# txthpc/amg

Measured on AMD Instinct MI355X. Metric: V-cycle iters/sec + fine-level SpMV GB/s (%HBM peak), 64M-row 7pt Poisson, higher is better.
Workload: dtype f64

## Files before the change

amg_amd/_native.py:

```python
from __future__ import annotations

import ctypes as C
import os
from pathlib import Path

import numpy as np

ROOT = Path(__file__).resolve().parent.parent
LIB_PATH = Path(os.environ["SSS_AMG_LIB"]) if os.environ.get("SSS_AMG_LIB") else ROOT / "amg_amd" / "lib" / "libsss_amg.so"
BIN_PATH = ROOT / "amg_amd" / "bin" / "amg"

_dbl_p = C.POINTER(C.c_double)
_int_p = C.POINTER(C.c_int)


class SSS_MAT(C.Structure):
    _fields_ = [("num_rows", C.c_int), ("num_cols", C.c_int), ("num_nnzs", C.c_int),
                ("row_ptr", _int_p), ("col_idx", _int_p), ("val", _dbl_p)]


class SSS_IMAT(C.Structure):
    _fields_ = [("num_rows", C.c_int), ("num_cols", C.c_int), ("num_nnzs", C.c_int),
                ("row_ptr", _int_p), ("col_idx", _int_p), ("val", _int_p)]


class SSS_VEC(C.Structure):
    _fields_ = [("n", C.c_int), ("d", _dbl_p)]


class SSS_IVEC(C.Structure):
    _fields_ = [("n", C.c_int), ("d", _int_p)]


class SSS_RTN(C.Structure):
    _fields_ = [("ares", C.c_double), ("rres", C.c_double), ("nits", C.c_int)]


class SSS_AMG_PARS(C.Structure):
    _fields_ = [("cycle_type", C.c_int), ("tol", C.c_double), ("ctol", C.c_double), ("max_it", C.c_int),
                ("cs_type", C.c_int), ("max_levels", C.c_int), ("coarse_dof", C.c_int), ("smoother", C.c_int),
                ("relax", C.c_double), ("cf_order", C.c_int), ("pre_iter", C.c_int), ("post_iter", C.c_int),
                ("poly_deg", C.c_int), ("interp_type", C.c_int), ("strong_threshold", C.c_double),
                ("max_row_sum", C.c_double), ("trunc_threshold", C.c_double)]


class SSS_AMG_COMP(C.Structure):
    _fields_ = [("A", SSS_MAT), ("R", SSS_MAT), ("P", SSS_MAT), ("b", SSS_VEC), ("x", SSS_VEC),
                ("cfmark", SSS_IVEC), ("wp", SSS_VEC)]


class SSS_AMG(C.Structure):
    _fields_ = [("num_levels", C.c_int), ("cg", C.POINTER(SSS_AMG_COMP)), ("pars", SSS_AMG_PARS),
                ("rtn", SSS_RTN)]


class SSS_SMTR(C.Structure):
    _fields_ = [("smoother", C.c_int), ("A", C.POINTER(SSS_MAT)), ("b", C.POINTER(SSS_VEC)),
                ("x", C.POINTER(SSS_VEC)), ("relax", C.c_double), ("nsweeps", C.c_int), ("istart", C.c_int),
                ("iend", C.c_int), ("istep", C.c_int), ("ndeg", C.c_int), ("cf_order", C.c_int),
                ("ordering", _int_p)]


class SSS_KRYLOV(C.Structure):
    _fields_ = [("tol", C.c_double), ("A", C.POINTER(SSS_MAT)), ("b", C.POINTER(SSS_VEC)),
                ("u", C.POINTER(SSS_VEC)), ("restart", C.c_int), ("matrix", C.c_int), ("stop_type", C.c_int)]


class SSS_HIP_OPTS(C.Structure):
    _fields_ = [("device", C.c_int), ("smoother", C.c_int), ("coarse", C.c_int), ("row_cap", C.c_int),
                ("use_graph", C.c_int), ("verbose", C.c_int),
                ("inner", C.c_int), ("inner_from", C.c_int), ("relabel", C.c_int),
                ("sorted_tiles", C.c_int), ("sum_order", C.c_int), ("inner_long", C.c_int), ("formats", C.c_int)]

FORMATS = {"auto": -1, "full": 0, "lean": 1}


class SSS_HIP_LEVEL_INFO(C.Structure):
    _fields_ = [("rows", C.c_int), ("nnz", C.c_int), ("nnz_p", C.c_int), ("dag_f", C.c_int),
                ("dag_c", C.c_int), ("smoother_kind", C.c_int), ("gs_engine_f", C.c_int), ("gs_engine_c", C.c_int),
                ("gs_stall", C.c_int), ("a_format", C.c_int), ("a_stream_bytes", C.c_longlong),
                ("inner", C.c_int), ("r_format", C.c_int), ("p_format", C.c_int), ("pad_", C.c_int)]


SMOOTH = {"exact": 0, "hybrid": 1, "jacobi": 2}
COARSE_RS, COARSE_PMIS = 1, 3
COARSE = {"krylov": 0, "direct": 1}
VEC = {"b": 0, "x": 1, "wp": 2}
SPMV = {"mxy": 0, "amxpy": 1, "resid": 2, "acc": 3}

ABI_SYMBOLS = [
    "SSS_amg_solve", "SSS_amg_cycle", "SSS_amg_coarest_solve", "SSS_amg_smoother_pre", "SSS_amg_smoother_post",
    "SSS_blas_mv_amxpy", "SSS_blas_mv_mxy", "SSS_solver_amg", "SSS_get_time", "SSS_free", "SSS_blas_vec_norm2",
    "SSS_print_itinfo", "SSS_exit_on_errcode", "SSS_blas_array_norm2", "SSS_blas_array_dot", "SSS_blas_array_axpy",
    "SSS_blas_array_norminf", "SSS_blas_array_set", "SSS_blas_array_axpby", "SSS_blas_array_ax", "SSS_vec_create",
    "SSS_vec_set_value", "SSS_mat_destroy", "SSS_vec_destroy", "SSS_calloc", "SSS_amg_data_create",
    "SSS_ivec_create", "SSS_mat_struct_create", "SSS_vec_cp", "SSS_iarray_cp", "SSS_blas_array_cp", "SSS_mat_cp",
    "SSS_mat_get_diag", "SSS_ivec_destroy", "SSS_amg_data_destroy", "SSS_imat_trans", "SSS_iarray_set",
    "SSS_imat_destroy", "SSS_mat_trans", "SSS_blas_mat_rap", "SSS_realloc", "SSS_amg_complexity_print",
    "SSS_amg_setup", "SSS_amg_coarsen", "SSS_amg_interp", "SSS_amg_interp_trunc", "interp_DIR", "SSS_mat_read",
    "SSS_amg_pars_init", "SSS_amg_pars_print", "mmio_info", "mmio_data",
    "sss_hip_opts_default", "sss_hip_device_count", "sss_hip_mem_info", "sss_hip_hier_create", "sss_hip_hier_destroy",
    "sss_hip_setup_create", "sss_amg_setup_hooked", "sss_hip_rap", "sss_hip_pmis", "sss_pmis_host",
    "sss_hip_std_pattern", "sss_std_pattern_host", "sss_hip_interp_std",
    "sss_hip_upload_vec", "sss_hip_download_vec", "sss_hip_cycle", "sss_hip_residual_norm", "sss_hip_pcg",
    "sss_hip_fgmres", "sss_hip_host_orth",
    "SSS_amg_save", "SSS_amg_load",
    "sss_hip_coarse_solve", "sss_hip_smooth", "sss_hip_sync", "sss_hip_level_info_get", "sss_hip_num_levels", "sss_hip_tail_from",
    "sss_hip_cycle_launches", "sss_hip_cycle_bytes",
    "sss_hip_spmv_plan_create", "sss_hip_spmv_plan_destroy", "sss_hip_spmv", "sss_hip_host_spmv", "sss_hip_host_spmv_order",
    "sss_hip_host_smooth", "sss_hip_host_coarse_solve", "sss_hip_host_cache_clear", "sss_hip_time_level0_spmv", "sss_hip_time_iterations",
    "sss_hip_time_level0_spmv_csr", "sss_hip_time_levels", "sss_hip_dist_time_tail_levels",
    "sss_gen_stencil",
    "sss_hip_rccl_unique_id", "sss_hip_comm_rccl", "sss_hip_comm_host", "sss_hip_comm_timing", "sss_hip_comm_destroy",
    "sss_hip_dist_create", "sss_hip_dist_destroy", "sss_hip_dist_info", "sss_hip_dist_level_flags",
    "sss_hip_dist_upload_vec",
    "sss_hip_dist_download_vec", "sss_hip_dist_cycle", "sss_hip_dist_residual_norm", "sss_hip_dist_sync",
    "sss_hip_dist_time_level0_spmv", "sss_hip_dist_time_levels", "sss_hip_dist_halo_stats",
    "sss_part_plan_create", "sss_part_plan_destroy", "sss_part_save", "sss_part_plan_load",
    "sss_hip_dist_create_from_files", "sss_hip_dist_level_size", "sss_part_plan_nagg", "sss_part_plan_level",
    "sss_part_plan_matrix", "sss_part_plan_ids", "sss_part_plan_halo",
]

_ip, _dp = C.POINTER(C.c_int), C.POINTER(C.c_double)
EXCHANGE_FN = C.CFUNCTYPE(C.c_int, C.c_void_p, C.c_int, _ip, _ip, _dp, C.c_int, _ip, _ip, _dp)
ALLREDUCE_FN = C.CFUNCTYPE(C.c_int, C.c_void_p, _dp, C.c_int)
ALLGATHERV_FN = C.CFUNCTYPE(C.c_int, C.c_void_p, _dp, C.c_int, _dp, _ip, _ip)


A_FORMATS = {0: "CSR (12 B/entry)", 1: "column-sorted tiles (12 B/entry)", 2: "dictionary tiles (4 B/entry)",
             3: "value-dictionary sorted tiles (5 B/entry)"}


def a_format_name(code: int) -> str:
    if code & 64:
        return "dictionary ELL (1 B/entry, padded rows)"
    if code & 128:
        return "column ELL (4 B/entry, padded rows)"
    return A_FORMATS.get(code & 3, A_FORMATS[0])


class SSS_HIP_HOST_TRANSPORT(C.Structure):
    _fields_ = [("ctx", C.c_void_p), ("exchange", EXCHANGE_FN), ("allreduce_sum", ALLREDUCE_FN),
                ("allgatherv", ALLGATHERV_FN)]

_lib = None


def _declare(lib):
    P = C.POINTER
    sig = {
        "SSS_amg_pars_init": (None, [P(SSS_AMG_PARS)]),
        "SSS_amg_pars_print": (None, [P(SSS_AMG_PARS)]),
        "SSS_amg_setup": (None, [P(SSS_AMG), P(SSS_MAT), P(SSS_AMG_PARS)]),
        "SSS_amg_data_destroy": (None, [P(SSS_AMG)]),
        "SSS_amg_solve": (SSS_RTN, [P(SSS_AMG), P(SSS_VEC), P(SSS_VEC)]),
        "SSS_print_itinfo": (None, [C.c_int, C.c_int, C.c_double, C.c_double, C.c_double]),
        "SSS_amg_cycle": (None, [P(SSS_AMG)]),
        "SSS_solver_amg": (SSS_RTN, [P(SSS_MAT), P(SSS_VEC), P(SSS_VEC), P(SSS_AMG_PARS)]),
        "SSS_mat_read": (None, [C.c_char_p, P(SSS_MAT)]),
        "SSS_mat_destroy": (None, [P(SSS_MAT)]),
        "SSS_mat_trans": (SSS_MAT, [P(SSS_MAT)]),
        "SSS_blas_mat_rap": (SSS_MAT, [P(SSS_MAT), P(SSS_MAT), P(SSS_MAT)]),
        "SSS_amg_coarsen": (C.c_int, [P(SSS_MAT), P(SSS_IVEC), P(SSS_MAT), P(SSS_IMAT), P(SSS_AMG_PARS)]),
        "SSS_amg_interp": (None, [P(SSS_MAT), P(SSS_IVEC), P(SSS_MAT), P(SSS_IMAT), P(SSS_AMG_PARS)]),
        "SSS_ivec_create": (SSS_IVEC, [C.c_int]),
        "SSS_blas_mv_amxpy": (None, [C.c_double, P(SSS_MAT), P(SSS_VEC), P(SSS_VEC)]),
        "SSS_blas_mv_mxy": (None, [P(SSS_MAT), P(SSS_VEC), P(SSS_VEC)]),
        "mmio_info": (C.c_int, [_int_p, _int_p, _int_p, _int_p, C.c_char_p]),
        "mmio_data": (C.c_int, [_int_p, _int_p, _dbl_p, C.c_char_p]),
        "sss_gen_stencil": (C.c_int, [C.c_int] * 6 + [P(SSS_MAT)]),
        "sss_hip_opts_default": (None, [P(SSS_HIP_OPTS)]),
        "sss_hip_device_count": (C.c_int, []),
        "sss_hip_mem_info": (C.c_int, [P(C.c_size_t), P(C.c_size_t)]),
        "sss_hip_hier_create": (C.c_void_p, [P(SSS_AMG), P(SSS_HIP_OPTS)]),
        "sss_hip_setup_create": (C.c_void_p, [P(SSS_AMG), P(SSS_MAT), P(SSS_AMG_PARS), P(SSS_HIP_OPTS),
                                              P(C.c_double)]),
        "sss_hip_hier_destroy": (None, [C.c_void_p]),
        "sss_hip_rap": (C.c_int, [P(SSS_MAT), P(SSS_MAT), P(SSS_MAT), P(SSS_MAT)]),
        "sss_hip_pmis": (C.c_int, [P(SSS_IMAT), _int_p, _int_p, _int_p]),
        "sss_pmis_host": (C.c_int, [P(SSS_IMAT), _int_p, _int_p, _int_p]),
        "sss_hip_std_pattern": (C.c_int, [P(SSS_IMAT), _int_p, C.c_int, P(SSS_MAT)]),
        "sss_std_pattern_host": (C.c_int, [P(SSS_IMAT), _int_p, C.c_int, P(SSS_MAT)]),
        "sss_hip_interp_std": (C.c_int, [P(SSS_MAT), P(SSS_IMAT), _int_p, P(SSS_MAT), C.c_double]),
        "SSS_mat_struct_create": (SSS_MAT, [C.c_int, C.c_int, C.c_int]),
        "sss_hip_upload_vec": (C.c_int, [C.c_void_p, C.c_int, C.c_int, _dbl_p, C.c_int]),
        "sss_hip_download_vec": (C.c_int, [C.c_void_p, C.c_int, C.c_int, _dbl_p, C.c_int]),
        "sss_hip_cycle": (C.c_int, [C.c_void_p]),
        "sss_hip_residual_norm": (C.c_int, [C.c_void_p, _dbl_p]),
        "sss_hip_pcg": (C.c_int, [C.c_void_p, C.c_double, C.c_int, P(C.c_int), _dbl_p, _dbl_p, C.c_int]),
        "sss_hip_fgmres": (C.c_int, [C.c_void_p, C.c_double, C.c_int, C.c_int, P(C.c_int), _dbl_p, _dbl_p, C.c_int]),
        "sss_hip_host_orth": (C.c_int, [C.c_int, C.c_int, _dbl_p, _dbl_p, _dbl_p, _dbl_p]),
        "SSS_amg_save": (C.c_int, [P(SSS_AMG), C.c_char_p]),
        "SSS_amg_load": (C.c_int, [P(SSS_AMG), C.c_char_p]),
        "sss_hip_coarse_solve": (C.c_int, [C.c_void_p]),
        "sss_hip_smooth": (C.c_int, [C.c_void_p, C.c_int, C.c_int]),
        "sss_hip_sync": (C.c_int, [C.c_void_p]),
        "sss_hip_level_info_get": (C.c_int, [C.c_void_p, C.c_int, P(SSS_HIP_LEVEL_INFO)]),
        "sss_hip_num_levels": (C.c_int, [C.c_void_p]),
        "sss_hip_tail_from": (C.c_int, [C.c_void_p]),
        "sss_hip_cycle_launches": (C.c_int, [C.c_void_p]),
        "sss_hip_cycle_bytes": (C.c_int, [C.c_void_p, C.POINTER(C.c_double), C.c_int]),
        "sss_hip_host_spmv": (C.c_int, [C.c_int, C.c_double, P(SSS_MAT), _dbl_p, _dbl_p, _dbl_p, C.c_int]),
        "sss_hip_host_spmv_order": (C.c_int, [C.c_int, C.c_double, P(SSS_MAT), _dbl_p, _dbl_p, _dbl_p, C.c_int, C.c_int]),
        "sss_hip_host_smooth": (C.c_int, [P(SSS_SMTR), C.c_int]),
        "sss_hip_host_coarse_solve": (C.c_int, [P(SSS_MAT), P(SSS_VEC), P(SSS_VEC), C.c_double, C.c_int,
                                                C.c_int]),
        "sss_hip_time_level0_spmv": (C.c_int, [C.c_void_p, C.c_int, _dbl_p]),
        "sss_hip_time_level0_spmv_csr": (C.c_int, [C.c_void_p, C.c_int, _dbl_p]),
        "sss_hip_time_levels": (C.c_int, [C.c_void_p, C.c_int, _dbl_p, C.c_int]),
        "sss_hip_dist_time_tail_levels": (C.c_int, [C.c_void_p, C.c_int, _dbl_p, C.c_int]),
        "sss_hip_time_iterations": (C.c_int, [C.c_void_p, C.c_int, _dbl_p, _dbl_p]),
        "sss_hip_rccl_unique_id": (C.c_int, [C.c_char_p]),
        "sss_hip_comm_rccl": (C.c_void_p, [C.c_int, C.c_int, C.c_char_p, C.c_int]),
        "sss_hip_comm_host": (C.c_void_p, [C.c_int, C.c_int, P(SSS_HIP_HOST_TRANSPORT)]),
        "sss_hip_comm_timing": (C.c_void_p, [C.c_int, C.c_int]),
        "sss_hip_comm_destroy": (None, [C.c_void_p]),
        "sss_hip_dist_create": (C.c_void_p, [P(SSS_AMG), P(SSS_HIP_OPTS), C.c_void_p, C.c_int]),
        "sss_hip_dist_destroy": (None, [C.c_void_p]),
        "sss_hip_dist_info": (C.c_int, [C.c_void_p, _int_p, _int_p, _int_p, _int_p]),
        "sss_hip_dist_level_size": (C.c_int, [C.c_void_p, C.c_int, _int_p, _int_p, P(C.c_longlong)]),
        "sss_hip_dist_level_flags": (C.c_int, [C.c_void_p, C.c_int]),
        "sss_hip_dist_upload_vec": (C.c_int, [C.c_void_p, C.c_int, _dbl_p, C.c_int]),
        "sss_hip_dist_download_vec": (C.c_int, [C.c_void_p, C.c_int, _dbl_p, C.c_int]),
        "sss_hip_dist_cycle": (C.c_int, [C.c_void_p]),
        "sss_hip_dist_residual_norm": (C.c_int, [C.c_void_p, _dbl_p]),
        "sss_hip_dist_sync": (C.c_int, [C.c_void_p]),
        "sss_hip_dist_time_level0_spmv": (C.c_int, [C.c_void_p, C.c_int, _dbl_p]),
        "sss_hip_dist_time_levels": (C.c_int, [C.c_void_p, C.c_int, _dbl_p, _dbl_p, C.c_int]),
        "sss_hip_dist_halo_stats": (C.c_int, [C.c_void_p, P(C.c_longlong), P(C.c_longlong), C.c_int, C.c_int,
                                              _int_p, _int_p, _int_p]),
        "sss_part_plan_create": (C.c_void_p, [P(SSS_AMG), C.c_int, C.c_int, C.c_int]),
        "sss_part_save": (C.c_int, [P(SSS_AMG), C.c_int, C.c_int, C.c_char_p]),
        "sss_part_plan_load": (C.c_void_p, [C.c_char_p]),
        "sss_hip_dist_create_from_files": (C.c_void_p, [C.c_char_p, P(SSS_HIP_OPTS), C.c_void_p]),
        "sss_part_plan_destroy": (None, [C.c_void_p]),
        "sss_part_plan_nagg": (C.c_int, [C.c_void_p]),
        "sss_part_plan_level": (C.c_int, [C.c_void_p, C.c_int, _int_p, _int_p, _int_p, _int_p]),
        "sss_part_plan_matrix": (C.c_int, [C.c_void_p, C.c_int, C.c_int, P(SSS_MAT)]),
        "sss_part_plan_ids": (C.c_int, [C.c_void_p, C.c_int, P(_int_p), P(_int_p)]),
        "sss_part_plan_halo": (C.c_int, [C.c_void_p, C.c_int, _int_p, P(_int_p), P(_int_p), P(_int_p), _int_p,
                                         P(_int_p), P(_int_p)]),
    }
    for name, (res, args) in sig.items():
        try:
            fn = getattr(lib, name)
        except AttributeError:
            if os.environ.get("SSS_AMG_LIB"):
                continue
            raise
        fn.restype = res
        fn.argtypes = args
    return lib


def lib():
    global _lib
    if _lib is None:
        if not LIB_PATH.exists():
            raise RuntimeError(f"{LIB_PATH} is missing: run `make` (or __graft_entry__.build())")
        _lib = _declare(C.CDLL(str(LIB_PATH)))
    return _lib


def dptr(a: np.ndarray):
    assert a.dtype == np.float64 and a.flags["C_CONTIGUOUS"]
    return a.ctypes.data_as(_dbl_p)


def iptr(a: np.ndarray):
    assert a.dtype == np.int32 and a.flags["C_CONTIGUOUS"]
    return a.ctypes.data_as(_int_p)


def csr_arrays(M: SSS_MAT, copy: bool = True):
    n, nnz = M.num_rows, M.num_nnzs
    rp = np.ctypeslib.as_array(M.row_ptr, shape=(n + 1,))
    ci = np.ctypeslib.as_array(M.col_idx, shape=(nnz,)) if nnz else np.zeros(0, np.int32)
    v = np.ctypeslib.as_array(M.val, shape=(nnz,)) if nnz else np.zeros(0, np.float64)
    return (rp.copy(), ci.copy(), v.copy()) if copy else (rp, ci, v)


class NumpyCSR:

    def __init__(self, rp, ci, v, ncols=None):
        self.rp = np.ascontiguousarray(rp, dtype=np.int32)
        self.ci = np.ascontiguousarray(ci, dtype=np.int32)
        self.v = np.ascontiguousarray(v, dtype=np.float64)
        n = len(self.rp) - 1
        self.mat = SSS_MAT(n, n if ncols is None else ncols, len(self.v), iptr(self.rp), iptr(self.ci),
                           dptr(self.v))


def default_pars() -> SSS_AMG_PARS:
    p = SSS_AMG_PARS()
    lib().SSS_amg_pars_init(C.byref(p))
    return p


def pmis(rp, ci, device: bool = False):
    rp = np.ascontiguousarray(rp, dtype=np.int32)
    ci = np.ascontiguousarray(ci, dtype=np.int32)
    n = len(rp) - 1
    S = SSS_IMAT(n, n, len(ci), iptr(rp), iptr(ci) if len(ci) else None, None)
    mark = np.full(max(n, 1), -7, np.int32)
    nc, rounds = C.c_int(-1), C.c_int(-1)
    fn = lib().sss_hip_pmis if device else lib().sss_pmis_host
    rc = fn(C.byref(S), iptr(mark), C.byref(nc), C.byref(rounds))
    if rc != 0:
        err = RuntimeError(f"PMIS split failed ({rc})")
        err.rc, err.mark = rc, mark[:n]
        raise err
    return mark[:n], nc.value, rounds.value


def _imat(rp, ci):
    rp = np.ascontiguousarray(rp, dtype=np.int32)
    ci = np.ascontiguousarray(ci, dtype=np.int32)
    n = len(rp) - 1
    return SSS_IMAT(n, n, len(ci), iptr(rp), iptr(ci) if len(ci) else None, None), (rp, ci)


def std_pattern(rp, ci, mark, device: bool = False):
    S, keep = _imat(rp, ci)
    mark = np.ascontiguousarray(mark, dtype=np.int32)
    P = SSS_MAT()
    fn = lib().sss_hip_std_pattern if device else lib().sss_std_pattern_host
    rc = fn(C.byref(S), iptr(mark), int((mark == 1).sum()), C.byref(P))
    if rc != 0:
        err = RuntimeError(f"standard pattern failed ({rc})")
        err.rc = rc
        raise err
    prp, pci, _ = csr_arrays(P)
    lib().SSS_mat_destroy(C.byref(P))
    return prp, pci


def interp_std(A_csr, S_csr, mark, P_pattern, trunc: float, device: bool = False):
    Am = NumpyCSR(*A_csr)
    S, keep = _imat(*S_csr)
    mark = np.ascontiguousarray(mark, dtype=np.int32)
    prp = np.ascontiguousarray(P_pattern[0], dtype=np.int32)
    pci = np.ascontiguousarray(P_pattern[1], dtype=np.int32)
    n = len(prp) - 1
    P = lib().SSS_mat_struct_create(n, int((mark == 1).sum()), len(pci))
    C.memmove(P.row_ptr, prp.ctypes.data, prp.nbytes)
    if len(pci):
        C.memmove(P.col_idx, pci.ctypes.data, pci.nbytes)
    try:
        if device:
            rc = lib().sss_hip_interp_std(C.byref(Am.mat), C.byref(S), iptr(mark), C.byref(P), trunc)
            if rc != 0:
                err = RuntimeError(f"standard interpolation failed ({rc})")
                err.rc = rc
                raise err
# ... 473 lines not shown
```

amg_amd/csrc/sss_build.hip:

```cpp
#include <hipcub/hipcub.hpp>

#include "sss_engine.hpp"

namespace sss {

namespace {

__global__ __launch_bounds__(kBlock) void merged_keys(int n, int G, const int *__restrict__ rp,
                                                      const int *__restrict__ ci, const int *__restrict__ seg,
                                                      unsigned *__restrict__ key)
{
    const int r = blockIdx.x * kBlock + threadIdx.x;
    if (r >= n) return;
    const unsigned rig = (unsigned)(r % G);
    const int s = seg ? seg[r] : rp[r + 1];
    for (int k = rp[r]; k < rp[r + 1]; ++k)
        key[k] = ((unsigned)ci[k] << kMergeShift) | ((k >= s ? 1u : 0u) << 3) | rig;
}

__global__ __launch_bounds__(kBlock) void group_bounds(int n, int G, int ng, const int *__restrict__ rp,
                                                       int *__restrict__ gp)
{
    const int g = blockIdx.x * kBlock + threadIdx.x;
    if (g < ng) gp[g] = rp[g * G];
    else if (g == ng) gp[g] = rp[n];
}

__global__ __launch_bounds__(kBlock) void segment_offsets(int n, const int *__restrict__ rp, const int *__restrict__ seg,
                                                          int *__restrict__ off)
{
    const int r = blockIdx.x * kBlock + threadIdx.x;
    if (r < n) {
        off[2 * r] = rp[r];
        off[2 * r + 1] = seg[r];
    } else if (r == n) {
        off[2 * n] = rp[n];
    }
}

int segmented_sort(const unsigned *kin, unsigned *kout, const double *vin, double *vout, int nnz, int nseg,
                   const int *off, hipStream_t s)
{
    if (nnz == 0 || nseg == 0) return 0;
    size_t tb = 0;
    SSS_HIP(hipcub::DeviceSegmentedRadixSort::SortPairs(nullptr, tb, kin, kout, vin, vout, nnz, nseg, off, off + 1, 0,
                                                        32, s));
    void *tmp = nullptr;
    SSS_HIP(hipMalloc(&tmp, std::max<size_t>(tb, 1)));
    const hipError_t e = hipcub::DeviceSegmentedRadixSort::SortPairs(tmp, tb, kin, kout, vin, vout, nnz, nseg, off,
                                                                     off + 1, 0, 32, s);
    const hipError_t e2 = hipStreamSynchronize(s);
    (void)hipFree(tmp);
    SSS_HIP(e);
    SSS_HIP(e2);
    return 0;
}

int upload_seg(const int *h_seg, int n, int **d_seg)
{
    *d_seg = nullptr;
    if (!h_seg) return 0;
    *d_seg = dev_alloc<int>((size_t)n);
    if (!*d_seg) return hip_fail(hipErrorOutOfMemory, "hipMalloc(seg)", __FILE__, __LINE__);
    return h2d(*d_seg, h_seg, sizeof(int) * (size_t)n);
}

}

bool device_builders_on()
{
    const char *e = getenv("SSS_HIP_GPU_BUILD");
    return !(e && *e == '0');
}

int merged_build_device(DevCSR &d, const int *h_seg)
{
    const int n = d.n, G = d.mg_G, ng = (n + G - 1) / G;
    d.mg_ng = ng;
    d.mg_gp = dev_alloc<int>((size_t)ng + 1);
    d.mg_k = dev_alloc<unsigned>((size_t)d.nnz);
    d.mg_v = dev_alloc<double>((size_t)d.nnz);
    unsigned *key = dev_alloc<unsigned>((size_t)d.nnz);
    int *dseg = nullptr;
    int rc = (!d.mg_gp || !d.mg_k || !d.mg_v || !key) ? hip_fail(hipErrorOutOfMemory, "hipMalloc(merged)", __FILE__, __LINE__)
                                                        : upload_seg(h_seg, n, &dseg);
    if (!rc) {
        hipLaunchKernelGGL(group_bounds, dim3((ng + kBlock) / kBlock), dim3(kBlock), 0, nullptr, n, G, ng, d.rp, d.mg_gp);
        if (n > 0)
            hipLaunchKernelGGL(merged_keys, dim3((n + kBlock - 1) / kBlock), dim3(kBlock), 0, nullptr, n, G, d.rp, d.ci,
                               dseg, key);
        const hipError_t e = hipGetLastError();
        if (e != hipSuccess) rc = hip_fail(e, "merged_keys", __FILE__, __LINE__);
    }
    if (!rc) rc = segmented_sort(key, d.mg_k, d.v, d.mg_v, d.nnz, ng, d.mg_gp, nullptr);
    dev_free(key);
    dev_free(dseg);
    return rc;
}

int sort_rows_device(DevCSR &d, const int *h_seg)
{
    const int n = d.n;
    unsigned *kin = dev_alloc<unsigned>((size_t)d.nnz);
    double *vin = dev_alloc<double>((size_t)d.nnz);
    int *dseg = nullptr, *off = nullptr;
    int rc = (!kin || !vin) ? hip_fail(hipErrorOutOfMemory, "hipMalloc(row sort)", __FILE__, __LINE__) : 0;
    if (!rc && h_seg) {
        rc = upload_seg(h_seg, n, &dseg);
        off = rc ? nullptr : dev_alloc<int>(2 * (size_t)n + 1);
        if (!rc && !off) rc = hip_fail(hipErrorOutOfMemory, "hipMalloc(row sort)", __FILE__, __LINE__);
        if (!rc) hipLaunchKernelGGL(segment_offsets, dim3((n + kBlock) / kBlock), dim3(kBlock), 0, nullptr, n, d.rp, dseg, off);
    }
    if (!rc && hipMemcpy(kin, d.ci, sizeof(int) * (size_t)d.nnz, hipMemcpyDeviceToDevice) != hipSuccess) rc = ERROR_MISC;
    if (!rc && hipMemcpy(vin, d.v, sizeof(double) * (size_t)d.nnz, hipMemcpyDeviceToDevice) != hipSuccess) rc = ERROR_MISC;
    if (!rc)
        rc = segmented_sort(kin, reinterpret_cast<unsigned *>(d.ci), vin, d.v, d.nnz, h_seg ? 2 * n : n,
                            h_seg ? off : d.rp, nullptr);
    if (!rc) d.rows_sorted = true;
    dev_free(kin);
    dev_free(vin);
    dev_free(dseg);
    dev_free(off);
    return rc;
}

}
```

amg_amd/csrc/sss_engine.hpp:

```cpp
#pragma once

#include <hip/hip_runtime.h>

#include <algorithm>
#include <atomic>
#include <chrono>
#include <cstdlib>
#include <string>
#include <functional>
#include <memory>
#include <cstdio>
#include <thread>
#include <vector>

#include "../../include/sss_hip.h"

extern "C" void sss_trace_push(const char *fmt, ...) __attribute__((format(printf, 1, 2)));
extern "C" void sss_trace_pop(void);
namespace sss {
struct TraceRange {
    template <class... Args>
    explicit TraceRange(const char *fmt, Args... a) { sss_trace_push(fmt, a...); }
    ~TraceRange() { sss_trace_pop(); }
    TraceRange(const TraceRange &) = delete;
// ... 20 lines not shown
inline T *dev_alloc(size_t count)
{
    void *p = nullptr;
    if (count == 0) count = 1;
    if (hipMalloc(&p, count * sizeof(T)) != hipSuccess) return nullptr;
    return static_cast<T *>(p);
}
inline void dev_free(void *p)
{
    if (p) (void)hipFree(p);
}

template <class T>
struct HostBuf {
    std::unique_ptr<T[]> p;
    size_t n = 0;
    void resize(size_t m)
    {
        p.reset(m ? new T[m] : nullptr);
        sss_huge_hint(p.get(), m * sizeof(T));
        n = m;
    }
    T *data() { return p.get(); }
    const T *data() const { return p.get(); }
    size_t size() const { return n; }
    T &operator[](size_t i) { return p[i]; }
    const T &operator[](size_t i) const { return p[i]; }
};

int host_pool_threads();
void host_thread_background();
bool host_pool_run(const std::function<void()> &work);

template <class Fn>
void parallel_chunks(int n, int grain, Fn fn)
{
    if (n <= 0) return;
    if (n <= grain || host_pool_threads() <= 1) {
        fn(0, n);
        return;
    }
    std::atomic<int> next{0};
    std::function<void()> work = [&]() {
        for (;;) {
            const int lo = next.fetch_add(grain);
            if (lo >= n) return;
            fn(lo, std::min(n, lo + grain));
        }
    };
    if (!host_pool_run(work)) work();
}

struct PhaseTimer {
    const char *what;
    bool on;
    double t;
    std::vector<std::pair<const char *, double>> marks;
    static double now()
    {
        return std::chrono::duration<double>(std::chrono::steady_clock::now().time_since_epoch()).count();
    }
    explicit PhaseTimer(const char *w) : what(w)
    {
        const char *e = getenv("SSS_HIP_TIMING");
        on = e && atoi(e) >= 2;
        t = now();
    }
    void mark(const char *name)
    {
        if (!on) return;
        const double t1 = now();
        marks.emplace_back(name, t1 - t);
        t = t1;
    }
    ~PhaseTimer()
    {
        if (!on || marks.empty()) return;
        std::string s;
        char buf[96];
        for (auto &m : marks) {
            snprintf(buf, sizeof(buf), " %s %.3f", m.first, m.second);
            s += buf;
        }
        fprintf(stderr, "[sss_hip]     %s:%s\n", what, s.c_str());
    }
};

inline void parallel_prefix(int *a, int n)
{
    constexpr int kC = 1 << 16;
    const int nc = (n + kC - 1) / kC;
    if (nc <= 1) {
        for (int i = 0; i < n; ++i) a[i + 1] += a[i];
        return;
    }
    std::vector<long long> tot((size_t)nc + 1, 0);
    parallel_chunks(nc, 1, [&](int c0, int c1) {
        for (int c = c0; c < c1; ++c) {
            long long t = 0;
            for (int i = c * kC; i < std::min(n, (c + 1) * kC); ++i) t += a[i + 1];
            tot[(size_t)c + 1] = t;
        }
    });
    tot[0] = a[0];
    for (int c = 0; c < nc; ++c) tot[(size_t)c + 1] += tot[c];
    parallel_chunks(nc, 1, [&](int c0, int c1) {
        for (int c = c0; c < c1; ++c) {
            long long run = tot[c];
            for (int i = c * kC; i < std::min(n, (c + 1) * kC); ++i) run += a[i + 1], a[i + 1] = (int)run;
        }
    });
}

int h2d(void *dst, const void *src, size_t bytes);

struct DevCSR {
    int n = 0, ncols = 0, nnz = 0;
    int *rp = nullptr, *ci = nullptr;
    double *v = nullptr;
    int nblk = 0;
    int *blk = nullptr;
    int2 *bk = nullptr;
    const int2 *h_bk = nullptr;
    int split_row = -1;
    int split_blk = 0;
    bool wave_rows = false;
    int ngrid = 0;
    unsigned *pk = nullptr;
    double *pv = nullptr;
    int2 *pb = nullptr;
    bool vec_rows = false;
    bool rows_sorted = false;
    bool tree_long = false;
    unsigned char *dv_ell = nullptr;
    int ell_w = 0;
    int *dv_ell_base = nullptr;
    unsigned *dv_xell = nullptr;
    int xell_w = 0;
    int xell_shift = 0;
    long long stream_bytes = 0;
    unsigned *dv_code = nullptr;
    unsigned char *dv_vi = nullptr;
    int4 *dv_pd = nullptr;
    int *dv_dd = nullptr;
    double *dv_vd = nullptr;
    int mg_G = 0;
    int mg_ng = 0;
    int mg_W = 4;
    int mg_acc = 0;
    int *mg_gp = nullptr;
    bool mg_two = false;
    unsigned *mg_k = nullptr;
    double *mg_v = nullptr;
};
constexpr int kMergeShift = 4;
constexpr int kTileShift = 11;
constexpr int kTileColBits = 20;
constexpr unsigned kTileDiagMark = (1u << kTileColBits) - 256;
static_assert((1 << kTileShift) == kTileEntries, "tile packing");
static_assert(1 + kTileColBits + kTileShift == 32, "tile packing");
enum { kEncSortedTiles = 1, kEncFreeOrder = 2, kEncDict = 4, kEncMergedOnly = 8, kEncXell = 16,
       kEncEll = 32,
       kEncEllBase = 64 };
int devcsr_upload(DevCSR &d, const SSS_MAT &h, int split = -1, int enc = 0, const int *seg = nullptr);
int level_encoding(const sss_hip_opts &o);
int transfer_encoding(const sss_hip_opts &o);
int restriction_encoding(const sss_hip_opts &o);
void devcsr_free(DevCSR &d);
int build_row_blocks(const int *h_rp, int n, std::vector<int> &blk, int split = -1);
int upload_block_bounds(int2 **dst, const std::vector<int> &blk, const int *h_rp, const int2 **host = nullptr);
int wave_row_min();
int free_row_min();
int devcsr_sort_rows(DevCSR &d, const SSS_MAT &h, const int *seg = nullptr);
bool device_builders_on();
int merged_build_device(DevCSR &d, const int *h_seg);
int sort_rows_device(DevCSR &d, const int *h_seg);
struct DevDict;
DevDict devdict(const DevCSR &A, int blo);
inline bool has_dict(const DevCSR &A)
{
    return A.dv_code != nullptr || A.dv_vi != nullptr || A.dv_ell != nullptr || A.dv_xell != nullptr;
}
constexpr int kXell = 256;
constexpr int rows_per_wg(int K) { return K >= kXell ? 1 : K >= 8 ? 2 : 1; }
template <class F>
inline void with_tile_kind(const DevCSR &A, F f)
{
    if (A.dv_xell) {
        if (A.xell_w == 8) f(std::integral_constant<int, kXell + 8>{});
        else if (A.xell_w == 16) f(std::integral_constant<int, kXell + 16>{});
        else if (A.xell_w == 20) f(std::integral_constant<int, kXell + 20>{});
        else if (A.xell_w == 24) f(std::integral_constant<int, kXell + 24>{});
        else if (A.xell_w == 32) f(std::integral_constant<int, kXell + 32>{});
        else f(std::integral_constant<int, kXell + 40>{});
    } else if (A.dv_ell) {
        if (A.ell_w == 8) f(std::integral_constant<int, 8>{});
        else if (A.ell_w == 16) f(std::integral_constant<int, 16>{});
        else f(std::integral_constant<int, 32>{});
    } else if (has_dict(A)) {
        f(std::integral_constant<int, 1>{});
    } else {
        f(std::integral_constant<int, 0>{});
    }
}
template <class F>
inline bool with_merged_kind(const DevCSR &A, F f)
{
    if (A.mg_G == 8 && A.mg_acc) f(std::integral_constant<int, 8>{}, std::true_type{});
    else if (A.mg_G == 8) f(std::integral_constant<int, 8>{}, std::false_type{});
    else if (A.mg_G == 4 && A.mg_acc) f(std::integral_constant<int, 4>{}, std::true_type{});
    else if (A.mg_G == 4) f(std::integral_constant<int, 4>{}, std::false_type{});
    else return false;
    return true;
}

struct ByteLedger {
    double bytes[kMaxLevels + 2] = {};
    int slot = 0;
};
extern thread_local ByteLedger *g_ledger;
inline void ledger_add(double b)
{
    if (g_ledger) g_ledger->bytes[g_ledger->slot] += b;
}
inline bool ledger_on() { return g_ledger != nullptr; }
double matrix_bytes(const DevCSR &A, int blo, int bhi);
double matrix_bytes_rows(const DevCSR &A, int lo, int hi);
inline double xgather_bytes(const DevCSR &A, double rows) { return A.n ? 8.0 * rows * A.ncols / A.n : 0.0; }

sss_hip_hier *hier_create_impl(const SSS_AMG *mg, const sss_hip_opts *o, int level_base, hipStream_t stream);
double *hier_vec(sss_hip_hier *h, int level, int which);
const std::vector<int> &hier_perm(sss_hip_hier *h, int level);
int level_kind_of(const sss_hip_opts &o, int global_level);
int hier_stall_check(sss_hip_hier *h);
unsigned *hier_err_word(sss_hip_hier *h);
bool hier_coarse_on_device(sss_hip_hier *h);
void hier_set_err_word(sss_hip_hier *h, unsigned *err);
int level_inner_of(const sss_hip_opts &o, int global_level, long long rows, long long nnz);

int launch_spmv(const DevCSR &A, int op, double alpha, const double *x, const double *b, double *y,
                int cap, double *partial, hipStream_t stream);
int launch_prolong_inject(int m, int lo, const int *col, const double *e, double *x, hipStream_t stream);
int launch_spmv_range(const DevCSR &A, int blo, int bhi, int op, double alpha, const double *x, const double *b,
                      double *y, double *partial, hipStream_t stream);
inline int launch_spmv_blocks(const DevCSR &A, int nblk, int op, double alpha, const double *x, const double *b,
                              double *y, double *partial, hipStream_t stream)
{
    return launch_spmv_range(A, 0, nblk, op, alpha, x, b, y, partial, stream);
}

struct GsPersist {
    int engine = 0;
    int lo = 0, hi = 0;
    int G = 64;
    bool overlap = false;
    bool natural = false, desc = false;
    int nchunks = 0, grid = 0;
    int *ck = nullptr;
    int *h_off = nullptr;
    unsigned *ctl = nullptr;
    unsigned *err = nullptr;
    int spin = 0;
    unsigned long long *gran = nullptr;
};
struct GsFused {
    int engine = 0;
    int sweeps = 0;
    int n = 0, split = 0;
    int G = 64;
    bool overlap = false;
    int shards = 8;
    int depth = 0, nchunks = 0, grid = 0;
    int *ck = nullptr;
    int *nodes = nullptr;
    int *rp0 = nullptr, *ci0 = nullptr;
    double *v0 = nullptr;
    unsigned *ctl = nullptr;
    unsigned *err = nullptr;
    int spin = 0;
    unsigned long long *gran = nullptr;
};
struct PassSchedule {
    int depth = 0;
    std::vector<int> h_off;
    int *rows = nullptr;
    int nrows = 0;
    int max_width = 0;
    bool compact = false;
    bool range = false;
    int lo = 0, hi = 0, blo = 0, bhi = 0;
    double *y2 = nullptr;
    DevCSR ts_nl, ts_lo;
    int *ts_split = nullptr;
    double *ts_P = nullptr;
    DevCSR sub;
    int *map = nullptr;
    double *y = nullptr;
    GsPersist gp;
};
int gs_persist_build(PassSchedule &ps, const SSS_MAT &A, int lo, int hi, bool long_rows, bool natural = false,
                     bool desc = false);
void gs_persist_free(PassSchedule &ps);
int gs_persist_run(const PassSchedule &ps, const DevCSR &A, const double *b, double *x, const double *deff,
                   hipStream_t s);
int gs_persist_error(const PassSchedule &ps, unsigned *out);
int gs_fused_build(GsFused &f, const SSS_MAT &A, const DevCSR *dA, const PassSchedule *pass, const int *cls,
                   int sweeps);
int gs_fused_run(const GsFused &f, const DevCSR &A, const double *b, double *x, const double *d_first,
                 const double *d_later, bool x_zero, hipStream_t s);
void gs_fused_free(GsFused &f);
int gs_fused_error(const GsFused &f, unsigned *out, bool clear);
struct SmootherPlan;
void smoother_set_err(SmootherPlan &sp, unsigned *err);
int launch_err_flag(unsigned *err, double *out, hipStream_t s);
struct SmootherPlan {
    int kind = SSS_HIP_SMOOTH_EXACT;
    bool natural = false;
    double *nd_first = nullptr, *nd_later = nullptr;
    PassSchedule pass[2];
    GsFused fz;
    double *d_first = nullptr;
    double *d_later = nullptr;
    int *cls = nullptr;
    bool long_rows = false;
    int *diag_pos = nullptr;
    int inner = 0;
    double *x2 = nullptr;
    int csplit = 0;
    bool fuse_resid = false;
    bool f_overwritten = false;
    bool own_diag = false;
    bool pend_ok = false;
    bool finite = false;
};
struct ResidFuse {
    double *r = nullptr;
    double *partial = nullptr;
    bool done = false;
};
struct PassHooks {
    void *ctx = nullptr;
    int (*exchange)(void *ctx, double *vec) = nullptr;
    double *w0 = nullptr, *w1 = nullptr;
    std::function<int(double *vec, int blo, int bhi, const std::function<void(int, int)> &launch)> split;
};
int smoother_build(SmootherPlan &sp, const SSS_MAT &A, const int *mark, int kind, const DevCSR *dA = nullptr,
                   int inner = 0, const int *gcls = nullptr, int enc = 0);
int smoother_build_natural(SmootherPlan &sp, const SSS_MAT &A, int lo, int hi);
struct XSrc {
    const double *f, *c;
    int split;
    __device__ __forceinline__ double operator()(int j) const { return j < split ? f[j] : c[j]; }
};
inline XSrc xsrc_of(const double *x) { return XSrc{x, x, 0x7fffffff}; }
void launch_ts_stage0(const DevCSR &M, int lo, const int *split, const double *b, XSrc x, const double *deff,
                      double *P, double *y, hipStream_t s);
void launch_ts_inner(const DevCSR &M, int lo, const double *deff, const double *P, const double *ycols, int col_off,
                     const double *ykeep, double *y, hipStream_t s);
void smoother_free(SmootherPlan &sp);
int smoother_run(const SmootherPlan &sp, const DevCSR &A, const double *b, double *x, int sweeps,
                 hipStream_t stream, const PassHooks *hooks = nullptr, ResidFuse *rf = nullptr,
                 const double *pre_f = nullptr, bool x_zero = false, bool post = false);
int launch_f_residual_pending(const SmootherPlan &sp, const DevCSR &A, const double *b, const double *x, double *r,
                              double *partial, double *pend, hipStream_t s);
// ... 36 lines not shown
```

amg_amd/csrc/sss_hier.hip:

```cpp
#include "sss_engine.hpp"
#include "sss_tail.hpp"

#include <atomic>
#include <condition_variable>
#include <mutex>
#include <thread>

#include <chrono>

#include <cmath>

#include <algorithm>
#include <cstdlib>
#include <cstring>
#include <string>
#include <thread>
#include <vector>

using namespace sss;

struct sss_hip_hier {
    int nl = 0;
    SSS_AMG_PARS pars{};
    sss_hip_opts opts{};
// ... 1197 lines not shown
    };
    SSS_HIP(hipMemcpyAsync(bs, L.b, bytes, hipMemcpyDeviceToDevice, s));
    SSS_HIP(hipMemcpyAsync(xs, L.x, bytes, hipMemcpyDeviceToDevice, s));
    double nb = 0.0, rel = 1.0;
    int it = 0;
    std::vector<double> R((size_t)(m + 1) * m, 0.0), cs((size_t)m), sn((size_t)m), g((size_t)m + 1);
    if ((rc = norm_of(bs, &nb))) return rc;
    if (!std::isfinite(nb)) rc = ERROR_SOLVER_EXIT;
    if (!rc && nb == 0.0) {
        SSS_HIP(hipMemsetAsync(xs, 0, bytes, s));
        rel = 0.0;
    }
    bool done = rc || nb == 0.0 || maxit < 1;
    while (!done) {
        double beta = 0.0;
        if ((rc = launch_spmv(L.A, SSS_HIP_SPMV_RESID, -1.0, xs, bs, V, 0, nullptr, s))) break;
        if ((rc = norm_of(V, &beta))) break;
        if (!std::isfinite(beta)) {
            rc = ERROR_SOLVER_EXIT;
            break;
        }
        if (it == 0) rel = beta / nb;
        if (beta == 0.0) break;
        if ((rc = launch_scale_inv(n, V, dh, s))) break;
        g[0] = beta;
        int ncols = 0;
        for (int j = 0; j < m && !done; ++j) {
            ++it;
            double *w = V + (size_t)(j + 1) * ld, *hj = R.data() + (size_t)j * (m + 1);
            if ((rc = precondition(V + (size_t)j * ld, Z + (size_t)j * ld))) break;
            if ((rc = launch_spmv(L.A, SSS_HIP_SPMV_MXY, 1.0, Z + (size_t)j * ld, nullptr, w, 0, nullptr, s))) break;
            if ((rc = launch_orth_step(n, j + 1, V, ld, w, h->fg_part, dc, dh, s))) break;
            if ((rc = launch_scale_inv(n, w, dh + j + 1, s))) break;
            if ((rc = fetch(dh, j + 2))) break;
            if (!std::isfinite(hh[j + 1])) {
                rc = ERROR_SOLVER_EXIT;
                break;
            }
            for (int i = 0; i < j + 2; ++i) hj[i] = hh[i];
            for (int i = 0; i < j; ++i) {
                const double t = cs[i] * hj[i] + sn[i] * hj[i + 1];
                hj[i + 1] = -sn[i] * hj[i] + cs[i] * hj[i + 1];
                hj[i] = t;
            }
            const double d = std::hypot(hj[j], hj[j + 1]);
            cs[j] = d != 0.0 ? hj[j] / d : 1.0;
            sn[j] = d != 0.0 ? hj[j + 1] / d : 0.0;
            hj[j] = d;
            g[j + 1] = -sn[j] * g[j];
            g[j] = cs[j] * g[j];
            rel = std::fabs(g[j + 1]) / nb;
            if (hist && it <= hist_cap) hist[it - 1] = rel;
            ncols = j + 1;
            done = rel < tol || it >= maxit || hh[j + 1] == 0.0;
        }
        if (rc) break;
        for (int i = ncols - 1; i >= 0; --i) {
            double t = g[i];
            for (int l = i + 1; l < ncols; ++l) t -= R[(size_t)l * (m + 1) + i] * yh[l];
            yh[i] = R[(size_t)i * (m + 1) + i] != 0.0 ? t / R[(size_t)i * (m + 1) + i] : 0.0;
        }
        SSS_HIP(hipMemcpyAsync(dy, yh, sizeof(double) * (size_t)ncols, hipMemcpyHostToDevice, s));
        if ((rc = launch_multi_axpy(n, ncols, Z, ld, dy, 1.0, xs, nullptr, s))) break;
        SSS_HIP(hipStreamSynchronize(s));
    }
    SSS_HIP(hipMemcpyAsync(L.x, xs, bytes, hipMemcpyDeviceToDevice, s));
    SSS_HIP(hipMemcpyAsync(L.b, bs, bytes, hipMemcpyDeviceToDevice, s));
    SSS_HIP(hipStreamSynchronize(s));
    h->resid_c_ready = false;
    h->pending_f = false;
    if (iters) *iters = it;
    if (relres) *relres = rel;
    if (rc) return rc;
    return hier_stall_check(h);
}

extern "C" int sss_hip_sync(sss_hip_hier *h)
{
    SSS_HIP(hipStreamSynchronize(h->stream));
    return hier_stall_check(h);
}

extern "C" int sss_hip_num_levels(sss_hip_hier *h) { return h ? h->nl : 0; }

extern "C" int sss_hip_cycle_bytes(sss_hip_hier *h, double *out, int nslots)
{
    if (!h || !out || nslots < h->nl + 2) return ERROR_INPUT_PAR;
    const bool pend = h->pending_f && h->nl > 1 && h->pars.pre_iter > 0;
    const bool f_only_next = h->nl > 1 && h->L[0].sm.fuse_resid && h->pars.post_iter > 0;
    const bool keep_pending = h->pending_f, keep_ready = h->resid_c_ready;
    ByteLedger led;
    SSS_HIP(hipStreamSynchronize(h->stream));
    SSS_HIP(hipStreamBeginCapture(h->stream, hipStreamCaptureModeThreadLocal));
    g_ledger = &led;
    int rc = walk_cycle(h, [](sss_hip_hier *hh) {
        return hh->coarse_mode == SSS_HIP_COARSE_DIRECT ? coarse_direct_apply(hh->direct, hh->L[hh->nl - 1].b,
                                                                              hh->L[hh->nl - 1].x, hh->stream)
                                                        : 0;
    }, pend);
    led.slot = kMaxLevels;
    if (!rc) rc = enqueue_residual_norm(h, f_only_next);
    g_ledger = nullptr;
    hipGraph_t g = nullptr;
    hipError_t e = hipStreamEndCapture(h->stream, &g);
    if (g) (void)hipGraphDestroy(g);
    h->pending_f = keep_pending;
    h->resid_c_ready = keep_ready;
    if (rc) return rc;
    SSS_HIP(e);
    for (int i = 0; i < nslots; ++i) out[i] = 0.0;
    for (int l = 0; l < h->nl && l < kMaxLevels; ++l) out[l] = led.bytes[l];
    out[nslots - 2] = led.bytes[kMaxLevels];
    out[nslots - 1] = led.bytes[kMaxLevels + 1];
    return 0;
}

extern "C" int sss_hip_tail_from(sss_hip_hier *h) { return h ? h->tail.from : -1; }

extern "C" int sss_hip_cycle_launches(sss_hip_hier *h)
{
    if (!h || !(h->cycle_graph_ready || h->cycle_graph_ready_p)) return -1;
    return h->cycle_graph_ready_p ? h->cycle_kernels_p : h->cycle_kernels;
}

extern "C" int sss_hip_level_info_get(sss_hip_hier *h, int level, sss_hip_level_info *out)
{
    if (!h || level < 0 || level >= h->nl) return ERROR_INPUT_PAR;
    auto &L = h->L[level];
    out->rows = L.A.n;
    out->nnz = L.A.nnz;
    out->nnz_p = L.P.nnz;
    out->dag_f = L.sm.pass[0].depth;
    out->dag_c = L.sm.pass[1].depth;
    out->smoother_kind = L.sm.kind;
    out->inner = L.sm.inner;
    out->gs_engine_f = L.sm.fz.engine ? 3 : L.sm.pass[0].gp.engine;
    out->gs_engine_c = L.sm.fz.engine ? 3 : L.sm.pass[1].gp.engine;
    unsigned ef = 0, ec = 0, ez = 0;
    if (gs_persist_error(L.sm.pass[0], &ef) || gs_persist_error(L.sm.pass[1], &ec)) return ERROR_MISC;
    if (L.sm.fz.err && hipMemcpy(&ez, L.sm.fz.err, sizeof(unsigned), hipMemcpyDeviceToHost) != hipSuccess)
        return ERROR_MISC;
    out->gs_stall = (int)(ef | ec | ez);
    auto fmt = [](const DevCSR &M) {
        return (M.pk ? 1 : 0) | (has_dict(M) ? 2 : 0) | (M.vec_rows ? 4 : 0) | (M.mg_G ? 8 : 0) | (M.wave_rows ? 16 : 0) |
               (M.dv_ell ? 64 : 0) | (M.dv_xell ? 128 : 0);
    };
    out->a_format = fmt(L.A);
    out->r_format = level + 1 < h->nl ? fmt(L.R) : 0;
    out->p_format = level + 1 < h->nl ? fmt(L.P) : 0;
    out->a_stream_bytes = L.A.stream_bytes;
    return 0;
}

extern "C" int sss_hip_time_levels(sss_hip_hier *h, int reps, double *level_ms, int nslots)
{
    if (!h || reps < 1 || nslots < h->nl) return ERROR_INPUT_PAR;
    const size_t nev = (size_t)4 * h->nl + 4;
    h->lev_ev.assign(nev, nullptr);
    h->lev_tag.assign(nev, -1);
    int rc = 0;
    for (auto &e : h->lev_ev)
        if (hipEventCreate(&e) != hipSuccess) rc = ERROR_MISC;
    std::vector<double> acc((size_t)h->nl, 0.0);
    for (int r = 0; r < reps && !rc; ++r) {
        h->lev_n = 0;
        h->resid_c_ready = h->pending_f = false;
        rc = walk_cycle(h, [](sss_hip_hier *hh) { return sss_hip_coarse_solve(hh); }, false);
        if (!rc && hipStreamSynchronize(h->stream) != hipSuccess) rc = ERROR_MISC;
        for (int k = 1; k < h->lev_n && !rc; ++k) {
            float t = 0.0f;
            if (hipEventElapsedTime(&t, h->lev_ev[(size_t)k - 1], h->lev_ev[(size_t)k]) != hipSuccess) rc = ERROR_MISC;
            const int lv = h->lev_tag[(size_t)k];
            if (lv >= 0 && lv < h->nl) acc[(size_t)lv] += t;
        }
    }
    for (hipEvent_t e : h->lev_ev)
        if (e) (void)hipEventDestroy(e);
    h->lev_ev.clear();
    h->lev_tag.clear();
    h->lev_n = 0;
    h->resid_c_ready = h->pending_f = false;
    if (rc) return rc;
    for (int l = 0; l < h->nl; ++l) level_ms[l] = acc[(size_t)l] / reps;
    return 0;
}

extern "C" int sss_hip_time_level0_spmv(sss_hip_hier *h, int reps, double *avg_ms)
{
    auto &L = h->L[0];
    SSS_HIP(hipStreamSynchronize(h->stream));
    SSS_HIP(hipEventRecord(h->ev0, h->stream));
    for (int r = 0; r < reps; ++r) {
        int rc = launch_spmv(L.A, SSS_HIP_SPMV_RESID, -1.0, L.x, L.b, L.wp, 0, nullptr, h->stream);
        if (rc) return rc;
    }
    SSS_HIP(hipEventRecord(h->ev1, h->stream));
    SSS_HIP(hipEventSynchronize(h->ev1));
    float ms = 0.f;
    SSS_HIP(hipEventElapsedTime(&ms, h->ev0, h->ev1));
    *avg_ms = (double)ms / reps;
    return 0;
}

extern "C" int sss_hip_time_level0_spmv_csr(sss_hip_hier *h, int reps, double *avg_ms)
{
    auto &L = h->L[0];
    if (L.A.wave_rows || L.A.vec_rows || L.A.dv_xell) return sss_hip_time_level0_spmv(h, reps, avg_ms);
    DevCSR c = L.A;
    c.pk = nullptr;
    c.pv = nullptr;
    c.pb = nullptr;
    c.dv_ell = nullptr;
    c.dv_code = nullptr;
    c.dv_vi = nullptr;
    SSS_HIP(hipStreamSynchronize(h->stream));
    SSS_HIP(hipEventRecord(h->ev0, h->stream));
    for (int r = 0; r < reps; ++r) {
        int rc = launch_spmv(c, SSS_HIP_SPMV_RESID, -1.0, L.x, L.b, L.wp, 0, nullptr, h->stream);
        if (rc) return rc;
    }
    SSS_HIP(hipEventRecord(h->ev1, h->stream));
    SSS_HIP(hipEventSynchronize(h->ev1));
    float ms = 0.f;
    SSS_HIP(hipEventElapsedTime(&ms, h->ev0, h->ev1));
    *avg_ms = (double)ms / reps;
    return 0;
}

extern "C" int sss_hip_time_iterations(sss_hip_hier *h, int reps, double *avg_ms, double *absres)
{
    SSS_HIP(hipStreamSynchronize(h->stream));
    SSS_HIP(hipEventRecord(h->ev0, h->stream));
    for (int r = 0; r < reps; ++r) {
        int rc = sss_hip_cycle(h);
        if (!rc) rc = sss_hip_residual_norm(h, absres);
        if (rc) return rc;
    }
    SSS_HIP(hipEventRecord(h->ev1, h->stream));
    SSS_HIP(hipEventSynchronize(h->ev1));
    float ms = 0.f;
    SSS_HIP(hipEventElapsedTime(&ms, h->ev0, h->ev1));
    *avg_ms = (double)ms / reps;
    return 0;
}

extern char **environ;

namespace {
struct HostCSR {
    DevCSR d;
    ~HostCSR() { devcsr_free(d); }
};
struct HostSmooth {
    std::mutex run;
    DevCSR d;
    SmootherPlan sp;
    ~HostSmooth()
    {
        smoother_free(sp);
        devcsr_free(d);
    }
};
struct HostCoarse {
    std::mutex run;
    DevCSR d;
    CoarseDirect cd;
    bool direct = false;
    CoarseKrylov *k = nullptr;
    ~HostCoarse()
    {
        if (direct) coarse_direct_free(cd);
        coarse_krylov_destroy(k);
        devcsr_free(d);
    }
};

inline unsigned long long mix64(unsigned long long h, unsigned long long w)
{
    h ^= w * 0x9E3779B97F4A7C15ull;
    h = (h << 31) | (h >> 33);
    return h * 0xC2B2AE3D27D4EB4Full;
}
unsigned long long hash_bytes(const void *p, size_t n, unsigned long long seed)
{
    const unsigned char *b = static_cast<const unsigned char *>(p);
    constexpr size_t kChunk = (size_t)1 << 20;
    const int nc = (int)((n + kChunk - 1) / kChunk);
    std::vector<unsigned long long> part((size_t)std::max(nc, 1), 0);
    parallel_chunks(nc, 1, [&](int c0, int c1) {
        for (int c = c0; c < c1; ++c) {
            const size_t lo = (size_t)c * kChunk, hi = std::min(n, lo + kChunk);
            unsigned long long h = 0x2545F4914F6CDD1Dull ^ (unsigned long long)c;
            size_t i = lo;
            for (; i + 8 <= hi; i += 8) {
                unsigned long long w;
                std::memcpy(&w, b + i, 8);
                h = mix64(h, w);
            }
            for (; i < hi; ++i) h = mix64(h, b[i]);
            part[(size_t)c] = h;
        }
    });
    unsigned long long h = mix64(seed, n);
    for (auto v : part) h = mix64(h, v);
    return h;
}
// ... 202 lines not shown
```

amg_amd/csrc/sss_smooth.hip:

```cpp
#include "sss_engine.hpp"
#include "sss_spmv_dev.hpp"

#include <algorithm>
#include <chrono>
#include <cstdlib>
#include <type_traits>
#include <cmath>

namespace sss {

template <class T>
static int upload_array(T **dst, const T *src, size_t count)
{
    *dst = dev_alloc<T>(count);
    if (!*dst) return hip_fail(hipErrorOutOfMemory, "hipMalloc(plan array)", __FILE__, __LINE__);
    return count == 0 ? 0 : h2d(*dst, src, sizeof(T) * count);
}
static int upload_ints(int **dst, const std::vector<int> &src) { return upload_array(dst, src.data(), src.size()); }
static int upload_ints(int **dst, const HostBuf<int> &src) { return upload_array(dst, src.data(), src.size()); }
static int upload_doubles(double **dst, const HostBuf<double> &src) { return upload_array(dst, src.data(), src.size()); }
static int upload_doubles(double **dst, const std::vector<double> &src) { return upload_array(dst, src.data(), src.size()); }

int smoother_build(SmootherPlan &sp, const SSS_MAT &A, const int *mark, int kind, const DevCSR *dA, int inner,
                   const int *gcls, int enc)
// ... 613 lines not shown
        if (partial && valid) {
            const double t = block_sum(sq, es.red);
            if (threadIdx.x == 0) partial[bid] = t;
        }
    }
}

template <int MODE, int DICT = 0>
__device__ __forceinline__ void relax_range_body(int blo, const int2 *__restrict__ blk, const int *__restrict__ rp,
                                                      const int *__restrict__ ci, const double *__restrict__ v,
                                                      const int *__restrict__ diag_pos, int lo,
                                                      const double *__restrict__ b, double *x,
                                                      const double *__restrict__ yp, double *__restrict__ y,
                                                      const double *__restrict__ deff, const unsigned *__restrict__ pk,
                                                      const double *__restrict__ pv, const int2 *__restrict__ pb,
                                                      double *__restrict__ rr, double *__restrict__ partial, XSrc xs,
                                                      DevDict dt = DevDict())
{
    if constexpr (DICT >= kXell) {
        relax_range_xell<MODE, DICT - kXell>(blo, blk, lo, b, x, y, deff, rr, partial, xs, dt);
    } else if constexpr (DICT == 8 && kEllPairs) {
        relax_range_ell2<MODE>(blo, blk, lo, b, x, y, deff, rr, partial, xs, dt);
    } else if constexpr (DICT >= 8) {
        relax_range_ell<MODE, DICT>(blo, blk, lo, b, x, y, deff, rr, partial, xs, dt);
    } else {
    __shared__ SpmvSmem sm;
    __shared__ std::conditional_t<DICT != 0, DictSmem, char> dsm;
    DictSmem *ds = nullptr;
    if constexpr (DICT != 0) ds = &dsm;
    const int bid = blo + xcd_bid();
    const int2 ba = blk[bid], be = blk[bid + 1];
    const int r0 = ba.x, r1 = be.x, k0 = ba.y, k1 = be.y;
    auto fetch = [&](int c) -> double { return xs(c); };
    auto dval = [&](int r) -> double { return deff ? deff[r] : sm.d[r - r0]; };
    auto finish = [&](int r, double acc) {
        const double d = dval(r);
        if (MODE != 1) {
            if (div_ok(d)) x[r] = acc / d;
        } else {
            y[r - lo] = div_ok(d) ? acc / d : xs(r);
        }
    };
    if (k1 - k0 <= kTileEntries) {
        const int r = r0 + (int)threadIdx.x;
        int a = 0, e = 0, dp = -1;
        double br = 0.0;
        if (r < r1) a = rp[r] - k0, e = rp[r + 1] - k0, dp = diag_pos[r], br = b[r];
        stage_any(sm.v, k0, k1, ci, v, pk, pv, pb, bid, r0, deff ? (double *)nullptr : sm.d, fetch, dt, ds, r1, rp);
        __syncthreads();
        double sq = 0.0;
        if (r < r1) {
            if constexpr (MODE >= 2) {
                const RelaxRow o = relax_row<MODE>(TileProds{sm.v}, a, dp >= 0, dp - k0, e, br, [&] { return dval(r); },
                                                   [&]() -> double { return x[r]; });
                if constexpr (MODE == 2) {
                    if (o.upd) x[r] = o.xn;
                } else {
                    y[r - lo] = o.xn;
                }
                rr[r] = o.res;
                sq = o.res * o.res;
            } else {
                finish(r, relax_acc(TileProds{sm.v}, a, dp >= 0, dp - k0, e, br));
            }
        }
        if constexpr (MODE >= 2) {
            if (partial) {
                const double t = block_sum(sq, sm.red);
                if (threadIdx.x == 0) partial[bid] = t;
            }
        }
    } else if constexpr (MODE < 2) {
        const int r = r0, dp = diag_pos[r];
        const double acc = long_row_chunks(
            k0, k1, b[r],
            [&](int base, int m) {
                stage_any(sm.v, base, base + m, ci, v, pk, pv, pb, bid, r0, deff ? (double *)nullptr : sm.d, fetch, dt,
                          ds, r1, rp);
            },
            [&](int base, int m, double acc) {
                if (dt.tree_long) {
                    if (threadIdx.x == 0 && dp >= base && dp < base + m) sm.v[dp - base] = 0.0;
                    __syncthreads();
                    const double c = block_tree_sum(sm.v, 0, m, sm.red);
                    if (threadIdx.x == 0) acc -= c;
                } else if (threadIdx.x == 0) {
                    if (dp >= base && dp < base + m) {
                        acc = chain_sub(acc, sm.v, 0, dp - base);
                        acc = chain_sub(acc, sm.v, dp - base + 1, m);
                    } else {
                        acc = chain_sub(acc, sm.v, 0, m);
                    }
                }
                return acc;
            });
        if (threadIdx.x == 0) finish(r, acc);
    }
    }
}

#define SSS_RELAX_ARGS                                                                                          \
    int blo, const int2 *__restrict__ blk, const int *__restrict__ rp, const int *__restrict__ ci,                 \
        const double *__restrict__ v, const int *__restrict__ diag_pos, int lo, const double *__restrict__ b,      \
        double *x, const double *__restrict__ yp, double *__restrict__ y, const double *__restrict__ deff,          \
        const unsigned *__restrict__ pk, const double *__restrict__ pv, const int2 *__restrict__ pb,               \
        double *__restrict__ rr, double *__restrict__ partial, XSrc xs, DevDict dt
#define SSS_RELAX_PASS blo, blk, rp, ci, v, diag_pos, lo, b, x, yp, y, deff, pk, pv, pb, rr, partial, xs, dt
template <int MODE, int DICT = 0>
__global__ __launch_bounds__(kBlock) void relax_range(SSS_RELAX_ARGS)
{
    relax_range_body<MODE, DICT>(SSS_RELAX_PASS);
}
template <int MODE, int DICT = 0>
__global__ __launch_bounds__(kBlock) __attribute__((amdgpu_waves_per_eu(5, 8))) void relax_range_occ(SSS_RELAX_ARGS)
{
    relax_range_body<MODE, DICT>(SSS_RELAX_PASS);
}
template <int M, int K, class... Args>
static void launch_relax_range(int blo, int nb, hipStream_t s, DevDict dt, Args... args)
{
    if constexpr (K < 8) {
        hipLaunchKernelGGL((relax_range_occ<M, K>), dim3(nb), dim3(kBlock), 0, s, blo, args..., dt);
    } else {
        dt.bend = blo + nb;
        hipLaunchKernelGGL((relax_range<M, K>), dim3((nb + rows_per_wg(K) - 1) / rows_per_wg(K)), dim3(kBlock), 0, s, blo,
                           args..., dt);
    }
}

template <int MODE, bool TREE>
__global__ __launch_bounds__(kBlock) void relax_range_wave(int lo, int hi, const int *__restrict__ rp,
                                                           const int *__restrict__ ci, const double *__restrict__ v,
                                                           const double *__restrict__ b, double *x,
                                                           const double *__restrict__ yp, double *__restrict__ y,
                                                           const double *__restrict__ deff, XSrc xs)
{
    __shared__ __attribute__((aligned(16))) double strips[TREE ? 1 : 4][TREE ? 1 : kWaveStage];
    const int wave = threadIdx.x >> 6;
    const int r = lo + xcd_bid() * 4 + wave;
    if (r >= hi) return;
    auto prod = [&](int c, double a) -> double { return c == r ? 0.0 : a * (MODE == 1 ? xs(c) : x[c]); };
    const double acc = TREE ? b[r] - wave_row_sum(rp[r], rp[r + 1], ci, v, prod)
                            : wave_row_chain<true>(rp[r], rp[r + 1], ci, v, prod, b[r], strips[TREE ? 0 : wave]);
    if ((threadIdx.x & 63) == 0) {
        const double d = deff[r];
        if (MODE == 0) {
            if (div_ok(d)) x[r] = acc / d;
        } else {
            y[r - lo] = div_ok(d) ? acc / d : xs(r);
        }
    }
}

template <int PATH, bool LDSACC = false>
__global__ __launch_bounds__(kBlock) void ts_stage0(int lo, DevCSR M, const int *__restrict__ split,
                                                    const double *__restrict__ b, XSrc x,
                                                    const double *__restrict__ deff, double *__restrict__ P,
                                                    double *__restrict__ y)
{
    auto finish = [&](int q, double acc) {
        const int r = lo + q;
        const double d = deff[r];
        y[q] = div_ok(d) ? acc / d : x(r);
    };
    if constexpr (PATH >= kXell) {
        constexpr int W = PATH - kXell;
        __shared__ XellSmem es;
        const int bq = blockIdx.x;
        double bq_v = 0.0, dq = 0.0;
        int sp = 0;
        const XellRow<W> row = xell_row_begin<W>(true, M.bk, bq, M.dv_xell, M.dv_pd, M.dv_vd, es, [&](int q) {
            bq_v = b[lo + q];
            dq = deff[lo + q];
            sp = split[q] - M.rp[q];
        });
        const unsigned(&w)[W] = row.w;
        const int q = row.r;
        const bool live = row.live;
        __syncthreads();
        if (live) {
            double xv[W];
            int ds;
            unsigned dcode;
            const int len = xell_gather<W>(w, -1, M.xell_shift, [&](int c) -> double { return x(c); }, xv, ds, dcode);
            const double Pq = xell_sum_bf<true>(bq_v, w, xv, es, M.xell_shift, 0, sp);
            P[q] = Pq;
            const double acc = xell_sum_bf<true>(Pq, w, xv, es, M.xell_shift, sp, len);
            y[q] = div_ok(dq) ? acc / dq : x(lo + q);
        }
        return;
    } else if constexpr (PATH >= 3) {
        constexpr int G = PATH;
        __shared__ double red[8 * G];
        __shared__ double acc[LDSACC ? 4 * 2 * G * kMergeAccDoubles : 1];
        int g = 0, u = 0;
        double n_sum = 0.0, l_sum = 0.0;
        if (merged_block<G, 2, LDSACC>(M.mg_gp, M.mg_ng, M.mg_W, M.mg_k, M.mg_v, [&](int c) -> double { return x(c); },
                                       red, acc, g, u, n_sum, l_sum)) {
            const int q = g * G + u;
            if (q < M.n) {
                const double Pq = b[lo + q] - n_sum;
                P[q] = Pq;
                finish(q, Pq - l_sum);
            }
        }
        return;
    } else if constexpr (PATH == 2) {
        const int q = xcd_bid() * 4 + (threadIdx.x >> 6);
        if (q >= M.n) return;
        auto prod = [&](int c, double a) { return a * x(c); };
        const int a = M.rp[q], sp = split[q], e = M.rp[q + 1];
        const double Pq = b[lo + q] - wave_row_sum(a, sp, M.ci, M.v, prod);
        const double acc = Pq - wave_row_sum(sp, e, M.ci, M.v, prod);
        if ((threadIdx.x & 63) == 0) {
            P[q] = Pq;
            finish(q, acc);
        }
        return;
    } else if constexpr (PATH == 1) {
        __shared__ __attribute__((aligned(16))) double strips[4][kWaveStage];
        const int wave = threadIdx.x >> 6, q = xcd_bid() * 4 + wave;
        if (q >= M.n) return;
        auto prod = [&](int c, double a) { return a * x(c); };
        const int a = M.rp[q], sp = split[q], e = M.rp[q + 1];
        double acc = wave_row_chain<true>(a, sp, M.ci, M.v, prod, b[lo + q], strips[wave]);
        acc = __shfl(acc, 0, 64);
        if ((threadIdx.x & 63) == 0) P[q] = acc;
        acc = wave_row_chain<true>(sp, e, M.ci, M.v, prod, acc, strips[wave]);
        if ((threadIdx.x & 63) == 0) finish(q, acc);
        return;
    } else {
        __shared__ SpmvSmem sm;
        const int bq = xcd_bid();
        const BlockBounds bb = block_bounds(M.bk, M.rp, bq);
        const int q0 = bb.r0, q1 = bb.r1, k0 = bb.k0, k1 = bb.k1;
        if (k1 - k0 <= kTileEntries) {
            const int q = q0 + (int)threadIdx.x;
            int a = 0, sp = 0, e = 0;
            double acc = 0.0;
            if (q < q1) a = M.rp[q] - k0, sp = split[q] - k0, e = M.rp[q + 1] - k0, acc = b[lo + q];
            stage_any(sm.v, k0, k1, M.ci, M.v, M.pk, M.pv, M.pb, bq, q0, (double *)nullptr, [&](int c) -> double { return x(c); });
            __syncthreads();
            if (q < q1) {
                acc = chain_sub(acc, sm.v, a, sp);
                P[q] = acc;
                acc = chain_sub(acc, sm.v, sp, e);
                finish(q, acc);
            }
        } else {
            const int q = q0, sp = split[q];
            const double acc = long_row_chunks(
                k0, k1, b[lo + q],
                [&](int base, int m) {
                    stage_any(sm.v, base, base + m, M.ci, M.v, M.pk, M.pv, M.pb, bq, q0, (double *)nullptr, [&](int c) -> double { return x(c); });
                },
                [&](int base, int m, double acc) {
                    if (M.tree_long) {
                        const int cut = min(max(sp - base, 0), m);
                        const double c1 = block_tree_sum(sm.v, 0, cut, sm.red);
                        const double c2 = block_tree_sum(sm.v, cut, m, sm.red);
                        if (threadIdx.x == 0) {
                            acc -= c1;
                            if (sp >= base && sp < base + m) P[q] = acc;
                            acc -= c2;
                        }
                    } else if (threadIdx.x == 0) {
                        if (sp >= base && sp < base + m) {
                            acc = chain_sub(acc, sm.v, 0, sp - base);
                            P[q] = acc;
                            acc = chain_sub(acc, sm.v, sp - base, m);
                        } else {
                            acc = chain_sub(acc, sm.v, 0, m);
                        }
                    }
                    return acc;
                });
            if (threadIdx.x == 0) {
                if (sp == k1) P[q] = acc;
                finish(q, acc);
            }
        }
    }
}

template <int PATH, bool LDSACC = false>
__global__ __launch_bounds__(kBlock) void ts_inner(int lo, DevCSR M, const double *__restrict__ deff,
                                                   const double *__restrict__ P, const double *ycols, int col_off,
                                                   const double *ykeep, double *__restrict__ y)
{
    auto fetch = [&](int c) -> double { return ycols[c - col_off]; };
    auto finish = [&](int q, double acc) {
        const double d = deff[lo + q];
        y[q] = div_ok(d) ? acc / d : ykeep[q];
    };
    if constexpr (PATH >= kXell) {
        constexpr int W = PATH - kXell;
        __shared__ XellSmem es;
        const int bq = blockIdx.x;
        double pq = 0.0, dq = 0.0;
        const XellRow<W> row = xell_row_begin<W>(true, M.bk, bq, M.dv_xell, M.dv_pd, M.dv_vd, es, [&](int q) {
            pq = P[q];
            dq = deff[lo + q];
        });
        const unsigned(&w)[W] = row.w;
        const int q = row.r;
        const bool live = row.live;
        __syncthreads();
        if (live) {
            double xv[W];
            int ds;
            unsigned dcode;
            const int len = xell_gather<W>(w, -1, M.xell_shift, fetch, xv, ds, dcode);
            const double acc = xell_sum_g<true>(pq, w, xv, es, M.xell_shift, 0, len);
            y[q] = div_ok(dq) ? acc / dq : ykeep[q];
        }
        return;
    } else if constexpr (PATH >= 3) {
        constexpr int G = PATH;
        __shared__ double red[8 * G];
        __shared__ double acc[LDSACC ? 4 * G * kMergeAccDoubles : 1];
        int g = 0, u = 0;
        double l_sum = 0.0, unused = 0.0;
        if (merged_block<G, 1, LDSACC>(M.mg_gp, M.mg_ng, M.mg_W, M.mg_k, M.mg_v, fetch, red, acc, g, u, l_sum,
                                       unused)) {
            const int q = g * G + u;
            if (q < M.n) finish(q, P[q] - l_sum);
        }
        return;
    } else if constexpr (PATH == 2) {
        const int q = xcd_bid() * 4 + (threadIdx.x >> 6);
        if (q >= M.n) return;
        const double acc =
            P[q] - wave_row_sum(M.rp[q], M.rp[q + 1], M.ci, M.v, [&](int c, double a) { return a * fetch(c); });
        if ((threadIdx.x & 63) == 0) finish(q, acc);
        return;
    } else if constexpr (PATH == 1) {
        __shared__ __attribute__((aligned(16))) double strips[4][kWaveStage];
        const int wave = threadIdx.x >> 6, q = xcd_bid() * 4 + wave;
        if (q >= M.n) return;
        const double acc = wave_row_chain<true>(
            M.rp[q], M.rp[q + 1], M.ci, M.v, [&](int c, double a) { return a * fetch(c); }, P[q], strips[wave]);
        if ((threadIdx.x & 63) == 0) finish(q, acc);
        return;
    } else {
        __shared__ SpmvSmem sm;
        const int bq = xcd_bid();
        const BlockBounds bb = block_bounds(M.bk, M.rp, bq);
        const int q0 = bb.r0, q1 = bb.r1, k0 = bb.k0, k1 = bb.k1;
        if (k1 - k0 <= kTileEntries) {
            const int q = q0 + (int)threadIdx.x;
            int a = 0, e = 0;
            double acc = 0.0;
            if (q < q1) a = M.rp[q] - k0, e = M.rp[q + 1] - k0, acc = P[q];
            stage_any(sm.v, k0, k1, M.ci, M.v, M.pk, M.pv, M.pb, bq, q0, (double *)nullptr, fetch);
            __syncthreads();
            if (q < q1) finish(q, chain_sub(acc, sm.v, a, e));
        } else {
            const int q = q0;
            const double acc = long_row_chunks(
                k0, k1, P[q],
                [&](int base, int m) {
                    stage_any(sm.v, base, base + m, M.ci, M.v, M.pk, M.pv, M.pb, bq, q0, (double *)nullptr, fetch);
                },
                [&](int, int m, double acc) {
                    if (M.tree_long) {
                        const double c = block_tree_sum(sm.v, 0, m, sm.red);
                        if (threadIdx.x == 0) acc -= c;
                    } else if (threadIdx.x == 0) {
                        acc = chain_sub(acc, sm.v, 0, m);
                    }
                    return acc;
                });
            if (threadIdx.x == 0) finish(q, acc);
        }
    }
}

static void ledger_pass(const DevCSR &A, const PassSchedule &ps, double vec)
{
    if (!ledger_on()) return;
    const double mat = ps.range ? matrix_bytes_rows(A, ps.lo, ps.hi)
                                : (A.n ? (double)A.stream_bytes * ps.nrows / A.n : 0.0);
    ledger_add(mat + (8.0 + vec) * ps.nrows);
}

void launch_ts_stage0(const DevCSR &M, int lo, const int *split, const double *b, XSrc x, const double *deff,
                      double *P, double *y, hipStream_t s)
{
    if (M.n == 0) return;
    ledger_add((double)M.stream_bytes + 40.0 * M.n);
    if (M.mg_two && with_merged_kind(M, [&](auto G, auto ACC) {
            hipLaunchKernelGGL((ts_stage0<decltype(G)::value, decltype(ACC)::value>), dim3(M.ngrid), dim3(kBlock), 0, s,
                               lo, M, split, b, x, deff, P, y);
        }))
        return;
    if (M.vec_rows)
        hipLaunchKernelGGL(ts_stage0<2>, dim3((M.n + 3) / 4), dim3(kBlock), 0, s, lo, M, split, b, x, deff, P, y);
    else if (M.wave_rows)
        hipLaunchKernelGGL(ts_stage0<1>, dim3(M.ngrid), dim3(kBlock), 0, s, lo, M, split, b, x, deff, P, y);
    else if (M.dv_xell)
        with_tile_kind(M, [&](auto K) {
            constexpr int KK = decltype(K)::value;
            if constexpr (KK >= kXell)
                hipLaunchKernelGGL(ts_stage0<KK>, dim3(M.nblk), dim3(kBlock), 0, s, lo, M, split, b, x, deff, P, y);
        });
    else
        hipLaunchKernelGGL(ts_stage0<0>, dim3(M.nblk), dim3(kBlock), 0, s, lo, M, split, b, x, deff, P, y);
}

void launch_ts_inner(const DevCSR &M, int lo, const double *deff, const double *P, const double *ycols, int col_off,
                     const double *ykeep, double *y, hipStream_t s)
{
    if (M.n == 0) return;
    ledger_add((double)M.stream_bytes + 40.0 * M.n);
    if (with_merged_kind(M, [&](auto G, auto ACC) {
            hipLaunchKernelGGL((ts_inner<decltype(G)::value, decltype(ACC)::value>), dim3(M.ngrid), dim3(kBlock), 0, s,
                               lo, M, deff, P, ycols, col_off, ykeep, y);
        }))
        return;
    if (M.vec_rows)
        hipLaunchKernelGGL(ts_inner<2>, dim3((M.n + 3) / 4), dim3(kBlock), 0, s, lo, M, deff, P, ycols, col_off, ykeep, y);
    else if (M.wave_rows)
        hipLaunchKernelGGL(ts_inner<1>, dim3(M.ngrid), dim3(kBlock), 0, s, lo, M, deff, P, ycols, col_off, ykeep, y);
    else if (M.dv_xell)
        with_tile_kind(M, [&](auto K) {
            constexpr int KK = decltype(K)::value;
            if constexpr (KK >= kXell)
                hipLaunchKernelGGL(ts_inner<KK>, dim3(M.nblk), dim3(kBlock), 0, s, lo, M, deff, P, ycols, col_off, ykeep,
                                   y);
        });
    else
        hipLaunchKernelGGL(ts_inner<0>, dim3(M.nblk), dim3(kBlock), 0, s, lo, M, deff, P, ycols, col_off, ykeep, y);
}

__device__ __forceinline__ double zero_x_sum(double t, const int *__restrict__ ci, const double *__restrict__ v, int a,
                                             int e, int skip_col)
{
    if (t == 0.0 && signbit(t))
        for (int k = a; k < e; ++k)
            if (ci[k] != skip_col && signbit(v[k])) return 0.0;
    return t;
}

template <bool TWO>
__global__ __launch_bounds__(kBlock) void zero_first_pass(int lo, int m, const int *__restrict__ rp,
                                                          const int *__restrict__ ci, const double *__restrict__ v,
                                                          const int *__restrict__ split, const double *__restrict__ b,
                                                          const double *__restrict__ deff, double *__restrict__ P,
                                                          double *__restrict__ y)
{
    const int q = blockIdx.x * kBlock + threadIdx.x;
    if (q >= m) return;
    const int r = lo + q;
    double t;
    if (TWO) {
        const double Pq = zero_x_sum(b[r], ci, v, rp[q], split[q], -1);
        P[q] = Pq;
        t = zero_x_sum(Pq, ci, v, split[q], rp[q + 1], -1);
    } else {
        t = zero_x_sum(b[r], ci, v, rp[r], rp[r + 1], r);
    }
    const double d = deff[r];
    y[q] = div_ok(d) ? t / d : 0.0;
}

int launch_f_residual_pending(const SmootherPlan &sp, const DevCSR &A, const double *b, const double *x, double *r,
                              double *partial, double *pend, hipStream_t s)
{
    if (!sp.pend_ok) return ERROR_INPUT_PAR;
    const PassSchedule &F = sp.pass[0];
    const double *deff = (sp.own_diag && (A.pk || has_dict(A))) ? nullptr : sp.d_first;
    ledger_pass(A, F, deff ? 40.0 : 32.0);
    with_tile_kind(A, [&](auto K) {
        launch_relax_range<3, decltype(K)::value>(F.blo, F.bhi - F.blo, s, devdict(A, 0), A.bk, A.rp, A.ci, A.v,
                                                  sp.diag_pos, F.lo, b, const_cast<double *>(x), (const double *)nullptr,
                                                  pend, deff, A.pk, A.pv, A.pb, r, partial, xsrc_of(x));
    });
    SSS_HIP(hipGetLastError());
    return 0;
}

__global__ __launch_bounds__(kBlock) void scatter_rows(int m, const int *__restrict__ map, const double *__restrict__ y,
                                                       double *__restrict__ x)
{
    const int r = blockIdx.x * kBlock + threadIdx.x;
    if (r < m) x[map[r]] = y[r];
}

static int depth_launches(const PassSchedule &ps, bool long_rows, bool nat, const DevCSR &A, const double *b, double *x,
                          const double *deff, hipStream_t s)
{
    ledger_pass(A, ps, 24.0);
    for (int l = 0; l < ps.depth; ++l) {
        const int off = ps.h_off[l], cnt = ps.h_off[l + 1] - off;
        if (cnt == 0) continue;
        if (long_rows)
            hipLaunchKernelGGL(nat ? gs_depth_wave<true> : gs_depth_wave<false>, dim3((cnt + 3) / 4), dim3(kBlock), 0, s,
                               ps.rows + off, cnt, A.rp, A.ci, A.v, b, x, deff);
        else
            hipLaunchKernelGGL(nat ? gs_depth_thread<true> : gs_depth_thread<false>, dim3((cnt + kBlock - 1) / kBlock),
                               dim3(kBlock), 0, s, ps.rows + off, cnt, A.rp, A.ci, A.v, b, x, deff);
    }
    SSS_HIP(hipGetLastError());
    return 0;
}

int smoother_build_natural(SmootherPlan &sp, const SSS_MAT &A, int lo, int hi)
{
    const int n = A.num_rows, m = hi - lo;
    const int *rp = A.row_ptr, *ci = A.col_idx;
    const double *v = A.val;
    int rc;
    sp.kind = SSS_HIP_SMOOTH_EXACT;
    sp.natural = true;
    long long nnz = 0;
    for (int i = lo; i < hi; ++i) nnz += rp[i + 1] - rp[i];
    sp.long_rows = m > 0 && nnz >= (long long)std::min(32, wave_row_min()) * m;
    std::vector<double> df[2] = {std::vector<double>(n, 0.0), std::vector<double>(n, 0.0)},
                        dl[2] = {std::vector<double>(n, 0.0), std::vector<double>(n, 0.0)};
    for (int dir = 0; dir < 2; ++dir) {
        double d = 0.0;
        for (int sweep = 0; sweep < 2; ++sweep)
            for (int q = 0; q < m; ++q) {
                const int i = dir == 0 ? lo + q : hi - 1 - q;
                for (int k = rp[i]; k < rp[i + 1]; ++k)
                    if (ci[k] == i && SSS_ABS(v[k]) > SMALLFLOAT) d = 1.e+0 / v[k];
                (sweep == 0 ? df : dl)[dir][i] = d;
            }
    }
    for (int dir = 0; dir < 2; ++dir) {
        PassSchedule &ps = sp.pass[dir];
        std::vector<int> depth(n, 0), pushed(n, 0);
        auto in = [&](int j) { return j >= lo && j < hi; };
        for (int q = 0; q < m; ++q) {
            const int i = dir == 0 ? lo + q : hi - 1 - q;
            int dep = pushed[i];
            for (int k = rp[i]; k < rp[i + 1]; ++k) {
                const int j = ci[k];
                if (in(j) && (dir == 0 ? j < i : j > i)) dep = std::max(dep, depth[j] + 1);
            }
            depth[i] = dep;
            for (int k = rp[i]; k < rp[i + 1]; ++k) {
                const int j = ci[k];
                if (in(j) && (dir == 0 ? j > i : j < i)) pushed[j] = std::max(pushed[j], dep + 1);
            }
        }
        int maxd = -1;
        for (int i = lo; i < hi; ++i) maxd = std::max(maxd, depth[i]);
        ps.depth = maxd + 1;
        ps.h_off.assign(ps.depth + 1, 0);
        for (int i = lo; i < hi; ++i) ps.h_off[depth[i] + 1]++;
        for (int l = 0; l < ps.depth; ++l) ps.h_off[l + 1] += ps.h_off[l];
        ps.nrows = m;
        std::vector<int> fill(ps.h_off.begin(), ps.h_off.end()), rows(std::max(m, 1));
        for (int i = lo; i < hi; ++i) rows[fill[depth[i]]++] = i;
        if ((rc = upload_ints(&ps.rows, rows))) return rc;
        if (ps.depth > 1 && (rc = gs_persist_build(ps, A, lo, hi, sp.long_rows, true, dir == 1))) return rc;
    }
    if ((rc = upload_doubles(&sp.d_first, df[0])) || (rc = upload_doubles(&sp.d_later, dl[0])) ||
        (rc = upload_doubles(&sp.nd_first, df[1])) || (rc = upload_doubles(&sp.nd_later, dl[1])))
        return rc;
    return 0;
}

int smoother_run(const SmootherPlan &sp, const DevCSR &A, const double *b, double *x, int sweeps, hipStream_t s,
                 const PassHooks *hk, ResidFuse *rf, const double *pre_f, bool x_zero, bool post)
{
    if (sp.natural) {
        if (hk || pre_f) return ERROR_INPUT_PAR;
        if (rf) rf->done = false;
// ... 188 lines not shown
```

amg_amd/csrc/sss_spmv.hip:

```cpp
#include "sss_engine.hpp"

#include <cstdlib>
#include "sss_spmv_dev.hpp"

#include <algorithm>
#include <type_traits>
#include <condition_variable>
#include <cstring>
#include <mutex>
#include <sched.h>
#include <sys/resource.h>
#include <sys/syscall.h>
#include <unistd.h>

namespace sss {

int hip_fail(hipError_t e, const char *what, const char *file, int line)
{
    fprintf(stderr, "### ERROR: HIP call %s failed at %s:%d: %s\n", what, file, line, hipGetErrorString(e));
    return ERROR_MISC;
}

static int usable_cpus()
{
// ... 253 lines not shown
        int ord[256];
        for (int t = 0; t < n; ++t) ord[t] = t;
        std::sort(ord, ord + n, [&](int a, int b) { return (T)val[a] < (T)val[b]; });
        sorted.resize((size_t)n);
        for (int t = 0; t < n; ++t) rk[ord[t]] = (unsigned char)t, sorted[t] = (T)val[ord[t]];
    }
};
static inline unsigned long long bits_of(double d)
{
    unsigned long long u;
    std::memcpy(&u, &d, sizeof(u));
    return u;
}
static inline double double_of(unsigned long long u)
{
    double d;
    std::memcpy(&d, &u, sizeof(d));
    return d;
}

static bool build_sorted_tiles(const SSS_MAT &h, const std::vector<int> &blk, HostBuf<unsigned> &pk,
                               HostBuf<double> &pv, std::vector<int2> &pb)
{
    const int *rp = h.row_ptr, *ci = h.col_idx;
    const int nb = (int)blk.size() - 1;
    constexpr long long kSpan = kTileDiagMark;
    pk.resize((size_t)h.num_nnzs);
    pv.resize((size_t)h.num_nnzs);
    pb.resize((size_t)std::max(nb, 1));
    std::atomic<int> ok{1};
    parallel_chunks(nb, 512, [&](int qlo, int qhi) {
        std::vector<unsigned long long> key, seg;
        std::vector<int> rowof;
        for (int q = qlo; q < qhi && ok; ++q) {
            const int a0 = rp[blk[q]], e0 = rp[blk[q + 1]];
            if (a0 == e0) {
                pb[q] = make_int2(0, 0);
                continue;
            }
            rowof.resize((size_t)(e0 - a0));
            for (int r = blk[q]; r < blk[q + 1]; ++r)
                for (int k = rp[r]; k < rp[r + 1]; ++k) rowof[(size_t)(k - a0)] = r;
            key.resize((size_t)(e0 - a0));
            for (int k = a0; k < e0; ++k) key[(size_t)(k - a0)] = (unsigned long long)(unsigned)ci[k] << 32 | (unsigned)(k - a0);
            std::sort(key.begin(), key.end());
            auto col = [&](size_t t) { return (int)(key[t] >> 32); };
            const size_t m = key.size();
            size_t gap = 0;
            for (size_t t = 1; t < m; ++t)
                if (col(t) - col(t - 1) > col(gap + 1) - col(gap)) gap = t - 1;
            const int b0 = col(0), b1 = m > 1 ? col(gap + 1) : col(0);
            const int cut = b1;
            if (m > 1 && ((long long)col(gap) - b0 >= kSpan || (long long)col(m - 1) - b1 >= kSpan)) {
                ok = 0;
                return;
            }
            pb[q] = make_int2(b0, b1);
            const int r0 = blk[q];
            for (int a = a0; a < e0; a += kTileEntries) {
                const int e = std::min(e0, a + kTileEntries);
                const unsigned long long *sk = key.data();
                if (e - a != e0 - a0) {
                    seg.resize((size_t)(e - a));
                    for (int k = a; k < e; ++k) seg[(size_t)(k - a)] = (unsigned long long)(unsigned)ci[k] << 32 | (unsigned)(k - a0);
                    std::sort(seg.begin(), seg.end());
                    sk = seg.data();
                }
                for (int t = 0; t < e - a; ++t) {
                    const int k = a0 + (int)(unsigned)sk[t], c = ci[k];
                    const int r = rowof[(size_t)(k - a0)];
                    const unsigned cl = (m > 1 && c >= cut) ? 1u : 0u;
                    const unsigned off = c == r ? kTileDiagMark + (unsigned)(r - r0) : (unsigned)(c - (cl ? b1 : b0));
                    pk[(size_t)a + t] = (cl << 31) | (off << kTileShift) | (unsigned)(k - a);
                    pv[(size_t)a + t] = h.val[k];
                }
            }
        }
    });
    return ok != 0;
}

static void sort_row_segments(const SSS_MAT &h, const int *seg, HostBuf<int> &ci, HostBuf<double> &v)
{
    const int n = h.num_rows;
    const int *rp = h.row_ptr;
    ci.resize((size_t)h.num_nnzs);
    v.resize((size_t)h.num_nnzs);
    parallel_chunks(n, 256, [&](int rlo, int rhi) {
        std::vector<unsigned long long> key;
        for (int r = rlo; r < rhi; ++r) {
            const int cut[3] = {rp[r], seg ? seg[r] : rp[r + 1], rp[r + 1]};
            for (int part = 0; part < 2; ++part) {
                const int a = cut[part], e = cut[part + 1];
                key.resize((size_t)std::max(0, e - a));
                for (int t = 0; t < e - a; ++t) key[t] = (unsigned long long)(unsigned)h.col_idx[a + t] << 32 | (unsigned)t;
                std::sort(key.begin(), key.end());
                for (int t = 0; t < e - a; ++t) {
                    const int k = a + (int)(unsigned)key[t];
                    ci[(size_t)a + t] = h.col_idx[k], v[(size_t)a + t] = h.val[k];
                }
            }
        }
    });
}

static void build_merged(const SSS_MAT &h, const int *seg, int G, std::vector<int> &gp, HostBuf<unsigned> &mk,
                         HostBuf<double> &mv)
{
    const int n = h.num_rows, ng = (n + G - 1) / G;
    const int *rp = h.row_ptr, *ci = h.col_idx;
    gp.resize((size_t)ng + 1);
    mk.resize((size_t)h.num_nnzs);
    mv.resize((size_t)h.num_nnzs);
    parallel_chunks(ng, 64, [&](int glo, int ghi) {
        std::vector<std::pair<unsigned long long, int>> ent;
        std::vector<unsigned long long> key;
        for (int g = glo; g < ghi; ++g) {
            const int r0 = g * G, r1 = std::min(n, r0 + G);
            const int base = rp[r0], cnt = rp[r1] - base;
            if (cnt < (1 << 24)) {
                key.resize((size_t)cnt);
                for (int r = r0; r < r1; ++r)
                    for (int k = rp[r]; k < rp[r + 1]; ++k) {
                        const unsigned long long sg = (seg && k >= seg[r]) ? 1u : 0u;
                        key[(size_t)(k - base)] =
                            ((((unsigned long long)ci[k] << kMergeShift) | (sg << 3) | (unsigned)(r - r0)) << 24) |
                            (unsigned)(k - base);
                    }
                std::sort(key.begin(), key.end());
                gp[g] = base;
                for (int t = 0; t < cnt; ++t) {
                    mk[(size_t)base + t] = (unsigned)(key[t] >> 24);
                    mv[(size_t)base + t] = h.val[base + (int)(key[t] & 0xffffff)];
                }
                continue;
            }
            ent.clear();
            for (int r = r0; r < r1; ++r)
                for (int k = rp[r]; k < rp[r + 1]; ++k) {
                    const unsigned sg = (seg && k >= seg[r]) ? 1u : 0u;
                    ent.emplace_back(((unsigned long long)ci[k] << kMergeShift) | (sg << 3) | (unsigned)(r - r0), k);
                }
            std::sort(ent.begin(), ent.end());
            int pos = rp[r0];
            gp[g] = pos;
            for (const auto &e : ent) {
                mk[pos] = (unsigned)e.first;
                mv[pos] = h.val[e.second];
                ++pos;
            }
        }
    });
    gp[ng] = rp[n];
}

DevDict devdict(const DevCSR &A, int blo)
{
    DevDict t;
    t.tree_long = A.tree_long ? 1 : 0;
    if (!has_dict(A)) return t;
    t.code = A.dv_code;
    t.ell = A.dv_ell;
    t.ellb = A.dv_ell_base;
    t.ellw = A.ell_w;
    t.xell = A.dv_xell;
    t.xshift = A.xell_shift;
    t.pd = A.dv_pd + blo;
    t.dd = A.dv_dd;
    t.vd = A.dv_vd;
    if (A.dv_vi) {
        t.pk = A.pk;
        t.vi = A.dv_vi;
        t.pb = A.pb + blo;
    }
    return t;
}

static bool build_dict_tiles(const SSS_MAT &h, const std::vector<int> &blk, HostBuf<unsigned> &code,
                             std::vector<int4> &pd, std::vector<int> &dd, std::vector<double> &vd)
{
    const int *rp = h.row_ptr, *ci = h.col_idx;
    const double *v = h.val;
    const int nb = (int)blk.size() - 1;
    if (h.num_rows != h.num_cols || nb <= 0) return false;
    std::vector<std::vector<int>> bd(nb);
    std::vector<std::vector<unsigned long long>> bv(nb);
    code.resize((size_t)h.num_nnzs);
    std::atomic<int> ok{1};
    parallel_chunks(nb, 256, [&](int qlo, int qhi) {
        std::unique_ptr<SmallDict> Dd(new SmallDict()), Vd(new SmallDict());
        std::vector<unsigned long long> key;
        std::vector<int> rowof;
        std::vector<unsigned char> did, vid;
        for (int q = qlo; q < qhi && ok; ++q) {
            const int a0 = rp[blk[q]], e0 = rp[blk[q + 1]];
            rowof.resize((size_t)(e0 - a0));
            did.resize((size_t)(e0 - a0));
            vid.resize((size_t)(e0 - a0));
            Dd->clear();
            Vd->clear();
            for (int r = blk[q]; r < blk[q + 1]; ++r)
                for (int k = rp[r]; k < rp[r + 1]; ++k) {
                    rowof[(size_t)(k - a0)] = r;
                    const int di = Dd->insert((unsigned long long)(long long)(ci[k] - r), 256);
                    const int vi = Vd->insert(bits_of(v[k]), 256);
                    if (di < 0 || vi < 0) {
                        ok = 0;
                        return;
                    }
                    did[(size_t)(k - a0)] = (unsigned char)di;
                    vid[(size_t)(k - a0)] = (unsigned char)vi;
                }
            std::vector<long long> ds;
            Dd->finish(ds);
            Vd->finish(bv[q]);
            bd[q].assign(ds.begin(), ds.end());
            for (int a = a0; a < e0; a += kTileEntries) {
                const int e = std::min(e0, a + kTileEntries);
                key.resize((size_t)(e - a));
                for (int k = a; k < e; ++k) key[(size_t)(k - a)] = (unsigned long long)(unsigned)ci[k] << 32 | (unsigned)(k - a);
                std::sort(key.begin(), key.end());
                for (int t = 0; t < e - a; ++t) {
                    const int k = a + (int)(unsigned)key[t];
                    const unsigned dix = Dd->rk[did[(size_t)(k - a0)]], vix = Vd->rk[vid[(size_t)(k - a0)]];
                    code[(size_t)a + t] = vix << (kTileShift + 8) | dix << kTileShift | (unsigned)(k - a);
                }
            }
        }
    });
    if (!ok) return false;
    pd.resize((size_t)nb);
    size_t nd = 0, nv = 0;
    for (int q = 0; q < nb; ++q) {
        pd[q] = make_int4((int)nd, (int)bd[q].size(), (int)nv, (int)bv[q].size());
        nd += bd[q].size();
        nv += bv[q].size();
    }
    dd.resize(std::max<size_t>(nd, 1));
    vd.resize(std::max<size_t>(nv, 1));
    for (int q = 0; q < nb; ++q) {
        std::copy(bd[q].begin(), bd[q].end(), dd.begin() + pd[q].x);
        for (size_t t = 0; t < bv[q].size(); ++t) vd[(size_t)pd[q].z + t] = double_of(bv[q][t]);
    }
    return true;
}

static bool build_value_dict(const std::vector<int> &blk, const int *rp, const HostBuf<double> &pv,
                             HostBuf<unsigned char> &vi, std::vector<int4> &pd, std::vector<double> &vd)
{
    const int nb = (int)blk.size() - 1;
    if (nb <= 0) return false;
    std::vector<std::vector<unsigned long long>> bv(nb);
    vi.resize(pv.size());
    std::atomic<int> ok{1};
    parallel_chunks(nb, 256, [&](int qlo, int qhi) {
        std::unique_ptr<SmallDict> Vd(new SmallDict());
        for (int q = qlo; q < qhi && ok; ++q) {
            const int a0 = rp[blk[q]], e0 = rp[blk[q + 1]];
            Vd->clear();
            for (int k = a0; k < e0; ++k) {
                const int id = Vd->insert(bits_of(pv[(size_t)k]), 256);
                if (id < 0) {
                    ok = 0;
                    return;
                }
                vi[(size_t)k] = (unsigned char)id;
            }
            Vd->finish(bv[q]);
            for (int k = a0; k < e0; ++k) vi[(size_t)k] = Vd->rk[vi[(size_t)k]];
        }
    });
    if (!ok) return false;
    pd.resize((size_t)nb);
    size_t nv = 0;
    for (int q = 0; q < nb; ++q) {
        pd[q] = make_int4(0, 0, (int)nv, (int)bv[q].size());
        nv += bv[q].size();
    }
    vd.resize(std::max<size_t>(nv, 1));
    for (int q = 0; q < nb; ++q)
        for (size_t t = 0; t < bv[q].size(); ++t) vd[(size_t)pd[q].z + t] = double_of(bv[q][t]);
    return true;
}

static bool build_ell(const SSS_MAT &h, const std::vector<int> &blk, HostBuf<unsigned char> &ell, int &W,
                      std::vector<int4> &pd, std::vector<int> &dd, std::vector<double> &vd, const int *base = nullptr)
{
    const int *rp = h.row_ptr, *ci = h.col_idx;
    const double *v = h.val;
    const int n = h.num_rows, nb = (int)blk.size() - 1;
    if (nb <= 0 || n <= 0) return false;
    std::atomic<int> Lmax{0};
    parallel_chunks(n, 1 << 16, [&](int lo, int hi) {
        int L = 0;
        for (int r = lo; r < hi; ++r) L = std::max(L, rp[r + 1] - rp[r]);
        int cur = Lmax.load();
        while (L > cur && !Lmax.compare_exchange_weak(cur, L)) {}
    });
    const int L = Lmax.load();
    if (L > 32) return false;
    W = L <= 8 ? 8 : L <= 16 ? 16 : 32;
    std::vector<int> bdf((size_t)nb * 31), nd_of(nb), nv_of(nb);
    std::vector<double> bvf((size_t)nb * 8);
    ell.resize((size_t)n * W);
    std::atomic<int> ok{1};
    parallel_chunks(nb, 256, [&](int qlo, int qhi) {
// ... 19 lines not shown
            Vd->finish(vs);
            nd_of[q] = (int)ds.size();
            nv_of[q] = (int)vs.size();
            std::copy(ds.begin(), ds.end(), bdf.begin() + (size_t)q * 31);
            for (size_t t = 0; t < vs.size(); ++t) bvf[(size_t)q * 8 + t] = double_of(vs[t]);
            for (int r = blk[q]; r < blk[q + 1]; ++r)
                for (int k = 0; k < rp[r + 1] - rp[r]; ++k) {
                    unsigned char &c = ell[(size_t)r * W + k];
                    c = (unsigned char)(Vd->rk[c >> 5] << 5 | Dd->rk[c & 31]);
                }
        }
    });
    if (!ok) return false;
    pd.resize((size_t)nb);
    size_t nd = 0, nv = 0;
    for (int q = 0; q < nb; ++q) {
        pd[q] = make_int4((int)nd, nd_of[q], (int)nv, nv_of[q]);
        nd += nd_of[q];
        nv += nv_of[q];
    }
    dd.resize(std::max<size_t>(nd, 1));
    vd.resize(std::max<size_t>(nv, 1));
    parallel_chunks(nb, 4096, [&](int qlo, int qhi) {
        for (int q = qlo; q < qhi; ++q) {
            std::copy(bdf.begin() + (size_t)q * 31, bdf.begin() + (size_t)q * 31 + nd_of[q], dd.begin() + pd[q].x);
            std::copy(bvf.begin() + (size_t)q * 8, bvf.begin() + (size_t)q * 8 + nv_of[q], vd.begin() + pd[q].z);
        }
    });
    return true;
}

static int xell_width(int L) { return L <= 8 ? 8 : L <= 16 ? 16 : L <= 20 ? 20 : L <= 24 ? 24 : L <= 32 ? 32 : L <= 40 ? 40 : 0; }
static int xell_shift_for(int ncols)
{
    for (int S = 23; S <= 28; ++S)
        if ((long long)ncols < (1LL << S)) return S;
    return 0;
}
static int build_rows_blocks(int n, std::vector<int> &blk, int split)
{
    blk.clear();
    for (int r = 0; r < n;) {
        blk.push_back(r);
        const int lim = (split > r && split < n) ? split : n;
        r = std::min(lim, r + kBlock);
    }
    blk.push_back(n);
    return (int)blk.size() - 1;
}
struct XellValues {
    static constexpr int kSlots = 4 * kXellValues;
    unsigned long long key[kSlots];
    short slot[kSlots];
    unsigned long long val[kXellValues];
    unsigned short rk[kXellValues];
    int n = 0;
    void clear()
    {
        std::memset(slot, 0xff, sizeof(slot));
        n = 0;
    }
    int insert(unsigned long long u, int cap)
    {
        for (unsigned h = (unsigned)((u * 0x9E3779B97F4A7C15ull) >> 53) & (kSlots - 1);; h = (h + 1) & (kSlots - 1)) {
            if (slot[h] < 0) {
                if (n >= cap) return -1;
                slot[h] = (short)n;
                key[h] = u;
                val[n] = u;
                return n++;
            }
            if (key[h] == u) return slot[h];
        }
    }
    void finish(std::vector<double> &sorted)
    {
        int ord[kXellValues];
        for (int t = 0; t < n; ++t) ord[t] = t;
        std::sort(ord, ord + n, [&](int a, int b) { return val[a] < val[b]; });
        sorted.resize((size_t)n);
        for (int t = 0; t < n; ++t) rk[ord[t]] = (unsigned short)t, sorted[t] = double_of(val[ord[t]]);
    }
};
static bool build_xell(const SSS_MAT &h, int split, int W, int S, std::vector<int> &blk, HostBuf<unsigned> &codes,
                       std::vector<int4> &pd, std::vector<double> &vd)
{
    const int vcap = std::min(kXellValues, 1 << (32 - S));
    const int *rp = h.row_ptr, *ci = h.col_idx;
    const double *v = h.val;
    std::vector<int> chunks;
    const int nc = build_rows_blocks(h.num_rows, chunks, split);
    codes.resize((size_t)h.num_rows * W);
    struct Part {
        int r0;
        std::vector<double> vals;
    };
    std::vector<std::vector<Part>> parts((size_t)nc);
    std::atomic<int> ok{1};
    parallel_chunks(nc, 64, [&](int clo, int chi) {
        std::unique_ptr<XellValues> D(new XellValues());
        std::function<bool(int, int, std::vector<Part> &)> fit = [&](int r0, int r1, std::vector<Part> &out) -> bool {
            D->clear();
            bool fits = true;
            for (int k = rp[r0]; k < rp[r1] && fits; ++k) fits = D->insert(bits_of(v[k]), vcap) >= 0;
            if (!fits) {
                if (r1 - r0 <= 16) return false;
                const int mid = r0 + (r1 - r0) / 2;
                return fit(r0, mid, out) && fit(mid, r1, out);
            }
            Part p;
            p.r0 = r0;
            D->finish(p.vals);
            for (int r = r0; r < r1; ++r) {
                unsigned *row = codes.data() + (size_t)r * W;
                int s = 0;
                for (int k = rp[r]; k < rp[r + 1]; ++k, ++s)
                    row[s] = (unsigned)D->rk[D->insert(bits_of(v[k]), vcap)] << S | (unsigned)ci[k];
                for (; s < W; ++s) row[s] = 0xffffffffu;
            }
            out.push_back(std::move(p));
            return true;
        };
        for (int c = clo; c < chi && ok; ++c)
            if (!fit(chunks[c], chunks[c + 1], parts[c])) ok = 0;
    });
    if (!ok) return false;
    blk.clear();
    pd.clear();
    vd.clear();
    for (int c = 0; c < nc; ++c)
        for (const Part &p : parts[c]) {
            blk.push_back(p.r0);
            pd.push_back(make_int4(0, 0, (int)vd.size(), (int)p.vals.size()));
            vd.insert(vd.end(), p.vals.begin(), p.vals.end());
        }
    blk.push_back(h.num_rows);
    if (vd.empty()) vd.push_back(0.0);
    return true;
}
static bool xell_on()
{
    const char *e = getenv("SSS_HIP_XELL");
    return !(e && *e == '0');
}

static int merge_acc(int G, bool two)
{
    const char *e = getenv("SSS_HIP_MERGE_ACC");
    if (e && *e) return *e != '0';
    (void)G, (void)two;
    return 1;
}

int devcsr_upload(DevCSR &d, const SSS_MAT &h, int split, int enc, const int *seg)
{
    PhaseTimer pt("devcsr");
    d.n = h.num_rows;
    d.ncols = h.num_cols;
    d.nnz = h.num_nnzs;
    d.wave_rows = d.n > 0 && (long long)d.nnz >= (long long)wave_row_min() * d.n;
    d.vec_rows = d.n > 0 && (enc & kEncFreeOrder) && (long long)d.nnz >= (long long)free_row_min() * d.n;
    d.tree_long = (enc & kEncFreeOrder) && !d.vec_rows;
    if (d.vec_rows && (unsigned long long)std::max(d.ncols, 1) < (1ull << (32 - kMergeShift))) {
        d.mg_G = merge_group_size(d.n);
        if (seg && d.mg_G > 4) d.mg_G = 4;
    }
    d.rp = dev_alloc<int>((size_t)d.n + 1);
    d.ci = dev_alloc<int>((size_t)d.nnz);
    d.v = dev_alloc<double>((size_t)d.nnz);
    if (!d.rp || !d.ci || !d.v) return hip_fail(hipErrorOutOfMemory, "hipMalloc(CSR)", __FILE__, __LINE__);
    pt.mark("alloc");
    if (int rc = h2d(d.rp, h.row_ptr, sizeof(int) * ((size_t)d.n + 1))) return rc;
    if (d.nnz > 0) {
        if (d.vec_rows && !((enc & kEncMergedOnly) && d.mg_G > 0) && !device_builders_on()) {
            HostBuf<int> sci;
            HostBuf<double> sv;
            sort_row_segments(h, seg, sci, sv);
            if (int rc = h2d(d.ci, sci.data(), sizeof(int) * (size_t)d.nnz)) return rc;
            if (int rc = h2d(d.v, sv.data(), sizeof(double) * (size_t)d.nnz)) return rc;
            d.rows_sorted = true;
        } else {
            if (int rc = h2d(d.ci, h.col_idx, sizeof(int) * (size_t)d.nnz)) return rc;
            if (int rc = h2d(d.v, h.val, sizeof(double) * (size_t)d.nnz)) return rc;
        }
    }
    pt.mark("csr");
    std::vector<int> blk;
    d.nblk = build_row_blocks(h.row_ptr, d.n, blk, split);
    d.split_blk = d.nblk;
    d.split_row = split;
    if (split >= 0)
        for (int q = 0; q <= d.nblk; ++q)
            if (blk[q] >= split) { d.split_blk = q; break; }
    d.blk = dev_alloc<int>(blk.size());
    if (!d.blk) return hip_fail(hipErrorOutOfMemory, "hipMalloc(blk)", __FILE__, __LINE__);
    if (int rc = h2d(d.blk, blk.data(), sizeof(int) * blk.size())) return rc;
    if (int rc = upload_block_bounds(&d.bk, blk, h.row_ptr, &d.h_bk)) return rc;
    d.ngrid = (d.wave_rows || d.vec_rows) ? (d.n + 3) / 4 : d.nblk;
    pt.mark("blocks");
    if (d.mg_G > 0 && device_builders_on()) {
        d.mg_two = seg != nullptr;
        const char *wz = getenv("SSS_HIP_MERGE_W");
        d.mg_W = (wz && *wz) ? atoi(wz) : 4;
        d.mg_W = d.mg_W >= 4 ? 4 : d.mg_W >= 2 ? 2 : 1;
        d.mg_acc = merge_acc(d.mg_G, d.mg_two);
        if (int rc = merged_build_device(d, seg)) return rc;
        d.ngrid = (d.mg_ng + 4 / d.mg_W - 1) / (4 / d.mg_W);
    } else if (d.mg_G > 0) {
        std::vector<int> gp;
        HostBuf<unsigned> mk;
        HostBuf<double> mv;
        build_merged(h, seg, d.mg_G, gp, mk, mv);
        d.mg_two = seg != nullptr;
        d.mg_ng = (int)gp.size() - 1;
        const char *wz = getenv("SSS_HIP_MERGE_W");
        d.mg_W = (wz && *wz) ? atoi(wz) : 4;
        d.mg_W = d.mg_W >= 4 ? 4 : d.mg_W >= 2 ? 2 : 1;
        d.mg_acc = merge_acc(d.mg_G, d.mg_two);
        d.ngrid = (d.mg_ng + 4 / d.mg_W - 1) / (4 / d.mg_W);
        d.mg_gp = dev_alloc<int>(gp.size());
        d.mg_k = dev_alloc<unsigned>(mk.size());
        d.mg_v = dev_alloc<double>(mv.size());
        if (!d.mg_gp || !d.mg_k || !d.mg_v) return hip_fail(hipErrorOutOfMemory, "hipMalloc(merged)", __FILE__, __LINE__);
        if (int rc = h2d(d.mg_gp, gp.data(), sizeof(int) * gp.size())) return rc;
        if (int rc = h2d(d.mg_k, mk.data(), sizeof(unsigned) * mk.size())) return rc;
        if (int rc = h2d(d.mg_v, mv.data(), sizeof(double) * mv.size())) return rc;
    }
    if (d.vec_rows && !((enc & kEncMergedOnly) && d.mg_G > 0) && device_builders_on() && d.nnz > 0)
        if (int rc = sort_rows_device(d, seg)) return rc;
    pt.mark("merged");
    const char *dz = getenv("SSS_HIP_DICT");
    const char *ez = getenv("SSS_HIP_ELL");
    const bool based = (enc & kEncEllBase) && d.n != d.ncols;
    if ((enc & (kEncDict | kEncEll | kEncEllBase)) && !(dz && *dz == '0') && !(ez && *ez == '0') && !d.wave_rows &&
        !d.vec_rows && d.nnz > 0 && ((enc & kEncEll) || based || d.n == d.ncols)) {
        HostBuf<unsigned char> ell;
        std::vector<int4> pd;
        std::vector<int> dd;
        std::vector<double> vd;
        std::vector<int> base;
        if (based) {
            base.resize((size_t)d.n);
            parallel_chunks(d.n, 1 << 16, [&](int lo, int hi) {
                for (int r = lo; r < hi; ++r) base[r] = h.row_ptr[r] < h.row_ptr[r + 1] ? h.col_idx[h.row_ptr[r]] : 0;
            });
        }
        int W = 0;
        if (build_ell(h, blk, ell, W, pd, dd, vd, based ? base.data() : nullptr)) {
            if (based) {
                d.dv_ell_base = dev_alloc<int>(base.size());
                if (!d.dv_ell_base) return hip_fail(hipErrorOutOfMemory, "hipMalloc(ELL bases)", __FILE__, __LINE__);
                if (int rc = h2d(d.dv_ell_base, base.data(), sizeof(int) * base.size())) return rc;
            }
            d.ell_w = W;
            d.dv_ell = dev_alloc<unsigned char>(ell.size());
            d.dv_pd = dev_alloc<int4>(pd.size());
            d.dv_dd = dev_alloc<int>(dd.size());
            d.dv_vd = dev_alloc<double>(vd.size());
            if (!d.dv_ell || !d.dv_pd || !d.dv_dd || !d.dv_vd)
                return hip_fail(hipErrorOutOfMemory, "hipMalloc(dictionary ELL)", __FILE__, __LINE__);
            if (int rc = h2d(d.dv_ell, ell.data(), ell.size())) return rc;
            if (int rc = h2d(d.dv_pd, pd.data(), sizeof(int4) * pd.size())) return rc;
            if (int rc = h2d(d.dv_dd, dd.data(), sizeof(int) * dd.size())) return rc;
            if (int rc = h2d(d.dv_vd, vd.data(), sizeof(double) * vd.size())) return rc;
        }
    }
    pt.mark("ell");
    const int xshift = xell_shift_for(d.ncols);
    if ((enc & kEncXell) && !(dz && *dz == '0') && xell_on() && !d.dv_ell && !d.wave_rows && !d.vec_rows &&
        d.nnz > 0 && xshift > 0) {
        std::atomic<int> Lmax{0};
        parallel_chunks(d.n, 1 << 16, [&](int lo, int hi) {
            int L = 0;
            for (int r = lo; r < hi; ++r) L = std::max(L, h.row_ptr[r + 1] - h.row_ptr[r]);
            int cur = Lmax.load();
            while (L > cur && !Lmax.compare_exchange_weak(cur, L)) {}
        });
        int W = xell_width(Lmax.load());
        if ((long long)d.nnz * 3 < (long long)W * d.n) W = 0;
        if (W == 40 && !(enc & kEncMergedOnly)) W = 0;
        std::vector<int> xb;
        HostBuf<unsigned> codes;
        std::vector<int4> pd;
        std::vector<double> vd;
        if (W > 0 && build_xell(h, split, W, xshift, xb, codes, pd, vd)) {
            dev_free(d.blk);
            dev_free(d.bk);
            d.blk = nullptr;
            d.bk = nullptr;
            blk.swap(xb);
            d.nblk = (int)blk.size() - 1;
            d.split_blk = d.nblk;
            if (split >= 0)
                for (int q = 0; q <= d.nblk; ++q)
                    if (blk[q] >= split) { d.split_blk = q; break; }
            d.ngrid = d.nblk;
            d.blk = dev_alloc<int>(blk.size());
            if (!d.blk) return hip_fail(hipErrorOutOfMemory, "hipMalloc(blk)", __FILE__, __LINE__);
            if (int rc = h2d(d.blk, blk.data(), sizeof(int) * blk.size())) return rc;
            if (int rc = upload_block_bounds(&d.bk, blk, h.row_ptr, &d.h_bk)) return rc;
            d.xell_w = W;
            d.xell_shift = xshift;
            d.dv_xell = dev_alloc<unsigned>(codes.size());
            d.dv_pd = dev_alloc<int4>(pd.size());
            d.dv_vd = dev_alloc<double>(vd.size());
            if (!d.dv_xell || !d.dv_pd || !d.dv_vd)
                return hip_fail(hipErrorOutOfMemory, "hipMalloc(column ELL)", __FILE__, __LINE__);
            if (int rc = h2d(d.dv_xell, codes.data(), sizeof(unsigned) * codes.size())) return rc;
            if (int rc = h2d(d.dv_pd, pd.data(), sizeof(int4) * pd.size())) return rc;
            if (int rc = h2d(d.dv_vd, vd.data(), sizeof(double) * vd.size())) return rc;
        }
    }
    pt.mark("xell");
    if ((enc & kEncDict) && !(dz && *dz == '0') && !d.dv_ell && !d.dv_xell && !d.wave_rows && !d.vec_rows && d.nnz > 0) {
        HostBuf<unsigned> code;
        std::vector<int4> pd;
        std::vector<int> dd;
        std::vector<double> vd;
        if (build_dict_tiles(h, blk, code, pd, dd, vd)) {
            d.dv_code = dev_alloc<unsigned>(code.size());
            d.dv_pd = dev_alloc<int4>(pd.size());
            d.dv_dd = dev_alloc<int>(dd.size());
            d.dv_vd = dev_alloc<double>(vd.size());
            if (!d.dv_code || !d.dv_pd || !d.dv_dd || !d.dv_vd)
                return hip_fail(hipErrorOutOfMemory, "hipMalloc(dictionary tiles)", __FILE__, __LINE__);
            if (int rc = h2d(d.dv_code, code.data(), sizeof(unsigned) * code.size())) return rc;
            if (int rc = h2d(d.dv_pd, pd.data(), sizeof(int4) * pd.size())) return rc;
            if (int rc = h2d(d.dv_dd, dd.data(), sizeof(int) * dd.size())) return rc;
            if (int rc = h2d(d.dv_vd, vd.data(), sizeof(double) * vd.size())) return rc;
        }
    }
    pt.mark("dict");
    HostBuf<unsigned> pk;
    HostBuf<double> pv;
    std::vector<int2> pb;
    if ((enc & kEncSortedTiles) && !d.dv_code && !d.dv_ell && !d.dv_xell && !d.wave_rows && !d.vec_rows && d.nnz > 0 &&
        build_sorted_tiles(h, blk, pk, pv, pb)) {
        d.pk = dev_alloc<unsigned>((size_t)d.nnz);
        d.pb = dev_alloc<int2>(pb.size());
        if (!d.pk || !d.pb) return hip_fail(hipErrorOutOfMemory, "hipMalloc(sorted tiles)", __FILE__, __LINE__);
        if (int rc = h2d(d.pk, pk.data(), sizeof(unsigned) * (size_t)d.nnz)) return rc;
        if (int rc = h2d(d.pb, pb.data(), sizeof(int2) * pb.size())) return rc;
        pt.mark("sorted");
        HostBuf<unsigned char> vi;
        std::vector<int4> pd;
        std::vector<double> vd;
        if ((enc & kEncDict) && !(dz && *dz == '0') && build_value_dict(blk, h.row_ptr, pv, vi, pd, vd)) {
            d.dv_vi = dev_alloc<unsigned char>(vi.size());
            d.dv_pd = dev_alloc<int4>(pd.size());
            d.dv_vd = dev_alloc<double>(vd.size());
            if (!d.dv_vi || !d.dv_pd || !d.dv_vd)
                return hip_fail(hipErrorOutOfMemory, "hipMalloc(value dictionaries)", __FILE__, __LINE__);
            if (int rc = h2d(d.dv_vi, vi.data(), vi.size())) return rc;
            if (int rc = h2d(d.dv_pd, pd.data(), sizeof(int4) * pd.size())) return rc;
            if (int rc = h2d(d.dv_vd, vd.data(), sizeof(double) * vd.size())) return rc;
        } else {
            d.pv = dev_alloc<double>((size_t)d.nnz);
            if (!d.pv) return hip_fail(hipErrorOutOfMemory, "hipMalloc(sorted tiles)", __FILE__, __LINE__);
            if (int rc = h2d(d.pv, pv.data(), sizeof(double) * (size_t)d.nnz)) return rc;
        }
    }
    pt.mark("tiles");
    const long long nnz = d.nnz, nb = d.nblk, rows = d.n;
    if (has_dict(d)) {
        long long dict = 0;
        std::vector<int4> pd((size_t)nb);
        if (nb > 0) SSS_HIP(hipMemcpy(pd.data(), d.dv_pd, sizeof(int4) * (size_t)nb, hipMemcpyDeviceToHost));
        for (const auto &p : pd) dict += 4LL * p.y + 8LL * p.w;
        d.stream_bytes = d.dv_xell ? 4LL * d.xell_w * rows + 8 * (nb + 1) + 16 * nb + dict
                         : d.dv_ell ? (long long)(d.ell_w + (d.dv_ell_base ? 4 : 0)) * rows + 8 * (nb + 1) + 16 * nb + dict
                                  : (d.dv_vi ? 5 * nnz + 8 * nb : 4 * nnz) + 4 * (rows + 1) + 8 * (nb + 1) + 16 * nb + dict;
    } else if (d.pk) {
        d.stream_bytes = 12 * nnz + 4 * (rows + 1) + 8 * (nb + 1) + 8 * nb;
    } else {
        d.stream_bytes = 12 * nnz + 4 * (rows + 1) + 8 * (nb + 1);
    }
    return 0;
}

int devcsr_sort_rows(DevCSR &d, const SSS_MAT &h, const int *seg)
{
    if (!d.vec_rows || d.rows_sorted || d.nnz == 0) return 0;
    if (device_builders_on()) return sort_rows_device(d, seg);
    HostBuf<int> sci;
    HostBuf<double> sv;
    sort_row_segments(h, seg, sci, sv);
    if (int rc = h2d(d.ci, sci.data(), sizeof(int) * (size_t)d.nnz)) return rc;
    if (int rc = h2d(d.v, sv.data(), sizeof(double) * (size_t)d.nnz)) return rc;
    d.rows_sorted = true;
    return 0;
}

void devcsr_free(DevCSR &d)
{
    dev_free(d.rp);
    dev_free(d.ci);
    dev_free(d.v);
    dev_free(d.blk);
    dev_free(d.bk);
    dev_free(d.pk);
    dev_free(d.pv);
    dev_free(d.pb);
    dev_free(d.mg_gp);
    dev_free(d.mg_k);
    dev_free(d.mg_v);
    dev_free(d.dv_code);
    dev_free(d.dv_ell);
    dev_free(d.dv_ell_base);
    dev_free(d.dv_xell);
    dev_free(d.dv_vi);
    dev_free(d.dv_pd);
    dev_free(d.dv_dd);
    dev_free(d.dv_vd);
    delete[] d.h_bk;
    d = DevCSR();
}

template <int OP, bool NORM>
__device__ __forceinline__ double spmv_row_out(int r, double s, double alpha, double br, double *__restrict__ y, int cap)
{
    double out;
    if constexpr (OP == SSS_HIP_SPMV_MXY) out = s;
    else if constexpr (OP == SSS_HIP_SPMV_AMXPY) out = y[r] + s * alpha;
    else if constexpr (OP == SSS_HIP_SPMV_RESID) out = br + s * alpha;
    else {
        if (cap > 0 && r >= cap) return 0.0;
        out = y[r] + s;
    }
    y[r] = out;
    return NORM ? out * out : 0.0;
}
template <int OP, bool NORM>
__device__ __forceinline__ double spmv_row_out(int r, double s, double alpha, const double *__restrict__ b,
                                               double *__restrict__ y, int cap)
{
    double br = 0.0;
    if constexpr (OP == SSS_HIP_SPMV_RESID) br = b[r];
    return spmv_row_out<OP, NORM>(r, s, alpha, br, y, cap);
}

template <int OP, bool NORM, int DICT = 0>
__global__ __launch_bounds__(kBlock) void spmv_adaptive(const int2 *__restrict__ blk, const int *__restrict__ rp,
                                                        const int *__restrict__ ci, const double *__restrict__ v,
                                                        const double *__restrict__ x, const double *__restrict__ b,
                                                        double *__restrict__ y, double alpha, int cap,
                                                        double *__restrict__ partial, const unsigned *__restrict__ pk,
                                                        const double *__restrict__ pv, const int2 *__restrict__ pb,
                                                        DevDict dt = DevDict())
{
    if constexpr (DICT >= kXell) {
        constexpr int W = DICT - kXell;
        __shared__ XellSmem es;
        const int bid = blockIdx.x;
        double br = 0.0;
        const bool valid = bid < dt.bend;
        const XellRow<W> row = xell_row_begin<W>(valid, blk, bid, dt.xell, dt.pd, dt.vd, es, [&](int r) {
            if constexpr (OP == SSS_HIP_SPMV_RESID) br = b[r];
        });
        const unsigned(&w)[W] = row.w;
        const int r = row.r;
        __syncthreads();
        double sq = 0.0;
        if (row.live) {
            double xv[W];
            int ds;
            unsigned dcode;
            const int len = xell_gather<W>(w, r, dt.xshift, [&](int c) -> double { return x[c]; }, xv, ds, dcode);
            sq = spmv_row_out<OP, NORM>(r, xell_sum_g<false>(0.0, w, xv, es, dt.xshift, 0, len), alpha, br, y, cap);
        }
        if (NORM && valid) {
            const double t = block_sum(sq, es.red);
            if (threadIdx.x == 0) partial[bid] = t;
        }
    } else if constexpr (DICT >= 8) {
        constexpr int W = DICT;
        constexpr int RPT = kEllRpt;
        __shared__ EllSmem es[RPT];
        const int g = (int)blockIdx.x;
        EllRow<W> row[RPT];
        double br[RPT];
        int rb[RPT];
#pragma unroll
        for (int j = 0; j < RPT; ++j) {
            br[j] = 0.0;
            rb[j] = 0;
            row[j] = ell_row_begin<W>(blk, g * RPT + j, dt, es[j], [&](int r) {
                rb[j] = dt.ellb ? dt.ellb[r] : r;
                if constexpr (OP == SSS_HIP_SPMV_RESID) br[j] = b[r];
            });
        }
        __syncthreads();
#pragma unroll
        for (int j = 0; j < RPT; ++j) {
            double sq = 0.0;
            if (row[j].live) {
                double p[W];
                int ds;
                double dv;
                const int len = ell_decode<W>(row[j].w, rb[j], es[j], [&](int c) -> double { return x[c]; }, p, ds, dv);
                sq = spmv_row_out<OP, NORM>(row[j].r, ell_add(0.0, p, 0, len), alpha, br[j], y, cap);
            }
            if (NORM && row[j].valid) {
                const double t = block_sum(sq, es[j].red);
                if (threadIdx.x == 0) partial[g * RPT + j] = t;
            }
        }
    } else {
        __shared__ SpmvSmem sm;
        __shared__ std::conditional_t<DICT != 0, DictSmem, char> dsm;
        DictSmem *ds = nullptr;
        if constexpr (DICT != 0) ds = &dsm;
        const double sq = csr_block_rows(
            blk, rp, ci, v, x, sm, [&](int r, double s) -> double { return spmv_row_out<OP, NORM>(r, s, alpha, b, y, cap); },
            pk, pv, pb, &dt, ds);
        if (NORM) {
            const double t = block_sum(sq, sm.red);
            if (threadIdx.x == 0) partial[xcd_bid()] = t;
        }
    }
}

template <int OP, bool NORM, bool TREE>
__global__ __launch_bounds__(kBlock) void spmv_wave(int n, const int *__restrict__ rp, const int *__restrict__ ci,
                                                    const double *__restrict__ v, const double *__restrict__ x,
                                                    const double *__restrict__ b, double *__restrict__ y, double alpha,
                                                    int cap, double *__restrict__ partial)
{
    __shared__ __attribute__((aligned(16))) double strips[TREE ? 1 : 4][TREE ? 1 : kWaveStage];
    __shared__ double red[kBlock / 64];
    const int wave = threadIdx.x >> 6, lane = threadIdx.x & 63;
    const int r = xcd_bid() * 4 + wave;
    double sq = 0.0;
    if (r < n) {
        auto prod = [&](int c, double a) { return a * x[c]; };
        const double s = TREE ? wave_row_sum(rp[r], rp[r + 1], ci, v, prod)
                              : wave_row_chain<false>(rp[r], rp[r + 1], ci, v, prod, 0.0, strips[TREE ? 0 : wave]);
        if (lane == 0) sq = spmv_row_out<OP, NORM>(r, s, alpha, b, y, cap);
    }
    if (NORM) {
        const double t = block_sum(sq, red);
        if (threadIdx.x == 0) partial[xcd_bid()] = t;
    }
}

template <int OP, bool NORM, int G, bool LDSACC = false>
__global__ __launch_bounds__(kBlock) void spmv_merged(int n, int ng, int W, const int *__restrict__ gp,
                                                      const unsigned *__restrict__ mk, const double *__restrict__ mv,
                                                      const double *__restrict__ x, const double *__restrict__ b,
                                                      double *__restrict__ y, double alpha, int cap,
                                                      double *__restrict__ partial)
{
    __shared__ double red[8 * G];
    __shared__ double nred[kBlock / 64];
    __shared__ double acc[LDSACC ? 4 * G * kMergeAccDoubles : 1];
    int g = 0, u = 0;
    double sr = 0.0, unused = 0.0, sq = 0.0;
    if (merged_block<G, 1, LDSACC>(gp, ng, W, mk, mv, [&](int c) -> double { return x[c]; }, red, acc, g, u, sr,
                                   unused)) {
        const int r = g * G + u;
        if (r < n) sq = spmv_row_out<OP, NORM>(r, sr, alpha, b, y, cap);
    }
    if (NORM) {
        const double t = block_sum(sq, nred);
        if (threadIdx.x == 0) partial[xcd_bid()] = t;
    }
}

template <int OP, bool NORM>
static void launch_op(const DevCSR &A, double alpha, const double *x, const double *b, double *y, int cap,
                      double *partial, hipStream_t s)
{
    if (with_merged_kind(A, [&](auto G, auto ACC) {
            hipLaunchKernelGGL((spmv_merged<OP, NORM, decltype(G)::value, decltype(ACC)::value>), dim3(A.ngrid),
                               dim3(kBlock), 0, s, A.n, A.mg_ng, A.mg_W, A.mg_gp, A.mg_k, A.mg_v, x, b, y, alpha, cap,
                               partial);
        }))
        return;
    if (A.vec_rows)
        hipLaunchKernelGGL((spmv_wave<OP, NORM, true>), dim3(A.ngrid), dim3(kBlock), 0, s, A.n, A.rp, A.ci, A.v, x,
                           b, y, alpha, cap, partial);
    else if (A.wave_rows)
        hipLaunchKernelGGL((spmv_wave<OP, NORM, false>), dim3(A.ngrid), dim3(kBlock), 0, s, A.n, A.rp, A.ci, A.v, x,
                           b, y, alpha, cap, partial);
    else
        with_tile_kind(A, [&](auto K) {
            constexpr int KK = decltype(K)::value;
            DevDict dt = devdict(A, 0);
            dt.bend = A.nblk;
            const int grid = (A.nblk + rows_per_wg(KK) - 1) / rows_per_wg(KK);
            hipLaunchKernelGGL((spmv_adaptive<OP, NORM, KK>), dim3(grid), dim3(kBlock), 0, s, A.bk, A.rp, A.ci, A.v, x,
                               b, y, alpha, cap, partial, A.pk, A.pv, A.pb, dt);
        });
}

static double spmv_row_bytes(int op) { return op == SSS_HIP_SPMV_MXY ? 8.0 : 16.0; }

template <class F>
static bool with_spmv_op(int op, bool partial, F f)
{
    switch (op) {
    case SSS_HIP_SPMV_MXY: f(std::integral_constant<int, SSS_HIP_SPMV_MXY>(), std::false_type()); break;
    case SSS_HIP_SPMV_AMXPY: f(std::integral_constant<int, SSS_HIP_SPMV_AMXPY>(), std::false_type()); break;
    case SSS_HIP_SPMV_RESID:
        if (partial) f(std::integral_constant<int, SSS_HIP_SPMV_RESID>(), std::true_type());
        else f(std::integral_constant<int, SSS_HIP_SPMV_RESID>(), std::false_type());
        break;
    case SSS_HIP_SPMV_ACC: f(std::integral_constant<int, SSS_HIP_SPMV_ACC>(), std::false_type()); break;
    default: return false;
    }
    return true;
}

int launch_spmv(const DevCSR &A, int op, double alpha, const double *x, const double *b, double *y, int cap,
                double *partial, hipStream_t stream)
{
    if (A.n == 0 || A.nblk == 0) return 0;
    if (ledger_on()) ledger_add(matrix_bytes(A, 0, A.nblk) + xgather_bytes(A, A.n) + spmv_row_bytes(op) * A.n);
    if (!with_spmv_op(op, partial != nullptr, [&](auto O, auto NM) {
            launch_op<decltype(O)::value, decltype(NM)::value>(A, alpha, x, b, y, cap,
                                                               decltype(NM)::value ? partial : nullptr, stream);
        }))
        return ERROR_INPUT_PAR;
    SSS_HIP(hipGetLastError());
    return 0;
}

__global__ __launch_bounds__(kBlock) void prolong_inject(int m, int lo, const int *__restrict__ col,
                                                         const double *__restrict__ e, double *__restrict__ x)
{
    const int q = blockIdx.x * kBlock + (int)threadIdx.x;
    if (q < m) {
        const double s = 0.0 + 1.0 * e[col[q]];
        x[lo + q] = x[lo + q] + s * 1.0;
    }
}

int launch_prolong_inject(int m, int lo, const int *col, const double *e, double *x, hipStream_t s)
{
    if (m <= 0) return 0;
    ledger_add(28.0 * m);
    hipLaunchKernelGGL(prolong_inject, dim3((m + kBlock - 1) / kBlock), dim3(kBlock), 0, s, m, lo, col, e, x);
    SSS_HIP(hipGetLastError());
    return 0;
}

int launch_spmv_range(const DevCSR &A, int blo, int bhi, int op, double alpha, const double *x, const double *b,
                      double *y, double *partial, hipStream_t s)
{
    if (A.wave_rows || A.vec_rows || blo < 0 || bhi > A.nblk) return ERROR_INPUT_PAR;
    if (op != SSS_HIP_SPMV_RESID && op != SSS_HIP_SPMV_AMXPY && op != SSS_HIP_SPMV_MXY) return ERROR_INPUT_PAR;
    const int nb = bhi - blo;
    if (nb <= 0) return 0;
    if (ledger_on()) {
        const double rows = A.h_bk ? A.h_bk[bhi].x - A.h_bk[blo].x : (double)A.n * nb / A.nblk;
        ledger_add(matrix_bytes(A, blo, bhi) + xgather_bytes(A, rows) + spmv_row_bytes(op) * rows);
    }
    const int2 *pb = A.pb ? A.pb + blo : nullptr;
    double *pp = partial ? partial + blo : nullptr;
    DevDict dt = devdict(A, blo);
    dt.bend = nb;
    with_spmv_op(op, partial != nullptr, [&](auto op_c, auto norm_c) {
        constexpr int O = decltype(op_c)::value;
        constexpr bool NM = decltype(norm_c)::value;
        with_tile_kind(A, [&](auto K) {
            constexpr int KK = decltype(K)::value;
            const int grid = (nb + rows_per_wg(KK) - 1) / rows_per_wg(KK);
            hipLaunchKernelGGL((spmv_adaptive<O, NM, KK>), dim3(grid), dim3(kBlock), 0, s, A.bk + blo, A.rp, A.ci, A.v,
                               x, b, y, alpha, 0, pp, A.pk, A.pv, pb, dt);
        });
    });
    SSS_HIP(hipGetLastError());
    return 0;
}

constexpr int kFinalChunks = kFinalScratch;

__device__ __forceinline__ double block_sum_1024(double v, double *red)
{
    for (int off = 32; off > 0; off >>= 1) v += __shfl_xor(v, off, 64);
    if ((threadIdx.x & 63) == 0) red[threadIdx.x >> 6] = v;
    __syncthreads();
    double t = 0.0;
    if (threadIdx.x == 0)
        for (int w = 0; w < 1024 / 64; ++w) t += red[w];
    return t;
}

__global__ __launch_bounds__(1024) void final_sum_chunks(const double *__restrict__ partials, int n, int chunk,
                                                         double *__restrict__ scratch)
{
    __shared__ double red[1024 / 64];
    const int a = blockIdx.x * chunk, e = min(n, a + chunk);
    double v = 0.0;
    for (int i = a + (int)threadIdx.x; i < e; i += 1024) v += partials[i];
    const double t = block_sum_1024(v, red);
    if (threadIdx.x == 0) scratch[blockIdx.x] = t;
}

__global__ __launch_bounds__(1024) void final_sum_kernel(const double *__restrict__ partials, int n,
                                                         double *__restrict__ out, int take_sqrt)
{
    __shared__ double red[1024 / 64];
    double v = 0.0;
    for (int i = threadIdx.x; i < n; i += 1024) v += partials[i];
    const double t = block_sum_1024(v, red);
    if (threadIdx.x == 0) *out = take_sqrt ? sqrt(t) : t;
}

int launch_final_sum(double *partials, int n, double *out, bool take_sqrt, hipStream_t s)
{
    ledger_add(8.0 * n);
    if (n > 4 * 1024) {
        const int chunk = (n + kFinalChunks - 1) / kFinalChunks, nb = (n + chunk - 1) / chunk;
        hipLaunchKernelGGL(final_sum_chunks, dim3(nb), dim3(1024), 0, s, partials, n, chunk, partials + n);
        hipLaunchKernelGGL(final_sum_kernel, dim3(1), dim3(1024), 0, s, partials + n, nb, out, take_sqrt ? 1 : 0);
    } else {
        hipLaunchKernelGGL(final_sum_kernel, dim3(1), dim3(1024), 0, s, partials, n, out, take_sqrt ? 1 : 0);
    }
    SSS_HIP(hipGetLastError());
    return 0;
}

}

struct sss_hip_spmv_plan {
    sss::DevCSR csr;
};

// ... 40 lines not shown
```

amg_amd/csrc/sss_spmv_dev.hpp:

```cpp
#pragma once

#include "sss_engine.hpp"

namespace sss {

__device__ __forceinline__ int xcd_bid() { return blockIdx.x; }

struct SpmvSmem {
    alignas(16) double v[kTileEntries];
    double red[kBlock / 64];
    double d[kBlock];
};

struct DictSmem {
    int dd[256];
    double vd[256];
    unsigned char rowof[kTileEntries];
};
struct DevDict {
    const unsigned *code = nullptr;
    const int4 *pd = nullptr;
    const int *dd = nullptr;
    const double *vd = nullptr;
    const unsigned *pk = nullptr;
// ... 615 lines not shown
        else if (pk) stage_sorted(sm.v, k0, k1, pk, pv, pb[bid], r0, (double *)nullptr, fetch);
        else stage_products(sm.v, k0, k1, ci, v, x);
        __syncthreads();
        if (r < r1) {
            const double s = re - ra >= kPipeRowMin ? chain_pipe16<false>(0.0, sm.v, ra - k0, re - k0)
                                                    : chain_add(0.0, sm.v, ra - k0, re - k0);
            contrib = epi(r, s);
        }
    } else if (!ds && !pk) {
        constexpr int H = kTileEntries / 2;
        double s = 0.0;
        stage_products(sm.v, k0, min(k0 + H, k1), ci, v, x);
        __syncthreads();
        for (int base = k0, c = 0; base < k1; base += H, ++c) {
            const int m = min(H, k1 - base), nb = base + H;
            double *cur = sm.v + (c & 1) * H, *nxt = sm.v + ((c + 1) & 1) * H;
            if (threadIdx.x == 0) s = chain_pipe16<false>(s, cur, 0, m);
            else if (threadIdx.x >= 64 && nb < k1)
                stage_loop<true, kBlock - 64>(nxt, nb, min(nb + H, k1), ci, v, fetch, (int)threadIdx.x - 64);
            __syncthreads();
        }
        if (threadIdx.x == 0) contrib = epi(r0, s);
    } else {
        double s = 0.0;
        for (int base = k0; base < k1; base += kTileEntries) {
            const int m = min(kTileEntries, k1 - base);
            if (ds) stage_dict<false>(sm.v, base, base + m, *dt, bid, r0, r1, rp, *ds, (double *)nullptr, fetch);
            else if (pk) stage_sorted(sm.v, base, base + m, pk, pv, pb[bid], r0, (double *)nullptr, fetch);
            else stage_products(sm.v, base, base + m, ci, v, x);
            __syncthreads();
            if (dt && dt->tree_long) {
                const double c = block_tree_sum(sm.v, 0, m, sm.red);
                if (threadIdx.x == 0) s += c;
            } else if (threadIdx.x == 0) {
                s = chain_pipe16<false>(s, sm.v, 0, m);
            }
            __syncthreads();
        }
        if (threadIdx.x == 0) contrib = epi(r0, s);
    }
    return contrib;
}

template <class Epi>
__device__ __forceinline__ void csr_block_relax(const int *__restrict__ blk, const int *__restrict__ rp,
                                                const int *__restrict__ ci, const double *__restrict__ v,
                                                const int *__restrict__ map, const double *__restrict__ b,
                                                const double *x, SpmvSmem &sm, Epi epi)
{
    const int bid = xcd_bid();
    const int r0 = blk[bid], r1 = blk[bid + 1];
    const int k0 = rp[r0], k1 = rp[r1];
    const int cnt = k1 - k0;
    if (cnt <= kTileEntries) {
        const int r = r0 + (int)threadIdx.x;
        int ra = 0, re = 0, i = 0;
        if (r < r1) ra = rp[r], re = rp[r + 1], i = map[r];
        stage_products(sm.v, k0, k1, ci, v, x);
        __syncthreads();
        if (r < r1) {
            const double acc = chain_sub(b[i], sm.v, ra - k0, re - k0);
            epi(r, i, acc);
        }
    } else {
        const int i = map[r0];
        const double acc = long_row_chunks(
            k0, k1, b[i], [=, &sm](int base, int m) { stage_products(sm.v, base, base + m, ci, v, x); },
            [&sm](int, int m, double acc) { return threadIdx.x == 0 ? chain_sub(acc, sm.v, 0, m) : acc; });
        if (threadIdx.x == 0) epi(r0, i, acc);
    }
}
constexpr int kWaveStage = 256;
constexpr int kWaveRowMin = 600;
constexpr int kFreeRowMin = 300;

__device__ __forceinline__ void wave_sync()
{
    __builtin_amdgcn_fence(__ATOMIC_RELEASE, "wavefront");
    __builtin_amdgcn_wave_barrier();
    __builtin_amdgcn_fence(__ATOMIC_ACQUIRE, "wavefront");
}

template <bool SUB, class Prod>
__device__ __forceinline__ double wave_row_chain(int k0, int k1, const int *__restrict__ ci,
                                                 const double *__restrict__ v, Prod prod, double init,
                                                 double *strip)
{
    constexpr int U = kWaveStage / 64;
    const int lane = threadIdx.x & 63;
    double acc = init;
    for (int base = k0; base < k1; base += kWaveStage) {
        const int m = min(kWaveStage, k1 - base);
        int c[U];
        double a[U];
#pragma unroll
        for (int u = 0; u < U; ++u) {
            const int q = lane + 64 * u, qc = q < m ? q : m - 1;
            const int cv = ci[base + qc];
            const double av = v[base + qc];
            c[u] = cv;
            a[u] = q < m ? av : 0.0;
        }
        double pv[U];
#pragma unroll
        for (int u = 0; u < U; ++u) pv[u] = prod(c[u], a[u]);
#pragma unroll
        for (int u = 0; u < U; ++u) {
            const int q = lane + 64 * u;
            if (q < m) strip[q] = pv[u];
        }
        wave_sync();
        if (lane == 0) acc = chain_pipe16<SUB>(acc, strip, 0, m);
        wave_sync();
    }
    return acc;
}

template <class Prod>
__device__ __forceinline__ double wave_row_sum(int k0, int k1, const int *__restrict__ ci,
                                               const double *__restrict__ v, Prod prod)
{
    constexpr int U = 4;
    const int lane = threadIdx.x & 63;
    double s0 = 0.0, s1 = 0.0;
    for (int k = k0 + lane; k < k1; k += 64 * U) {
        int c[U];
        double a[U];
#pragma unroll
        for (int u = 0; u < U; ++u) {
            const int kk = k + 64 * u, kc = kk < k1 ? kk : k1 - 1;
            const int cv = ci[kc];
            const double av = v[kc];
            c[u] = cv;
            a[u] = kk < k1 ? av : 0.0;
        }
        double pv[U];
#pragma unroll
        for (int u = 0; u < U; ++u) pv[u] = prod(c[u], a[u]);
#pragma unroll
        for (int u = 0; u < U; ++u) {
            const double p = k + 64 * u < k1 ? pv[u] : 0.0;
            if (u & 1) s1 += p;
            else s0 += p;
        }
    }
    double s = s0 + s1;
#pragma unroll
    for (int off = 32; off > 0; off >>= 1) s += __shfl_xor(s, off, 64);
    return s;
}



template <int G, int S, class Fetch>
__device__ __forceinline__ void merged_sums(int k0, int k1, const unsigned *__restrict__ mk,
                                            const double *__restrict__ mv, Fetch fetch, double (&s0)[G],
                                            double (&s1)[G])
{
    constexpr int U = 8;
    const int lane = threadIdx.x & 63;
#pragma unroll
    for (int u = 0; u < G; ++u) s0[u] = 0.0, s1[u] = 0.0;
    for (int k = k0 + lane; k < k1 && S == 2; k += 64 * U) {
        unsigned q[U];
        double a[U];
#pragma unroll
        for (int t = 0; t < U; ++t) {
            const int kk = k + 64 * t;
            q[t] = kk < k1 ? mk[kk] : 0u;
            a[t] = kk < k1 ? mv[kk] : 0.0;
        }
#pragma unroll
        for (int t = 0; t < U; ++t) {
            if (k + 64 * t >= k1) break;
            const double p = a[t] * fetch((int)(q[t] >> kMergeShift));
            const unsigned key = q[t] & ((1u << kMergeShift) - 1);
#pragma unroll
            for (int u = 0; u < G; ++u) {
                s0[u] += key == (unsigned)u ? p : 0.0;
                s1[u] += key == (unsigned)(8 + u) ? p : 0.0;
            }
        }
    }
    for (int k = k0 + lane; k < k1 && S == 1; k += 64 * U) {
        unsigned q[U];
        double a[U], xv[U];
#pragma unroll
        for (int t = 0; t < U; ++t) {
            const int kk = k + 64 * t, kc = kk < k1 ? kk : k1 - 1;
            q[t] = mk[kc];
            a[t] = mv[kc];
        }
#pragma unroll
        for (int t = 0; t < U; ++t) xv[t] = k + 64 * t < k1 ? fetch((int)(q[t] >> kMergeShift)) : 0.0;
#pragma unroll
        for (int t = 0; t < U; ++t) {
            const bool live = k + 64 * t < k1;
            const double p = live ? a[t] * xv[t] : 0.0;
            const unsigned key = live ? q[t] & ((1u << kMergeShift) - 1) : 0u;
#pragma unroll
            for (int u = 0; u < G; ++u) {
                s0[u] += key == (unsigned)u ? p : 0.0;
                if (S == 2) s1[u] += key == (unsigned)(8 + u) ? p : 0.0;
            }
        }
    }
#pragma unroll
    for (int u = 0; u < G; ++u)
#pragma unroll
        for (int off = 32; off > 0; off >>= 1) {
            s0[u] += __shfl_xor(s0[u], off, 64);
            if (S == 2) s1[u] += __shfl_xor(s1[u], off, 64);
        }
}

constexpr int kMergeAccDoubles = 64;
template <int S>
constexpr int kMergeLdsChunks = S == 2 ? 6 : 8;
template <int G, int S>
constexpr unsigned kMergeKeyMask = S == 2 ? (8u | (unsigned)(G - 1)) : (unsigned)(G - 1);
template <int G, int S>
__device__ __forceinline__ constexpr int merged_acc_key(int a)
{
    return S == 2 ? (a / G) << 3 | (a % G) : a;
}
template <int G, int S>
__device__ __forceinline__ int merged_acc_base(int w)
{
    if (S == 2 && G == 4) return ((w >> 1) * 16 + (w & 1) * 4) * kMergeAccDoubles;
    return w * (S * G * kMergeAccDoubles);
}
template <int G, int S, int C, class Fetch>
__device__ __forceinline__ void merged_batch_lds(const unsigned *__restrict__ pk, const double *__restrict__ pv,
                                                 int last_n, Fetch fetch, double *mine)
{
    const int lane = threadIdx.x & 63;
    const int ll = min(lane, last_n - 1);
    unsigned q[C];
    double a[C], xv[C];
#pragma unroll
    for (int t = 0; t < C; ++t) {
        const int o = 64 * t + (t == C - 1 ? ll : lane);
        q[t] = pk[o];
        a[t] = pv[o];
    }
#pragma unroll
    for (int t = 0; t < C; ++t) xv[t] = fetch((int)(q[t] >> kMergeShift));
#pragma unroll
    for (int t = 0; t < C; ++t) {
        static_assert(kMergeKeyMask<G, S> < (1u << kMergeShift), "key bits");
        const unsigned key = q[t] & kMergeKeyMask<G, S>;
        double p = a[t] * xv[t];
        if (t == C - 1) p = lane < last_n ? p : 0.0;
        atomicAdd(&mine[key * kMergeAccDoubles], p);
    }
}
template <int G, int S, int C, class Fetch>
__device__ __forceinline__ void merged_batch_dispatch(int nch, const unsigned *__restrict__ pk,
                                                      const double *__restrict__ pv, int last_n, Fetch fetch,
                                                      double *mine)
{
    if constexpr (C == 1) {
        merged_batch_lds<G, S, 1>(pk, pv, last_n, fetch, mine);
    } else {
        if (nch == C) merged_batch_lds<G, S, C>(pk, pv, last_n, fetch, mine);
        else merged_batch_dispatch<G, S, C - 1>(nch, pk, pv, last_n, fetch, mine);
    }
}
template <int G, int S>
__device__ __forceinline__ void merged_tree_lds(const double *acc, double *out)
{
    constexpr int NA = S * G, LP = 64 / NA;
    static_assert(NA >= 2 && NA <= 32 && LP * NA == 64, "accumulators per wave");
    const int lane = threadIdx.x & 63, a = lane / LP, i = lane % LP;
    const double *col = acc + merged_acc_key<G, S>(a) * kMergeAccDoubles + i;
    wave_sync();
    double v[NA];
#pragma unroll
    for (int m = 0; m < NA; ++m) v[m] = col[LP * m];
#pragma unroll
    for (int h = NA / 2; h > 0; h >>= 1)
#pragma unroll
        for (int m = 0; m < h; ++m) v[m] += v[m + h];
    double s = v[0];
#pragma unroll
    for (int off = LP / 2; off > 0; off >>= 1) s += __shfl_xor(s, off, 64);
    if (i == 0) out[a] = s;
}
template <int G, int S, class Fetch>
__device__ __forceinline__ void merged_sums_lds(int k0, int k1, const unsigned *__restrict__ mk,
                                                const double *__restrict__ mv, Fetch fetch, double *acc,
                                                double *out)
{
    constexpr int U = kMergeLdsChunks<S>;
    const int lane = threadIdx.x & 63;
    double *mine = acc + lane;
#pragma unroll
    for (int a = 0; a < S * G; ++a) mine[merged_acc_key<G, S>(a) * kMergeAccDoubles] = 0.0;
    k1 = __builtin_amdgcn_readfirstlane(k1);
    for (int kb = __builtin_amdgcn_readfirstlane(k0); kb < k1; kb += 64 * U) {
        const int rem = min(k1 - kb, 64 * U), nch = (rem + 63) >> 6, last_n = rem - 64 * (nch - 1);
        const unsigned *pk = mk + kb;
        const double *pv = mv + kb;
        merged_batch_dispatch<G, S, U>(nch, pk, pv, last_n, fetch, mine);
    }
    merged_tree_lds<G, S>(acc, out);
}

template <int G, int S, bool LDSACC, class Fetch>
__device__ __forceinline__ bool merged_block(const int *__restrict__ gp, int ng, int W, const unsigned *__restrict__ mk,
                                             const double *__restrict__ mv, Fetch fetch, double *red, double *acc,
                                             int &g_out, int &u_out, double &t0, double &t1)
{
    const int w = __builtin_amdgcn_readfirstlane(threadIdx.x >> 6), lane = threadIdx.x & 63;
    const int wsh = W >= 4 ? 2 : W >= 2 ? 1 : 0, gpb = 4 >> wsh;
    const int g = xcd_bid() * gpb + (w >> wsh), part = w & ((1 << wsh) - 1);
    if (LDSACC && g < ng) {
        const int k0 = gp[g], k1 = gp[g + 1], len = k1 - k0, per = (len + (1 << wsh) - 1) >> wsh;
        merged_sums_lds<G, S>(k0 + min(len, part * per), k0 + min(len, (part + 1) * per), mk, mv, fetch,
                              acc + merged_acc_base<G, S>(w), red + (w * 2) * G);
    } else {
        double s0[G], s1[G];
        if (g < ng) {
            const int k0 = gp[g], k1 = gp[g + 1], len = k1 - k0, per = (len + (1 << wsh) - 1) >> wsh;
            merged_sums<G, S>(k0 + min(len, part * per), k0 + min(len, (part + 1) * per), mk, mv, fetch, s0, s1);
        } else {
#pragma unroll
            for (int u = 0; u < G; ++u) s0[u] = 0.0, s1[u] = 0.0;
        }
        if (lane == 0)
#pragma unroll
            for (int u = 0; u < G; ++u) {
                red[(w * 2) * G + u] = s0[u];
                if (S == 2) red[(w * 2 + 1) * G + u] = s1[u];
            }
    }
    __syncthreads();
    const int t = threadIdx.x;
    if (t >= gpb * G) return false;
    const int gi = t / G, u = t % G, gg = xcd_bid() * gpb + gi;
    if (gg >= ng) return false;
    const int w0 = gi << wsh;
    double a0 = red[(w0 * 2) * G + u], a1 = S == 2 ? red[(w0 * 2 + 1) * G + u] : 0.0;
    for (int v = 1; v < (1 << wsh); ++v) {
        a0 += red[((w0 + v) * 2) * G + u];
        if (S == 2) a1 += red[((w0 + v) * 2 + 1) * G + u];
    }
    g_out = gg, u_out = u, t0 = a0, t1 = a1;
    return true;
}

}
```

include/sss_hip.h:

```cpp
#ifndef SSS_HIP_H
#define SSS_HIP_H

#include "sss_amg.h"

#ifdef __cplusplus
extern "C" {
#endif

enum {
    SSS_HIP_SMOOTH_EXACT = 0,
    SSS_HIP_SMOOTH_HYBRID = 1,
    SSS_HIP_SMOOTH_JACOBI = 2
};
enum {
    SSS_HIP_COARSE_KRYLOV = 0,
    SSS_HIP_COARSE_DIRECT = 1
};
enum { SSS_HIP_VEC_B = 0, SSS_HIP_VEC_X = 1, SSS_HIP_VEC_WP = 2 };

typedef struct sss_hip_opts {
    int device;
    int smoother;
    int coarse;
    int row_cap;
    int use_graph;
    int verbose;
    int inner;
    int inner_from;
    int relabel;
    int sorted_tiles;
    int sum_order;
    int inner_long;
    int formats;
} sss_hip_opts;

#define SSS_HIP_LONG_ROW_MIN 300
void sss_hip_opts_default(sss_hip_opts *o);

int sss_hip_device_count(void);
int sss_hip_mem_info(size_t *free_bytes, size_t *total_bytes);

typedef struct sss_hip_hier sss_hip_hier;

sss_hip_hier *sss_hip_hier_create(const SSS_AMG *mg, const sss_hip_opts *o);
void sss_hip_hier_destroy(sss_hip_hier *h);

sss_hip_hier *sss_hip_setup_create(SSS_AMG *mg, SSS_MAT *A, SSS_AMG_PARS *pars, const sss_hip_opts *o,
                                   double *times);

int sss_hip_rap(const SSS_MAT *R, const SSS_MAT *A, const SSS_MAT *P, SSS_MAT *C);

#define SSS_SETUP_GPU_PMIS_MIN_DEFAULT 10000000
int sss_hip_pmis(const SSS_IMAT *S, int *mark, int *ncoarse, int *rounds);
int sss_pmis_host(const SSS_IMAT *S, int *mark, int *ncoarse, int *rounds);

#define SSS_SETUP_GPU_INTERP_MIN_DEFAULT 10000000
int sss_hip_std_pattern(const SSS_IMAT *S, const int *mark, int ncoarse, SSS_MAT *P);
int sss_hip_interp_std(const SSS_MAT *A, const SSS_IMAT *S, const int *mark, SSS_MAT *P, double trunc_threshold);
int sss_std_pattern_host(const SSS_IMAT *S, const int *mark, int ncoarse, SSS_MAT *P);

typedef void (*sss_setup_hook)(void *ctx, const SSS_AMG *mg, int done, int final);
void sss_amg_setup_hooked(SSS_AMG *mg, SSS_MAT *A, SSS_AMG_PARS *pars, sss_setup_hook hook, void *ctx);

int sss_hip_upload_vec(sss_hip_hier *h, int level, int which, const double *src, int n);
int sss_hip_download_vec(sss_hip_hier *h, int level, int which, double *dst, int n);

int sss_hip_cycle(sss_hip_hier *h);
int sss_hip_residual_norm(sss_hip_hier *h, double *absres);
int SSS_amg_save(const SSS_AMG *mg, const char *path);
int SSS_amg_load(SSS_AMG *mg, const char *path);

int sss_hip_pcg(sss_hip_hier *h, double tol, int maxit, int *iters, double *relres, double *hist, int hist_cap);
int sss_hip_fgmres(sss_hip_hier *h, double tol, int restart, int maxit, int *iters, double *relres, double *hist,
                   int hist_cap);
int sss_hip_coarse_solve(sss_hip_hier *h);
int sss_hip_smooth(sss_hip_hier *h, int level, int post);
int sss_hip_sync(sss_hip_hier *h);

typedef struct sss_hip_level_info {
    int rows, nnz, nnz_p, dag_f, dag_c, smoother_kind;
    int gs_engine_f, gs_engine_c, gs_stall, a_format;
    long long a_stream_bytes;
    int inner;
    int r_format, p_format;
    int pad_;
} sss_hip_level_info;
int sss_hip_level_info_get(sss_hip_hier *h, int level, sss_hip_level_info *out);
int sss_hip_num_levels(sss_hip_hier *h);
int sss_hip_tail_from(sss_hip_hier *h);
int sss_hip_cycle_launches(sss_hip_hier *h);
int sss_hip_cycle_bytes(sss_hip_hier *h, double *out, int nslots);

enum {
    SSS_HIP_SPMV_MXY = 0,
    SSS_HIP_SPMV_AMXPY = 1,
    SSS_HIP_SPMV_RESID = 2,
    SSS_HIP_SPMV_ACC = 3
};
typedef struct sss_hip_spmv_plan sss_hip_spmv_plan;
sss_hip_spmv_plan *sss_hip_spmv_plan_create(int n, int nnz, const int *d_rp, const int *h_rp);
void sss_hip_spmv_plan_destroy(sss_hip_spmv_plan *p);
int sss_hip_spmv(const sss_hip_spmv_plan *p, int op, double alpha, const int *d_rp, const int *d_ci,
                 const double *d_v, const double *d_x, const double *d_b, double *d_y, int cap,
                 void *stream);

int sss_hip_host_spmv(int op, double alpha, const SSS_MAT *A, const double *x, const double *b,
                      double *y, int cap);
int sss_hip_host_spmv_order(int op, double alpha, const SSS_MAT *A, const double *x, const double *b,
                            double *y, int cap, int sum_order);
int sss_hip_host_smooth(const SSS_SMTR *s, int post);
int sss_hip_host_orth(int n, int k, const double *V, double *w, double *hcol, double *norm);
void sss_hip_host_cache_clear(void);
int sss_hip_host_coarse_solve(SSS_MAT *A, SSS_VEC *b, SSS_VEC *x, double ctol, int coarse_mode,
                              int row_cap);

int sss_hip_time_level0_spmv(sss_hip_hier *h, int reps, double *avg_ms);
int sss_hip_time_levels(sss_hip_hier *h, int reps, double *level_ms, int nslots);
int sss_hip_time_level0_spmv_csr(sss_hip_hier *h, int reps, double *avg_ms);
int sss_hip_time_iterations(sss_hip_hier *h, int reps, double *avg_ms, double *absres);

typedef struct sss_hip_comm sss_hip_comm;
typedef struct sss_hip_dist sss_hip_dist;
typedef struct sss_hip_host_transport {
    void *ctx;
    int (*exchange)(void *ctx, int nsend, const int *sdst, const int *scount, const double *sbuf, int nrecv,
                    const int *rsrc, const int *rcount, double *rbuf);
    int (*allreduce_sum)(void *ctx, double *v, int n);
    int (*allgatherv)(void *ctx, const double *mine, int count, double *all, const int *counts, const int *displs);
} sss_hip_host_transport;

#define SSS_HIP_RCCL_ID_BYTES 128
int sss_hip_rccl_unique_id(unsigned char *id);
sss_hip_comm *sss_hip_comm_rccl(int nranks, int rank, const unsigned char *id, int device);
sss_hip_comm *sss_hip_comm_host(int nranks, int rank, const sss_hip_host_transport *t);
sss_hip_comm *sss_hip_comm_timing(int nranks, int rank);
void sss_hip_comm_destroy(sss_hip_comm *c);

sss_hip_dist *sss_hip_dist_create(const SSS_AMG *mg, const sss_hip_opts *o, sss_hip_comm *c, int agg_rows);
sss_hip_dist *sss_hip_dist_create_from_files(const char *prefix, const sss_hip_opts *o, sss_hip_comm *c);
void sss_hip_dist_destroy(sss_hip_dist *d);
int sss_hip_dist_info(sss_hip_dist *d, int *lo, int *hi, int *nagg, int *nghost0);
int sss_hip_dist_level_size(sss_hip_dist *d, int l, int *m, int *g, long long *nnz);
int sss_hip_dist_level_flags(sss_hip_dist *d, int l);
int sss_hip_dist_upload_vec(sss_hip_dist *d, int which, const double *own, int n);
int sss_hip_dist_download_vec(sss_hip_dist *d, int which, double *own, int n);
int sss_hip_dist_cycle(sss_hip_dist *d);
int sss_hip_dist_residual_norm(sss_hip_dist *d, double *absres);
int sss_hip_dist_sync(sss_hip_dist *d);
int sss_hip_dist_time_level0_spmv(sss_hip_dist *d, int reps, double *avg_ms);
int sss_hip_dist_time_levels(sss_hip_dist *d, int reps, double *cycle_ms, double *level_ms, int nslots);
int sss_hip_dist_time_tail_levels(sss_hip_dist *d, int reps, double *level_ms, int nslots);
int sss_hip_dist_halo_stats(sss_hip_dist *d, long long *calls, long long *doubles, int nslots, int reset,
                            int *nc_own, int *nc_all, int *tail_levels);

typedef struct sss_part_plan sss_part_plan;
sss_part_plan *sss_part_plan_create(const SSS_AMG *mg, int nranks, int rank, int agg_rows);
int sss_part_save(const SSS_AMG *mg, int nranks, int agg_rows, const char *prefix);
sss_part_plan *sss_part_plan_load(const char *path);
void sss_part_plan_destroy(sss_part_plan *p);
int sss_part_plan_nagg(const sss_part_plan *p);
int sss_part_plan_level(const sss_part_plan *p, int l, int *lo, int *hi, int *m, int *g);
int sss_part_plan_matrix(const sss_part_plan *p, int l, int which, SSS_MAT *out);
int sss_part_plan_ids(const sss_part_plan *p, int l, const int **perm, const int **ghosts);
int sss_part_plan_halo(const sss_part_plan *p, int l, int *nsend, const int **sdst, const int **scount,
                       const int **sidx, int *nrecv, const int **rsrc, const int **rcount);

int sss_gen_stencil(int kind, int nx, int ny, int nz, int z0, int z1, SSS_MAT *A);

#ifdef __cplusplus
}
#endif
#endif
```

Measured before the change: 54.34.

## Compress merged SpMV column keys to 16-bit deltas with per-chunk descriptors

Replaces the 32-bit sorted column keys of the merged-group SpMV/smoother format with 16-bit keys. Each key holds a 13-bit column offset from one or two per-64-entry base columns plus the accumulator slot, and the bases live in an int4 descriptor per chunk. Wave shares whose chunks cannot be encoded this way fall back to an escape array of full 32-bit keys. The intent is to cut index traffic in the bandwidth-bound fine-level kernels, at the cost of extra descriptor loads, decode arithmetic and more template instantiations. Gating depends on merge_key16_on().

Result: faster. 55.35, median of 6 (+1.9%).

```diff
diff --git a/amg_amd/_native.py b/amg_amd/_native.py
--- a/amg_amd/_native.py
+++ b/amg_amd/_native.py
@@ -107,6 +107,7 @@
     "SSS_amg_save", "SSS_amg_load",
     "sss_hip_coarse_solve", "sss_hip_smooth", "sss_hip_sync", "sss_hip_level_info_get", "sss_hip_num_levels", "sss_hip_tail_from",
     "sss_hip_cycle_launches", "sss_hip_cycle_bytes",
+    "sss_hip_merged_narrow", "sss_hip_merged_key_stats", "sss_hip_merged_keys_get",
     "sss_hip_spmv_plan_create", "sss_hip_spmv_plan_destroy", "sss_hip_spmv", "sss_hip_host_spmv", "sss_hip_host_spmv_order",
     "sss_hip_host_smooth", "sss_hip_host_coarse_solve", "sss_hip_host_cache_clear", "sss_hip_time_level0_spmv", "sss_hip_time_iterations",
     "sss_hip_time_level0_spmv_csr", "sss_hip_time_levels", "sss_hip_dist_time_tail_levels",
@@ -200,6 +201,11 @@
         "sss_hip_tail_from": (C.c_int, [C.c_void_p]),
         "sss_hip_cycle_launches": (C.c_int, [C.c_void_p]),
         "sss_hip_cycle_bytes": (C.c_int, [C.c_void_p, C.POINTER(C.c_double), C.c_int]),
+        "sss_hip_merged_narrow": (C.c_int, [C.c_void_p, C.c_longlong, _int_p, C.c_int, C.c_int, C.c_int, C.c_void_p,
+                                            C.c_void_p, C.c_longlong, P(C.c_longlong), C.c_void_p, C.c_longlong,
+                                            P(C.c_longlong), P(C.c_longlong)]),
+        "sss_hip_merged_key_stats": (C.c_int, [C.c_void_p, C.c_int, C.c_int, P(C.c_longlong)]),
+        "sss_hip_merged_keys_get": (C.c_int, [C.c_void_p, C.c_int, C.c_int, C.c_void_p, C.c_void_p, C.c_void_p]),
         "sss_hip_host_spmv": (C.c_int, [C.c_int, C.c_double, P(SSS_MAT), _dbl_p, _dbl_p, _dbl_p, C.c_int]),
         "sss_hip_host_spmv_order": (C.c_int, [C.c_int, C.c_double, P(SSS_MAT), _dbl_p, _dbl_p, _dbl_p, C.c_int, C.c_int]),
         "sss_hip_host_smooth": (C.c_int, [P(SSS_SMTR), C.c_int]),
diff --git a/amg_amd/csrc/sss_build.hip b/amg_amd/csrc/sss_build.hip
--- a/amg_amd/csrc/sss_build.hip
+++ b/amg_amd/csrc/sss_build.hip
@@ -56,6 +56,91 @@
     return 0;
 }
 
+struct ShareSpan {
+    int a, e;
+    long long d0;
+};
+__device__ __forceinline__ ShareSpan share_span(long long s, int W, const int *__restrict__ gp)
+{
+    const int g = (int)(s / W), part = (int)(s % W);
+    const long long k0 = gp[g], len = gp[g + 1] - k0, per = (len + W - 1) / W;
+    ShareSpan sp;
+    sp.a = (int)(k0 + min(len, part * per));
+    sp.e = (int)(k0 + min(len, (part + 1) * per));
+    sp.d0 = (sp.a >> 6) + (long long)g * W + part;
+    return sp;
+}
+__global__ __launch_bounds__(kBlock) void narrow_chunks(int ng, int W, int two, const int *__restrict__ gp,
+                                                        const unsigned *__restrict__ key,
+                                                        unsigned short *__restrict__ k16, int4 *__restrict__ desc,
+                                                        int *__restrict__ elen, unsigned long long *__restrict__ cnt)
+{
+    constexpr int kSpan = 1 << kMergeDeltaBits;
+    const int lane = threadIdx.x & 63;
+    const long long s = (long long)blockIdx.x * (kBlock / 64) + (threadIdx.x >> 6);
+    if (s >= (long long)ng * W) return;
+    const ShareSpan sp = share_span(s, W, gp);
+    unsigned c[4] = {0, 0, 0, 0};
+    bool wide = false;
+    int ch = 0;
+    for (int kb = sp.a; kb < sp.e; kb += 64, ++ch) {
+        const int m = min(64, sp.e - kb);
+        const bool live = lane < m;
+        const unsigned q = live ? key[kb + lane] : 0u;
+        const int col = (int)(q >> kMergeShift);
+        const int prev = __shfl_up(col, 1, 64);
+        const int w = (live && lane >= 1) ? col - prev : 0;
+        unsigned long long best = ((unsigned long long)(unsigned)w << 6) | (unsigned)(63 - lane);
+#pragma unroll
+        for (int off = 32; off > 0; off >>= 1) {
+            const unsigned long long o = __shfl_xor(best, off, 64);
+            best = o > best ? o : best;
+        }
+        int split = (best >> 6) > 0 ? 63 - (int)(best & 63) : 64;
+        const int first = __shfl(col, 0, 64), last = __shfl(col, m - 1, 64);
+        int lo = first, hi = first, kind;
+        if (last - first < kSpan) {
+            kind = 1, split = 64;
+        } else {
+            hi = __shfl(col, split, 64);
+            const int below = __shfl(col, split - 1, 64) - first;
+            kind = (below < kSpan && last - hi < kSpan) ? 2 : 3;
+        }
+        ++c[0], ++c[kind];
+        unsigned short k = 0;
+        int4 d = make_int4(0, 0, 64, -1);
+        if (kind == 3) {
+            wide = true;
+        } else {
+            d = make_int4(lo, hi, split, -1);
+            const unsigned acc = two ? ((q >> 1) & 4u) | (q & 3u) : q & 7u;
+            k = (unsigned short)((unsigned)(col - (lane < split ? lo : hi)) << 3 | acc);
+        }
+        if (live) k16[kb + lane] = k;
+        if (lane == 0) desc[sp.d0 + ch] = d;
+    }
+    if (lane == 0) {
+        elen[s] = wide ? sp.e - sp.a : 0;
+        for (int i = 0; i < 4; ++i)
+            if (c[i]) atomicAdd(&cnt[i], (unsigned long long)c[i]);
+        if (wide) atomicAdd(&cnt[4], (unsigned long long)ch);
+    }
+}
+__global__ __launch_bounds__(kBlock) void narrow_escape(int ng, int W, const int *__restrict__ gp,
+                                                        const unsigned *__restrict__ key, const int *__restrict__ eoff,
+                                                        int4 *__restrict__ desc, unsigned *__restrict__ ke)
+{
+    const int lane = threadIdx.x & 63;
+    const long long s = (long long)blockIdx.x * (kBlock / 64) + (threadIdx.x >> 6);
+    if (s >= (long long)ng * W) return;
+    const int o = eoff[s];
+    if (eoff[s + 1] == o) return;
+    const ShareSpan sp = share_span(s, W, gp);
+    const int m = sp.e - sp.a;
+    for (int i = lane; i < m; i += 64) ke[o + i] = key[sp.a + i];
+    for (int c = lane; c < (m + 63) >> 6; c += 64) desc[sp.d0 + c].w = o + 64 * c;
+}
+
 int upload_seg(const int *h_seg, int n, int **d_seg)
 {
     *d_seg = nullptr;
@@ -65,6 +150,58 @@
     return h2d(*d_seg, h_seg, sizeof(int) * (size_t)n);
 }
 
+int merged_narrow_device(DevCSR &d, const unsigned *sorted)
+{
+    const int ng = d.mg_ng, W = d.mg_W;
+    const long long ns = (long long)ng * W, nd = merged_desc_slots(d.nnz, ng, W);
+    d.mg_nd = nd;
+    d.mg_k16 = dev_alloc<unsigned short>((size_t)d.nnz);
+    d.mg_d = dev_alloc<int4>((size_t)nd);
+    int *elen = dev_alloc<int>((size_t)ns + 1), *eoff = dev_alloc<int>((size_t)ns + 1);
+    unsigned long long *cnt = dev_alloc<unsigned long long>(5);
+    void *tmp = nullptr;
+    int rc = (!d.mg_k16 || !d.mg_d || !elen || !eoff || !cnt) ? hip_fail(hipErrorOutOfMemory, "hipMalloc(narrow)", __FILE__, __LINE__) : 0;
+    auto check = [&](hipError_t e, const char *what) {
+        if (!rc && e != hipSuccess) rc = hip_fail(e, what, __FILE__, __LINE__);
+    };
+    if (!rc) {
+        check(hipMemsetAsync(d.mg_d, 0, sizeof(int4) * (size_t)nd, nullptr), "hipMemset(narrow)");
+        check(hipMemsetAsync(elen, 0, sizeof(int) * ((size_t)ns + 1), nullptr), "hipMemset(narrow)");
+        check(hipMemsetAsync(cnt, 0, sizeof(unsigned long long) * 5, nullptr), "hipMemset(narrow)");
+    }
+    const unsigned grid = (unsigned)((ns + kBlock / 64 - 1) / (kBlock / 64));
+    int total = 0;
+    if (!rc && ns > 0) {
+        hipLaunchKernelGGL(narrow_chunks, dim3(grid), dim3(kBlock), 0, nullptr, ng, W, d.mg_two ? 1 : 0, d.mg_gp, sorted,
+                           d.mg_k16, d.mg_d, elen, cnt);
+        check(hipGetLastError(), "narrow_chunks");
+        size_t tb = 0;
+        check(hipcub::DeviceScan::ExclusiveSum(nullptr, tb, elen, eoff, (int)(ns + 1), nullptr), "scan(narrow)");
+        check(hipMalloc(&tmp, std::max<size_t>(tb, 1)), "hipMalloc(narrow)");
+        if (!rc) check(hipcub::DeviceScan::ExclusiveSum(tmp, tb, elen, eoff, (int)(ns + 1), nullptr), "scan(narrow)");
+        if (!rc) check(hipMemcpy(&total, eoff + ns, sizeof(int), hipMemcpyDeviceToHost), "hipMemcpy(narrow)");
+    }
+    if (!rc) {
+        unsigned long long c[5] = {};
+        check(hipMemcpy(c, cnt, sizeof(c), hipMemcpyDeviceToHost), "hipMemcpy(narrow)");
+        for (int i = 0; i < 5; ++i) d.mg_cnt[i] = (long long)c[i];
+        d.mg_ne = total;
+        d.mg_ke = dev_alloc<unsigned>((size_t)std::max(total, 1));
+        if (!d.mg_ke) rc = hip_fail(hipErrorOutOfMemory, "hipMalloc(narrow)", __FILE__, __LINE__);
+    }
+    if (!rc && total > 0) {
+        hipLaunchKernelGGL(narrow_escape, dim3(grid), dim3(kBlock), 0, nullptr, ng, W, d.mg_gp, sorted, eoff, d.mg_d,
+                           d.mg_ke);
+        check(hipGetLastError(), "narrow_escape");
+    }
+    check(hipStreamSynchronize(nullptr), "narrow");
+    (void)hipFree(tmp);
+    dev_free(elen);
+    dev_free(eoff);
+    dev_free(cnt);
+    return rc;
+}
+
 }
 
 bool device_builders_on()
@@ -77,13 +214,14 @@
 {
     const int n = d.n, G = d.mg_G, ng = (n + G - 1) / G;
     d.mg_ng = ng;
+    const bool narrow = merged_key16_ok(d);
     d.mg_gp = dev_alloc<int>((size_t)ng + 1);
-    d.mg_k = dev_alloc<unsigned>((size_t)d.nnz);
+    unsigned *sorted = dev_alloc<unsigned>((size_t)d.nnz);
     d.mg_v = dev_alloc<double>((size_t)d.nnz);
     unsigned *key = dev_alloc<unsigned>((size_t)d.nnz);
     int *dseg = nullptr;
-    int rc = (!d.mg_gp || !d.mg_k || !d.mg_v || !key) ? hip_fail(hipErrorOutOfMemory, "hipMalloc(merged)", __FILE__, __LINE__)
-                                                        : upload_seg(h_seg, n, &dseg);
+    int rc = (!d.mg_gp || !sorted || !d.mg_v || !key) ? hip_fail(hipErrorOutOfMemory, "hipMalloc(merged)", __FILE__, __LINE__)
+                                                       : upload_seg(h_seg, n, &dseg);
     if (!rc) {
         hipLaunchKernelGGL(group_bounds, dim3((ng + kBlock) / kBlock), dim3(kBlock), 0, nullptr, n, G, ng, d.rp, d.mg_gp);
         if (n > 0)
@@ -92,9 +230,15 @@
         const hipError_t e = hipGetLastError();
         if (e != hipSuccess) rc = hip_fail(e, "merged_keys", __FILE__, __LINE__);
     }
-    if (!rc) rc = segmented_sort(key, d.mg_k, d.v, d.mg_v, d.nnz, ng, d.mg_gp, nullptr);
+    if (!rc) rc = segmented_sort(key, sorted, d.v, d.mg_v, d.nnz, ng, d.mg_gp, nullptr);
     dev_free(key);
     dev_free(dseg);
+    if (!narrow || rc) {
+        d.mg_k = sorted;
+        return rc;
+    }
+    rc = merged_narrow_device(d, sorted);
+    dev_free(sorted);
     return rc;
 }
 
diff --git a/amg_amd/csrc/sss_engine.hpp b/amg_amd/csrc/sss_engine.hpp
--- a/amg_amd/csrc/sss_engine.hpp
+++ b/amg_amd/csrc/sss_engine.hpp
@@ -196,8 +196,26 @@
     bool mg_two = false;
     unsigned *mg_k = nullptr;
     double *mg_v = nullptr;
-};
+    unsigned short *mg_k16 = nullptr;
+    int4 *mg_d = nullptr;
+    unsigned *mg_ke = nullptr;
+    long long mg_nd = 0, mg_ne = 0;
+    long long mg_cnt[5] = {};
+};
+struct MergedKeys {
+    const unsigned *k;
+    const unsigned short *k16;
+    const int4 *d;
+    const unsigned *ke;
+};
+__host__ __device__ inline MergedKeys merged_keys_of(const DevCSR &A) { return MergedKeys{A.mg_k, A.mg_k16, A.mg_d, A.mg_ke}; }
 constexpr int kMergeShift = 4;
+constexpr int kMergeDeltaBits = 13;
+inline long long merged_desc_slots(long long nnz, int ng, int W) { return (nnz >> 6) + (long long)ng * W + 1; }
+void merged_narrow(const unsigned *keys, long long nnz, const int *gp, int ng, bool two, int W, unsigned short *k16,
+                   int *desc, std::vector<unsigned> &esc, long long cnt[5]);
+bool merge_key16_on();
+inline bool merged_key16_ok(const DevCSR &d) { return merge_key16_on() && d.mg_G > 0 && !(d.mg_two && d.mg_G > 4); }
 constexpr int kTileShift = 11;
 constexpr int kTileColBits = 20;
 constexpr unsigned kTileDiagMark = (1u << kTileColBits) - 256;
@@ -250,10 +268,16 @@
 template <class F>
 inline bool with_merged_kind(const DevCSR &A, F f)
 {
-    if (A.mg_G == 8 && A.mg_acc) f(std::integral_constant<int, 8>{}, std::true_type{});
-    else if (A.mg_G == 8) f(std::integral_constant<int, 8>{}, std::false_type{});
-    else if (A.mg_G == 4 && A.mg_acc) f(std::integral_constant<int, 4>{}, std::true_type{});
-    else if (A.mg_G == 4) f(std::integral_constant<int, 4>{}, std::false_type{});
+    auto acc = [&](auto G, auto K16) {
+        if (A.mg_acc) f(G, std::true_type{}, K16);
+        else f(G, std::false_type{}, K16);
+    };
+    auto keys = [&](auto G) {
+        if (A.mg_k16) acc(G, std::true_type{});
+        else acc(G, std::false_type{});
+    };
+    if (A.mg_G == 8) keys(std::integral_constant<int, 8>{});
+    else if (A.mg_G == 4) keys(std::integral_constant<int, 4>{});
     else return false;
     return true;
 }
diff --git a/amg_amd/csrc/sss_hier.hip b/amg_amd/csrc/sss_hier.hip
--- a/amg_amd/csrc/sss_hier.hip
+++ b/amg_amd/csrc/sss_hier.hip
@@ -1373,6 +1373,41 @@
     return 0;
 }
 
+static const DevCSR *merged_copy(sss_hip_hier *h, int level, int which)
+{
+    if (!h || level < 0 || level >= h->nl || which < 0 || which > 4) return nullptr;
+    auto &L = h->L[level];
+    if (which == 0) return &L.A;
+    const auto &p = L.sm.pass[(which - 1) & 1];
+    return which <= 2 ? &p.ts_nl : &p.ts_lo;
+}
+
+extern "C" int sss_hip_merged_key_stats(sss_hip_hier *h, int level, int which, long long *out)
+{
+    const DevCSR *M = merged_copy(h, level, which);
+    if (!M || !out) return ERROR_INPUT_PAR;
+    for (int i = 0; i < 8; ++i) out[i] = 0;
+    if (!M->mg_k16) return 1;
+    for (int i = 0; i < 5; ++i) out[i] = M->mg_cnt[i];
+    out[5] = M->nnz, out[6] = M->mg_nd, out[7] = M->mg_ne;
+    return 0;
+}
+
+extern "C" int sss_hip_merged_keys_get(sss_hip_hier *h, int level, int which, unsigned short *k16, int *desc,
+                                       unsigned *esc)
+{
+    const DevCSR *M = merged_copy(h, level, which);
+    if (!M || !M->mg_k16 || !k16 || !desc) return ERROR_INPUT_PAR;
+    SSS_HIP(hipDeviceSynchronize());
+    SSS_HIP(hipMemcpy(k16, M->mg_k16, sizeof(unsigned short) * (size_t)M->nnz, hipMemcpyDeviceToHost));
+    SSS_HIP(hipMemcpy(desc, M->mg_d, sizeof(int4) * (size_t)M->mg_nd, hipMemcpyDeviceToHost));
+    if (M->mg_ne > 0) {
+        if (!esc) return ERROR_INPUT_PAR;
+        SSS_HIP(hipMemcpy(esc, M->mg_ke, sizeof(unsigned) * (size_t)M->mg_ne, hipMemcpyDeviceToHost));
+    }
+    return 0;
+}
+
 extern "C" int sss_hip_time_levels(sss_hip_hier *h, int reps, double *level_ms, int nslots)
 {
     if (!h || reps < 1 || nslots < h->nl) return ERROR_INPUT_PAR;
diff --git a/amg_amd/csrc/sss_smooth.hip b/amg_amd/csrc/sss_smooth.hip
--- a/amg_amd/csrc/sss_smooth.hip
+++ b/amg_amd/csrc/sss_smooth.hip
@@ -789,7 +789,7 @@
     }
 }
 
-template <int PATH, bool LDSACC = false>
+template <int PATH, bool LDSACC = false, bool K16 = false>
 __global__ __launch_bounds__(kBlock) void ts_stage0(int lo, DevCSR M, const int *__restrict__ split,
                                                     const double *__restrict__ b, XSrc x,
                                                     const double *__restrict__ deff, double *__restrict__ P,
@@ -832,8 +832,9 @@
         __shared__ double acc[LDSACC ? 4 * 2 * G * kMergeAccDoubles : 1];
         int g = 0, u = 0;
         double n_sum = 0.0, l_sum = 0.0;
-        if (merged_block<G, 2, LDSACC>(M.mg_gp, M.mg_ng, M.mg_W, M.mg_k, M.mg_v, [&](int c) -> double { return x(c); },
-                                       red, acc, g, u, n_sum, l_sum)) {
+        constexpr bool K = K16 && 2 * G <= 8;
+        if (merged_block<G, 2, LDSACC, K>(M.mg_gp, M.mg_ng, M.mg_W, merged_keys_of(M), M.mg_v,
+                                          [&](int c) -> double { return x(c); }, red, acc, g, u, n_sum, l_sum)) {
             const int q = g * G + u;
             if (q < M.n) {
                 const double Pq = b[lo + q] - n_sum;
@@ -920,7 +921,7 @@
     }
 }
 
-template <int PATH, bool LDSACC = false>
+template <int PATH, bool LDSACC = false, bool K16 = false>
 __global__ __launch_bounds__(kBlock) void ts_inner(int lo, DevCSR M, const double *__restrict__ deff,
                                                    const double *__restrict__ P, const double *ycols, int col_off,
                                                    const double *ykeep, double *__restrict__ y)
@@ -958,8 +959,8 @@
         __shared__ double acc[LDSACC ? 4 * G * kMergeAccDoubles : 1];
         int g = 0, u = 0;
         double l_sum = 0.0, unused = 0.0;
-        if (merged_block<G, 1, LDSACC>(M.mg_gp, M.mg_ng, M.mg_W, M.mg_k, M.mg_v, fetch, red, acc, g, u, l_sum,
-                                       unused)) {
+        if (merged_block<G, 1, LDSACC, K16>(M.mg_gp, M.mg_ng, M.mg_W, merged_keys_of(M), M.mg_v, fetch, red, acc, g, u,
+                                            l_sum, unused)) {
             const int q = g * G + u;
             if (q < M.n) finish(q, P[q] - l_sum);
         }
@@ -1026,9 +1027,9 @@
 {
     if (M.n == 0) return;
     ledger_add((double)M.stream_bytes + 40.0 * M.n);
-    if (M.mg_two && with_merged_kind(M, [&](auto G, auto ACC) {
-            hipLaunchKernelGGL((ts_stage0<decltype(G)::value, decltype(ACC)::value>), dim3(M.ngrid), dim3(kBlock), 0, s,
-                               lo, M, split, b, x, deff, P, y);
+    if (M.mg_two && with_merged_kind(M, [&](auto G, auto ACC, auto K16) {
+            hipLaunchKernelGGL((ts_stage0<decltype(G)::value, decltype(ACC)::value, decltype(K16)::value>), dim3(M.ngrid),
+                               dim3(kBlock), 0, s, lo, M, split, b, x, deff, P, y);
         }))
         return;
     if (M.vec_rows)
@@ -1050,9 +1051,9 @@
 {
     if (M.n == 0) return;
     ledger_add((double)M.stream_bytes + 40.0 * M.n);
-    if (with_merged_kind(M, [&](auto G, auto ACC) {
-            hipLaunchKernelGGL((ts_inner<decltype(G)::value, decltype(ACC)::value>), dim3(M.ngrid), dim3(kBlock), 0, s,
-                               lo, M, deff, P, ycols, col_off, ykeep, y);
+    if (with_merged_kind(M, [&](auto G, auto ACC, auto K16) {
+            hipLaunchKernelGGL((ts_inner<decltype(G)::value, decltype(ACC)::value, decltype(K16)::value>), dim3(M.ngrid),
+                               dim3(kBlock), 0, s, lo, M, deff, P, ycols, col_off, ykeep, y);
         }))
         return;
     if (M.vec_rows)
diff --git a/amg_amd/csrc/sss_spmv.hip b/amg_amd/csrc/sss_spmv.hip
--- a/amg_amd/csrc/sss_spmv.hip
+++ b/amg_amd/csrc/sss_spmv.hip
@@ -429,6 +429,111 @@
         }
     });
     gp[ng] = rp[n];
+}
+
+bool merge_key16_on()
+{
+    const char *e = getenv("SSS_HIP_MERGE_KEY16");
+    return !(e && *e == '0');
+}
+
+void merged_narrow(const unsigned *keys, long long nnz, const int *gp, int ng, bool two, int W, unsigned short *k16,
+                   int *desc, std::vector<unsigned> &esc, long long cnt[5])
+{
+    constexpr int kSpan = 1 << kMergeDeltaBits;
+    const long long nd = merged_desc_slots(nnz, ng, W);
+    std::memset(desc, 0, sizeof(int) * 4 * (size_t)nd);
+    std::vector<long long> eoff((size_t)ng * W + 1, 0);
+    std::mutex mu;
+    for (int i = 0; i < 5; ++i) cnt[i] = 0;
+    auto acc_of = [two](unsigned q) { return two ? ((q >> 1) & 4u) | (q & 3u) : q & 7u; };
+    parallel_chunks(ng, 64, [&](int glo, int ghi) {
+        long long c[5] = {};
+        for (int g = glo; g < ghi; ++g) {
+            const long long k0 = gp[g], len = gp[g + 1] - k0, per = (len + W - 1) / W;
+            for (int part = 0; part < W; ++part) {
+                const long long a = k0 + std::min(len, part * per), e = k0 + std::min(len, (part + 1) * per);
+                if (a >= e) continue;
+                const long long d0 = (a >> 6) + (long long)g * W + part;
+                bool wide = false;
+                for (long long kb = a, ch = 0; kb < e; kb += 64, ++ch) {
+                    const int m = (int)std::min<long long>(64, e - kb);
+                    int *d = desc + 4 * (d0 + ch);
+                    const int first = (int)(keys[kb] >> kMergeShift), last = (int)(keys[kb + m - 1] >> kMergeShift);
+                    int split = 64, gap = 0;
+                    for (int l = 1; l < m; ++l) {
+                        const int w = (int)(keys[kb + l] >> kMergeShift) - (int)(keys[kb + l - 1] >> kMergeShift);
+                        if (w > gap) gap = w, split = l;
+                    }
+                    ++c[0];
+                    int lo = first, hi = first, kind;
+                    if (last - first < kSpan) {
+                        kind = 1, split = 64;
+                    } else {
+                        hi = (int)(keys[kb + split] >> kMergeShift);
+                        const int below = (int)(keys[kb + split - 1] >> kMergeShift) - first;
+                        kind = (below < kSpan && last - hi < kSpan) ? 2 : 3;
+                    }
+                    ++c[kind];
+                    if (kind == 3) {
+                        wide = true;
+                        d[0] = d[1] = 0, d[2] = 64, d[3] = -1;
+                        for (int l = 0; l < m; ++l) k16[kb + l] = 0;
+                        continue;
+                    }
+                    d[0] = lo, d[1] = hi, d[2] = split, d[3] = -1;
+                    for (int l = 0; l < m; ++l) {
+                        const unsigned q = keys[kb + l];
+                        const unsigned delta = (q >> kMergeShift) - (unsigned)(l < split ? lo : hi);
+                        k16[kb + l] = (unsigned short)(delta << 3 | acc_of(q));
+                    }
+                }
+                if (wide) {
+                    eoff[(size_t)g * W + part] = e - a;
+                    c[4] += (e - a + 63) >> 6;
+                }
+            }
+        }
+        std::lock_guard<std::mutex> lk(mu);
+        for (int i = 0; i < 5; ++i) cnt[i] += c[i];
+    });
+    long long run = 0;
+    for (auto &x : eoff) {
+        const long long l = x;
+        x = run, run += l;
+    }
+    esc.resize((size_t)run);
+    parallel_chunks(ng, 64, [&](int glo, int ghi) {
+        for (int g = glo; g < ghi; ++g) {
+            const long long k0 = gp[g], len = gp[g + 1] - k0, per = (len + W - 1) / W;
+            for (int part = 0; part < W; ++part) {
+                const size_t s = (size_t)g * W + part;
+                if (eoff[s + 1] == eoff[s]) continue;
+                const long long a = k0 + std::min(len, part * per), e = k0 + std::min(len, (part + 1) * per);
+                const long long d0 = (a >> 6) + (long long)g * W + part;
+                std::memcpy(esc.data() + eoff[s], keys + a, sizeof(unsigned) * (size_t)(e - a));
+                for (long long kb = a, ch = 0; kb < e; kb += 64, ++ch) desc[4 * (d0 + ch) + 3] = (int)(eoff[s] + 64 * ch);
+            }
+        }
+    });
+}
+
+extern "C" int sss_hip_merged_narrow(const unsigned *keys, long long nnz, const int *gp, int ng, int two, int W,
+                                     unsigned short *k16, int *desc, long long desc_cap, long long *n_desc,
+                                     unsigned *esc, long long esc_cap, long long *n_esc, long long *counts)
+{
+    if (!keys || !gp || ng < 0 || nnz < 0 || (W != 1 && W != 2 && W != 4) || !k16 || !desc || !n_desc || !n_esc || !counts)
+        return ERROR_INPUT_PAR;
+    if (nnz >= (1ll << 31) || gp[ng] != nnz) return ERROR_INPUT_PAR;
+    const long long nd = merged_desc_slots(nnz, ng, W);
+    *n_desc = nd;
+    if (desc_cap < nd) return ERROR_INPUT_PAR;
+    std::vector<unsigned> e;
+    merged_narrow(keys, nnz, gp, ng, two != 0, W, k16, desc, e, counts);
+    *n_esc = (long long)e.size();
+    if ((long long)e.size() > esc_cap || (!e.empty() && !esc)) return ERROR_INPUT_PAR;
+    if (!e.empty()) std::memcpy(esc, e.data(), sizeof(unsigned) * e.size());
+    return 0;
 }
 
 DevDict devdict(const DevCSR &A, int blo)
@@ -754,6 +859,27 @@
     return 1;
 }
 
+static int merged_upload_narrow(DevCSR &d, const unsigned *hk, const int *hgp)
+{
+    const long long nd = merged_desc_slots(d.nnz, d.mg_ng, d.mg_W);
+    HostBuf<unsigned short> k16;
+    HostBuf<int> desc;
+    std::vector<unsigned> esc;
+    k16.resize((size_t)d.nnz);
+    desc.resize(4 * (size_t)nd);
+    merged_narrow(hk, d.nnz, hgp, d.mg_ng, d.mg_two, d.mg_W, k16.data(), desc.data(), esc, d.mg_cnt);
+    d.mg_nd = nd, d.mg_ne = (long long)esc.size();
+    d.mg_k16 = dev_alloc<unsigned short>((size_t)d.nnz);
+    d.mg_d = dev_alloc<int4>((size_t)nd);
+    d.mg_ke = dev_alloc<unsigned>(std::max<size_t>(esc.size(), 1));
+    if (!d.mg_k16 || !d.mg_d || !d.mg_ke) return hip_fail(hipErrorOutOfMemory, "hipMalloc(merged)", __FILE__, __LINE__);
+    if (int rc = h2d(d.mg_k16, k16.data(), sizeof(unsigned short) * (size_t)d.nnz)) return rc;
+    if (int rc = h2d(d.mg_d, desc.data(), sizeof(int4) * (size_t)nd)) return rc;
+    if (!esc.empty())
+        if (int rc = h2d(d.mg_ke, esc.data(), sizeof(unsigned) * esc.size())) return rc;
+    return 0;
+}
+
 int devcsr_upload(DevCSR &d, const SSS_MAT &h, int split, int enc, const int *seg)
 {
     PhaseTimer pt("devcsr");
@@ -820,12 +946,18 @@
         d.mg_W = d.mg_W >= 4 ? 4 : d.mg_W >= 2 ? 2 : 1;
         d.mg_acc = merge_acc(d.mg_G, d.mg_two);
         d.ngrid = (d.mg_ng + 4 / d.mg_W - 1) / (4 / d.mg_W);
+        const bool narrow = merged_key16_ok(d);
         d.mg_gp = dev_alloc<int>(gp.size());
-        d.mg_k = dev_alloc<unsigned>(mk.size());
+        if (!narrow) d.mg_k = dev_alloc<unsigned>(mk.size());
         d.mg_v = dev_alloc<double>(mv.size());
-        if (!d.mg_gp || !d.mg_k || !d.mg_v) return hip_fail(hipErrorOutOfMemory, "hipMalloc(merged)", __FILE__, __LINE__);
+        if (!d.mg_gp || (!narrow && !d.mg_k) || !d.mg_v)
+            return hip_fail(hipErrorOutOfMemory, "hipMalloc(merged)", __FILE__, __LINE__);
         if (int rc = h2d(d.mg_gp, gp.data(), sizeof(int) * gp.size())) return rc;
-        if (int rc = h2d(d.mg_k, mk.data(), sizeof(unsigned) * mk.size())) return rc;
+        if (narrow) {
+            if (int rc = merged_upload_narrow(d, mk.data(), gp.data())) return rc;
+        } else if (int rc = h2d(d.mg_k, mk.data(), sizeof(unsigned) * mk.size())) {
+            return rc;
+        }
         if (int rc = h2d(d.mg_v, mv.data(), sizeof(double) * mv.size())) return rc;
     }
     if (d.vec_rows && !((enc & kEncMergedOnly) && d.mg_G > 0) && device_builders_on() && d.nnz > 0)
@@ -977,6 +1109,7 @@
     } else {
         d.stream_bytes = 12 * nnz + 4 * (rows + 1) + 8 * (nb + 1);
     }
+    if (d.mg_k16) d.stream_bytes += 2 * nnz + 16 * d.mg_nd + 4 * d.mg_ne - 4 * nnz;
     return 0;
 }
 
@@ -1006,6 +1139,9 @@
     dev_free(d.mg_gp);
     dev_free(d.mg_k);
     dev_free(d.mg_v);
+    dev_free(d.mg_k16);
+    dev_free(d.mg_d);
+    dev_free(d.mg_ke);
     dev_free(d.dv_code);
     dev_free(d.dv_ell);
     dev_free(d.dv_ell_base);
@@ -1145,9 +1281,9 @@
     }
 }
 
-template <int OP, bool NORM, int G, bool LDSACC = false>
+template <int OP, bool NORM, int G, bool LDSACC = false, bool K16 = false>
 __global__ __launch_bounds__(kBlock) void spmv_merged(int n, int ng, int W, const int *__restrict__ gp,
-                                                      const unsigned *__restrict__ mk, const double *__restrict__ mv,
+                                                      MergedKeys mk, const double *__restrict__ mv,
                                                       const double *__restrict__ x, const double *__restrict__ b,
                                                       double *__restrict__ y, double alpha, int cap,
                                                       double *__restrict__ partial)
@@ -1157,8 +1293,8 @@
     __shared__ double acc[LDSACC ? 4 * G * kMergeAccDoubles : 1];
     int g = 0, u = 0;
     double sr = 0.0, unused = 0.0, sq = 0.0;
-    if (merged_block<G, 1, LDSACC>(gp, ng, W, mk, mv, [&](int c) -> double { return x[c]; }, red, acc, g, u, sr,
-                                   unused)) {
+    if (merged_block<G, 1, LDSACC, K16>(gp, ng, W, mk, mv, [&](int c) -> double { return x[c]; }, red, acc, g, u, sr,
+                                        unused)) {
         const int r = g * G + u;
         if (r < n) sq = spmv_row_out<OP, NORM>(r, sr, alpha, b, y, cap);
     }
@@ -1172,10 +1308,10 @@
 static void launch_op(const DevCSR &A, double alpha, const double *x, const double *b, double *y, int cap,
                       double *partial, hipStream_t s)
 {
-    if (with_merged_kind(A, [&](auto G, auto ACC) {
-            hipLaunchKernelGGL((spmv_merged<OP, NORM, decltype(G)::value, decltype(ACC)::value>), dim3(A.ngrid),
-                               dim3(kBlock), 0, s, A.n, A.mg_ng, A.mg_W, A.mg_gp, A.mg_k, A.mg_v, x, b, y, alpha, cap,
-                               partial);
+    if (with_merged_kind(A, [&](auto G, auto ACC, auto K16) {
+            hipLaunchKernelGGL((spmv_merged<OP, NORM, decltype(G)::value, decltype(ACC)::value, decltype(K16)::value>),
+                               dim3(A.ngrid), dim3(kBlock), 0, s, A.n, A.mg_ng, A.mg_W, A.mg_gp, merged_keys_of(A), A.mg_v,
+                               x, b, y, alpha, cap, partial);
         }))
         return;
     if (A.vec_rows)
diff --git a/amg_amd/csrc/sss_spmv_dev.hpp b/amg_amd/csrc/sss_spmv_dev.hpp
--- a/amg_amd/csrc/sss_spmv_dev.hpp
+++ b/amg_amd/csrc/sss_spmv_dev.hpp
@@ -791,29 +791,56 @@
 
 
 
-template <int G, int S, class Fetch>
-__device__ __forceinline__ void merged_sums(int k0, int k1, const unsigned *__restrict__ mk,
+
+typedef const int __attribute__((address_space(4))) *MergedDesc;
+__device__ __forceinline__ MergedDesc merged_desc(const int4 *d) { return (MergedDesc)(unsigned long long)d; }
+struct MergedChunk {
+    int lo, hi, split;
+};
+__device__ __forceinline__ MergedChunk merged_chunk(MergedDesc d, int c)
+{
+    return MergedChunk{d[4 * c], d[4 * c + 1], d[4 * c + 2]};
+}
+__device__ __forceinline__ int merged_col16(unsigned q, const MergedChunk &d, int el)
+{
+    return (int)(q >> 3) + (el < d.split ? d.lo : d.hi);
+}
+template <int S, class KT>
+__device__ __forceinline__ unsigned merged_code(unsigned q)
+{
+    if constexpr (sizeof(KT) == 2) return S == 2 ? ((q & 4u) << 1) | (q & 3u) : q & 7u;
+    else return q & ((1u << kMergeShift) - 1);
+}
+template <int G, int S, class KT, class Fetch>
+__device__ __forceinline__ void merged_sums(int k0, int k1, const KT *__restrict__ mk, MergedDesc md,
                                             const double *__restrict__ mv, Fetch fetch, double (&s0)[G],
                                             double (&s1)[G])
 {
     constexpr int U = 8;
+    constexpr bool K16 = sizeof(KT) == 2;
     const int lane = threadIdx.x & 63;
+    const int lastc = ((k1 - k0 + 63) >> 6) - 1, lastl = (k1 - 1 - k0) & 63;
 #pragma unroll
     for (int u = 0; u < G; ++u) s0[u] = 0.0, s1[u] = 0.0;
-    for (int k = k0 + lane; k < k1 && S == 2; k += 64 * U) {
+    for (int k = k0 + lane, cb = 0; k < k1 && S == 2; k += 64 * U, cb += U) {
         unsigned q[U];
         double a[U];
+        MergedChunk d[U];
 #pragma unroll
         for (int t = 0; t < U; ++t) {
             const int kk = k + 64 * t;
             q[t] = kk < k1 ? mk[kk] : 0u;
             a[t] = kk < k1 ? mv[kk] : 0.0;
+            if constexpr (K16) d[t] = merged_chunk(md, min(cb + t, lastc));
         }
 #pragma unroll
         for (int t = 0; t < U; ++t) {
             if (k + 64 * t >= k1) break;
-            const double p = a[t] * fetch((int)(q[t] >> kMergeShift));
-            const unsigned key = q[t] & ((1u << kMergeShift) - 1);
+            int col;
+            if constexpr (K16) col = merged_col16(q[t], d[t], lane);
+            else col = (int)(q[t] >> kMergeShift);
+            const double p = a[t] * fetch(col);
+            const unsigned key = merged_code<S, KT>(q[t]);
 #pragma unroll
             for (int u = 0; u < G; ++u) {
                 s0[u] += key == (unsigned)u ? p : 0.0;
@@ -821,22 +848,29 @@
             }
         }
     }
-    for (int k = k0 + lane; k < k1 && S == 1; k += 64 * U) {
+    for (int k = k0 + lane, cb = 0; k < k1 && S == 1; k += 64 * U, cb += U) {
         unsigned q[U];
         double a[U], xv[U];
+        MergedChunk d[U];
 #pragma unroll
         for (int t = 0; t < U; ++t) {
             const int kk = k + 64 * t, kc = kk < k1 ? kk : k1 - 1;
             q[t] = mk[kc];
             a[t] = mv[kc];
-        }
-#pragma unroll
-        for (int t = 0; t < U; ++t) xv[t] = k + 64 * t < k1 ? fetch((int)(q[t] >> kMergeShift)) : 0.0;
+            if constexpr (K16) d[t] = merged_chunk(md, min(cb + t, lastc));
+        }
+#pragma unroll
+        for (int t = 0; t < U; ++t) {
+            int col;
+            if constexpr (K16) col = merged_col16(q[t], d[t], k + 64 * t < k1 ? lane : lastl);
+            else col = (int)(q[t] >> kMergeShift);
+            xv[t] = k + 64 * t < k1 ? fetch(col) : 0.0;
+        }
 #pragma unroll
         for (int t = 0; t < U; ++t) {
             const bool live = k + 64 * t < k1;
             const double p = live ? a[t] * xv[t] : 0.0;
-            const unsigned key = live ? q[t] & ((1u << kMergeShift) - 1) : 0u;
+            const unsigned key = live ? merged_code<S, KT>(q[t]) : 0u;
 #pragma unroll
             for (int u = 0; u < G; ++u) {
                 s0[u] += key == (unsigned)u ? p : 0.0;
@@ -858,61 +892,75 @@
 constexpr int kMergeLdsChunks = S == 2 ? 6 : 8;
 template <int G, int S>
 constexpr unsigned kMergeKeyMask = S == 2 ? (8u | (unsigned)(G - 1)) : (unsigned)(G - 1);
-template <int G, int S>
+template <int G, int S, bool DENSE = false>
 __device__ __forceinline__ constexpr int merged_acc_key(int a)
 {
-    return S == 2 ? (a / G) << 3 | (a % G) : a;
-}
-template <int G, int S>
+    return S == 2 && !DENSE ? (a / G) << 3 | (a % G) : a;
+}
+template <int G, int S, bool DENSE = false>
 __device__ __forceinline__ int merged_acc_base(int w)
 {
-    if (S == 2 && G == 4) return ((w >> 1) * 16 + (w & 1) * 4) * kMergeAccDoubles;
+    if (S == 2 && G == 4 && !DENSE) return ((w >> 1) * 16 + (w & 1) * 4) * kMergeAccDoubles;
     return w * (S * G * kMergeAccDoubles);
 }
-template <int G, int S, int C, class Fetch>
-__device__ __forceinline__ void merged_batch_lds(const unsigned *__restrict__ pk, const double *__restrict__ pv,
-                                                 int last_n, Fetch fetch, double *mine)
-{
+template <int G, int S, bool DENSE, class KT>
+__device__ __forceinline__ unsigned merged_slot(unsigned q)
+{
+    static_assert(kMergeKeyMask<G, S> < (1u << kMergeShift), "key bits");
+    static_assert(!DENSE || S * G <= 8, "accumulator bits of a narrow key");
+    if constexpr (sizeof(KT) == 2) return q & (unsigned)(S * G - 1);
+    else if constexpr (DENSE && S == 2) return ((q >> 1) & (unsigned)G) | (q & (unsigned)(G - 1));
+    else return q & kMergeKeyMask<G, S>;
+}
+template <int G, int S, int C, bool DENSE, class KT, class Fetch>
+__device__ __forceinline__ void merged_batch_lds(const KT *__restrict__ pk, MergedDesc pd,
+                                                 const double *__restrict__ pv, int last_n, Fetch fetch, double *mine)
+{
+    constexpr bool K16 = sizeof(KT) == 2;
     const int lane = threadIdx.x & 63;
     const int ll = min(lane, last_n - 1);
     unsigned q[C];
     double a[C], xv[C];
+    MergedChunk d[C];
 #pragma unroll
     for (int t = 0; t < C; ++t) {
         const int o = 64 * t + (t == C - 1 ? ll : lane);
         q[t] = pk[o];
         a[t] = pv[o];
-    }
-#pragma unroll
-    for (int t = 0; t < C; ++t) xv[t] = fetch((int)(q[t] >> kMergeShift));
+        if constexpr (K16) d[t] = merged_chunk(pd, t);
+    }
 #pragma unroll
     for (int t = 0; t < C; ++t) {
-        static_assert(kMergeKeyMask<G, S> < (1u << kMergeShift), "key bits");
-        const unsigned key = q[t] & kMergeKeyMask<G, S>;
+        if constexpr (K16) xv[t] = fetch(merged_col16(q[t], d[t], t == C - 1 ? ll : lane));
+        else xv[t] = fetch((int)(q[t] >> kMergeShift));
+    }
+#pragma unroll
+    for (int t = 0; t < C; ++t) {
+        const unsigned key = merged_slot<G, S, DENSE, KT>(q[t]);
         double p = a[t] * xv[t];
         if (t == C - 1) p = lane < last_n ? p : 0.0;
         atomicAdd(&mine[key * kMergeAccDoubles], p);
     }
 }
-template <int G, int S, int C, class Fetch>
-__device__ __forceinline__ void merged_batch_dispatch(int nch, const unsigned *__restrict__ pk,
+template <int G, int S, int C, bool DENSE, class KT, class Fetch>
+__device__ __forceinline__ void merged_batch_dispatch(int nch, const KT *__restrict__ pk, MergedDesc pd,
                                                       const double *__restrict__ pv, int last_n, Fetch fetch,
                                                       double *mine)
 {
     if constexpr (C == 1) {
-        merged_batch_lds<G, S, 1>(pk, pv, last_n, fetch, mine);
+        merged_batch_lds<G, S, 1, DENSE>(pk, pd, pv, last_n, fetch, mine);
     } else {
-        if (nch == C) merged_batch_lds<G, S, C>(pk, pv, last_n, fetch, mine);
-        else merged_batch_dispatch<G, S, C - 1>(nch, pk, pv, last_n, fetch, mine);
-    }
-}
-template <int G, int S>
+        if (nch == C) merged_batch_lds<G, S, C, DENSE>(pk, pd, pv, last_n, fetch, mine);
+        else merged_batch_dispatch<G, S, C - 1, DENSE>(nch, pk, pd, pv, last_n, fetch, mine);
+    }
+}
+template <int G, int S, bool DENSE = false>
 __device__ __forceinline__ void merged_tree_lds(const double *acc, double *out)
 {
     constexpr int NA = S * G, LP = 64 / NA;
     static_assert(NA >= 2 && NA <= 32 && LP * NA == 64, "accumulators per wave");
     const int lane = threadIdx.x & 63, a = lane / LP, i = lane % LP;
-    const double *col = acc + merged_acc_key<G, S>(a) * kMergeAccDoubles + i;
+    const double *col = acc + merged_acc_key<G, S, DENSE>(a) * kMergeAccDoubles + i;
     wave_sync();
     double v[NA];
 #pragma unroll
@@ -926,8 +974,8 @@
     for (int off = LP / 2; off > 0; off >>= 1) s += __shfl_xor(s, off, 64);
     if (i == 0) out[a] = s;
 }
-template <int G, int S, class Fetch>
-__device__ __forceinline__ void merged_sums_lds(int k0, int k1, const unsigned *__restrict__ mk,
+template <int G, int S, bool DENSE, class KT, class Fetch>
+__device__ __forceinline__ void merged_sums_lds(int k0, int k1, const KT *__restrict__ mk, MergedDesc md,
                                                 const double *__restrict__ mv, Fetch fetch, double *acc,
                                                 double *out)
 {
@@ -935,34 +983,48 @@
     const int lane = threadIdx.x & 63;
     double *mine = acc + lane;
 #pragma unroll
-    for (int a = 0; a < S * G; ++a) mine[merged_acc_key<G, S>(a) * kMergeAccDoubles] = 0.0;
+    for (int a = 0; a < S * G; ++a) mine[merged_acc_key<G, S, DENSE>(a) * kMergeAccDoubles] = 0.0;
     k1 = __builtin_amdgcn_readfirstlane(k1);
-    for (int kb = __builtin_amdgcn_readfirstlane(k0); kb < k1; kb += 64 * U) {
+    for (int kb = __builtin_amdgcn_readfirstlane(k0); kb < k1; kb += 64 * U, md += 4 * U) {
         const int rem = min(k1 - kb, 64 * U), nch = (rem + 63) >> 6, last_n = rem - 64 * (nch - 1);
-        const unsigned *pk = mk + kb;
+        const KT *pk = mk + kb;
         const double *pv = mv + kb;
-        merged_batch_dispatch<G, S, U>(nch, pk, pv, last_n, fetch, mine);
-    }
-    merged_tree_lds<G, S>(acc, out);
-}
-
-template <int G, int S, bool LDSACC, class Fetch>
-__device__ __forceinline__ bool merged_block(const int *__restrict__ gp, int ng, int W, const unsigned *__restrict__ mk,
+        merged_batch_dispatch<G, S, U, DENSE>(nch, pk, md, pv, last_n, fetch, mine);
+    }
+    merged_tree_lds<G, S, DENSE>(acc, out);
+}
+
+template <int G, int S, bool LDSACC, bool K16, class Fetch>
+__device__ __forceinline__ bool merged_block(const int *__restrict__ gp, int ng, int W, const MergedKeys &mk,
                                              const double *__restrict__ mv, Fetch fetch, double *red, double *acc,
                                              int &g_out, int &u_out, double &t0, double &t1)
 {
     const int w = __builtin_amdgcn_readfirstlane(threadIdx.x >> 6), lane = threadIdx.x & 63;
     const int wsh = W >= 4 ? 2 : W >= 2 ? 1 : 0, gpb = 4 >> wsh;
     const int g = xcd_bid() * gpb + (w >> wsh), part = w & ((1 << wsh) - 1);
+    int ka = 0, kb = 0;
+    if (g < ng) {
+        const int k0 = gp[g], k1 = gp[g + 1], len = k1 - k0, per = (len + (1 << wsh) - 1) >> wsh;
+        ka = k0 + min(len, part * per), kb = k0 + min(len, (part + 1) * per);
+    }
+    const unsigned *k32 = mk.k;
+    MergedDesc md = nullptr;
+    bool narrow = false;
+    if (K16 && ka < kb) {
+        md = merged_desc(mk.d) + 4 * (long long)__builtin_amdgcn_readfirstlane((ka >> 6) + (g << wsh) + part);
+        const int esc = md[3];
+        narrow = esc < 0;
+        if (!narrow) k32 = mk.ke + ((long long)esc - ka);
+    }
     if (LDSACC && g < ng) {
-        const int k0 = gp[g], k1 = gp[g + 1], len = k1 - k0, per = (len + (1 << wsh) - 1) >> wsh;
-        merged_sums_lds<G, S>(k0 + min(len, part * per), k0 + min(len, (part + 1) * per), mk, mv, fetch,
-                              acc + merged_acc_base<G, S>(w), red + (w * 2) * G);
+        double *mine = acc + merged_acc_base<G, S, K16>(w), *out = red + (w * 2) * G;
+        if (K16 && narrow) merged_sums_lds<G, S, K16>(ka, kb, mk.k16, md, mv, fetch, mine, out);
+        else merged_sums_lds<G, S, K16>(ka, kb, k32, (MergedDesc)nullptr, mv, fetch, mine, out);
     } else {
         double s0[G], s1[G];
         if (g < ng) {
-            const int k0 = gp[g], k1 = gp[g + 1], len = k1 - k0, per = (len + (1 << wsh) - 1) >> wsh;
-            merged_sums<G, S>(k0 + min(len, part * per), k0 + min(len, (part + 1) * per), mk, mv, fetch, s0, s1);
+            if (K16 && narrow) merged_sums<G, S>(ka, kb, mk.k16, md, mv, fetch, s0, s1);
+            else merged_sums<G, S>(ka, kb, k32, (MergedDesc)nullptr, mv, fetch, s0, s1);
         } else {
 #pragma unroll
             for (int u = 0; u < G; ++u) s0[u] = 0.0, s1[u] = 0.0;
diff --git a/include/sss_hip.h b/include/sss_hip.h
--- a/include/sss_hip.h
+++ b/include/sss_hip.h
@@ -87,6 +87,12 @@
 } sss_hip_level_info;
 int sss_hip_level_info_get(sss_hip_hier *h, int level, sss_hip_level_info *out);
 int sss_hip_num_levels(sss_hip_hier *h);
+int sss_hip_merged_narrow(const unsigned *keys, long long nnz, const int *gp, int ng, int two, int W,
+                          unsigned short *k16, int *desc, long long desc_cap, long long *n_desc,
+                          unsigned *esc, long long esc_cap, long long *n_esc, long long *counts);
+int sss_hip_merged_key_stats(sss_hip_hier *h, int level, int which, long long *out);
+int sss_hip_merged_keys_get(sss_hip_hier *h, int level, int which, unsigned short *k16, int *desc,
+                            unsigned *esc);
 int sss_hip_tail_from(sss_hip_hier *h);
 int sss_hip_cycle_launches(sss_hip_hier *h);
 int sss_hip_cycle_bytes(sss_hip_hier *h, double *out, int nslots);
```
